# OAID/Tengine

Hardware: AMD Instinct MI355X
Metric: images/sec int8 MobileNet-v1 224x224 (higher is better)
Workload: dtype int8; 1 GPU; mobilenet_v1 int8 batch=1 per GPU (BASELINE configs[1]), weights = seeded synthetic tmfile, input resident in HBM, direct AQL dispatch of the launch list (14 packets per step), 1 stream(s); streams=1, halves=0, global_batch=1, parallelism=dp1, collectives=none

## Files before the change

include/tengine_amd.h:

```cpp
#ifndef TENGINE_AMD_H
#define TENGINE_AMD_H

#include <stddef.h>
#include <stdint.h>

#ifdef __cplusplus
extern "C" {
#endif

#define TAMD_API __attribute__((visibility("default")))

enum { TAMD_DT_FP32 = 0, TAMD_DT_FP16 = 1, TAMD_DT_INT8 = 2, TAMD_DT_UINT8 = 3, TAMD_DT_INT32 = 4 };
enum { TAMD_TT_VAR = 1, TAMD_TT_CONST = 2, TAMD_TT_INPUT = 3 };

enum {
    TAMD_OP_INPUT = 0,
    TAMD_OP_CONST = 1,
    TAMD_OP_CONV = 2,
    TAMD_OP_FC = 3,
    TAMD_OP_POOL = 4,
    TAMD_OP_RELU = 5,
    TAMD_OP_ELTWISE = 6,
    TAMD_OP_CONCAT = 7,
    TAMD_OP_DROPOUT = 8,
    TAMD_OP_UPSAMPLE = 9,
    TAMD_OP_RELU6 = 10,
    TAMD_OP_FLATTEN = 11,
    TAMD_OP_SOFTMAX = 12,
    TAMD_OP_PERMUTE = 13,
    TAMD_OP_RESHAPE = 14,
    TAMD_OP_PRIORBOX = 15,
    TAMD_OP_SIGMOID = 16,
    TAMD_OP_CLIP = 17,
    TAMD_OP_HARDSWISH = 18,
    TAMD_OP_MISH = 19,
    TAMD_OP_INTERP = 20,
    TAMD_OP_SPLIT = 22,
    TAMD_OP_SHUFFLECHANNEL = 23,
    TAMD_OP_PRELU = 25,
    TAMD_OP_SLICE = 26,
    TAMD_OP_TRANSPOSE = 28,
    TAMD_OP_CROP = 30,
    TAMD_OP_BATCHNORM = 32,
    TAMD_OP_NUM
};

typedef struct tamd_conv_param {
    int kernel_h, kernel_w, stride_h, stride_w;
    int pad_h0, pad_h1, pad_w0, pad_w1;
    int dilation_h, dilation_w;
    int input_channel, output_channel, group, activation;
} tamd_conv_param;

typedef struct tamd_fc_param { int num_output; } tamd_fc_param;

typedef struct tamd_pool_param {
    int pool_method, kernel_h, kernel_w, stride_h, stride_w;
    int pad_h0, pad_h1, pad_w0, pad_w1;
    int global, caffe_flavor;
} tamd_pool_param;

typedef struct tamd_relu_param { float negative_slope; } tamd_relu_param;
typedef struct tamd_batchnorm_param { float rescale_factor, eps; int caffe_flavor; } tamd_batchnorm_param;
typedef struct tamd_eltwise_param { int type; int caffe_flavor; float shift, power, scale; } tamd_eltwise_param;
typedef struct tamd_concat_param { int axis; } tamd_concat_param;
typedef struct tamd_upsample_param { float scale; } tamd_upsample_param;
typedef struct tamd_permute_param { int order[4]; } tamd_permute_param;
typedef struct tamd_softmax_param { int axis; } tamd_softmax_param;
typedef struct tamd_reshape_param { int dim_num; int dims[8]; } tamd_reshape_param;
typedef struct tamd_clip_param { float max, min; } tamd_clip_param;
typedef struct tamd_hardswish_param { float alpha, beta; } tamd_hardswish_param;
typedef struct tamd_interp_param { int resize_type; float width_scale, height_scale; int output_width, output_height; } tamd_interp_param;
#define TAMD_SPLIT_MAX 8
typedef struct tamd_split_param { int axis; int num; int sizes[TAMD_SPLIT_MAX]; } tamd_split_param;
typedef struct tamd_shufflechannel_param { int group; } tamd_shufflechannel_param;
typedef struct tamd_slice_param {
    int axis, begin, end, step;
    int iscaffe, ismxnet, isonnx;
    int slice_point_num, begin_num, size_num;
} tamd_slice_param;
typedef struct tamd_transpose_param { int dim_num; int order[8]; } tamd_transpose_param;
typedef struct tamd_crop_param { int num_args, offset_c, offset_h, offset_w, crop_h, crop_w, center_crop, axis, flag; } tamd_crop_param;

#define TAMD_PRIORBOX_MAX 8
typedef struct tamd_priorbox_param {
    int min_size_num, max_size_num, aspect_ratio_num;
    float min_size[TAMD_PRIORBOX_MAX], max_size[TAMD_PRIORBOX_MAX], aspect_ratio[TAMD_PRIORBOX_MAX], variance[4];
    int flip, clip, image_h, image_w;
    float step_h, step_w, offset;
} tamd_priorbox_param;

typedef struct tamd_tensor_desc {
    int dtype;
    int ttype;
    int dim_num;
    int dims[8];
    const void* data;
    int quant_num;
    const float* scales;
    const int* zero_points;
    const char* name;
} tamd_tensor_desc;

typedef struct tamd_node_desc {
    int op;
    int input_num;
    const int* inputs;
    int output_num;
    const int* outputs;
    const void* param;
    const char* name;
} tamd_node_desc;

typedef struct tamd_options {
    const char* dev_name;
    int size;
    int gpu_index;
    int use_hip_graph;
    int profile;
    int direct_dispatch;
    int keep_tensors;
    int u8_integer;
    int split_batch;
} tamd_options;
#define TAMD_OPTIONS_HAS(size, field) ((size) >= (int)(offsetof(tamd_options, field) + sizeof(((const tamd_options*)0)->field)))

typedef struct tamd_graph tamd_graph;

TAMD_API int tamd_device_count(void);
TAMD_API int tamd_init(int gpu_index);
TAMD_API int tamd_shutdown(void);
TAMD_API const char* tamd_last_error(void);
TAMD_API const char* tamd_version(void);
TAMD_API int tamd_op_supported(int op, int dtype);
TAMD_API int tamd_node_supported(const tamd_node_desc* node, const tamd_tensor_desc* inputs, int input_num,
                                 const tamd_tensor_desc* outputs, int output_num);
TAMD_API int tamd_lut_table(int op, int dtype, const void* param, float in_scale, int in_zp, float out_scale, int out_zp,
                            unsigned char table[256]);
TAMD_API int tamd_eltwise_table(int type, int dtype, const tamd_eltwise_param* param, float scalar, float in_scale, int in_zp,
                                float out_scale, int out_zp, unsigned char table[256]);
TAMD_API int tamd_eltwise_scalar(int const_dtype, const void* value, float scale, int zp, float* scalar);
TAMD_API int tamd_eltwise_pair(int type, int dtype, unsigned char a, float a_scale, int a_zp, unsigned char b, float b_scale, int b_zp,
                               float out_scale, int out_zp);
TAMD_API int tamd_batchnorm_table(const tamd_batchnorm_param* param, float gamma, float beta, float mean, float var, float in_scale, int in_zp,
                                  float out_scale, int out_zp, unsigned char table[256]);
TAMD_API int tamd_interp_table(int dtype, float in_scale, int in_zp, float out_scale, int out_zp, unsigned char table[256]);
TAMD_API int tamd_interp_indices(int in_extent, int out_extent, float scale, int* idx);
TAMD_API int tamd_shuffle_sources(int channels, int group, int* src);
TAMD_API int tamd_split_table(float in_scale, int in_zp, float out_scale, int out_zp, unsigned char table[256]);
TAMD_API int tamd_slice_table(float in_scale, int in_zp, float out_scale, int out_zp, unsigned char table[256]);
TAMD_API int tamd_transpose_table(int dtype, float in_scale, int in_zp, float out_scale, int out_zp, unsigned char table[256]);
TAMD_API float tamd_prelu_slope(unsigned short half_bits);
TAMD_API int tamd_prelu_table(int dtype, unsigned short slope_bits, float in_scale, int in_zp, float out_scale, int out_zp,
                              unsigned char table[256]);

TAMD_API tamd_graph* tamd_graph_create(void);
TAMD_API int tamd_graph_add_tensor(tamd_graph* g, const tamd_tensor_desc* desc);
TAMD_API int tamd_graph_add_node(tamd_graph* g, const tamd_node_desc* desc);
TAMD_API int tamd_graph_set_inputs(tamd_graph* g, int n, const int* tensor_ids);
TAMD_API int tamd_graph_set_outputs(tamd_graph* g, int n, const int* tensor_ids);
TAMD_API tamd_graph* tamd_graph_load_tm2(const void* mem, size_t size);
TAMD_API int tamd_graph_set_batch(tamd_graph* g, int batch);

TAMD_API int tamd_graph_prerun(tamd_graph* g, const tamd_options* opt);
TAMD_API int tamd_graph_halves(const tamd_graph* g);
TAMD_API int tamd_graph_slots(const tamd_graph* g);
TAMD_API int tamd_graph_input_num(const tamd_graph* g);
TAMD_API int tamd_graph_output_num(const tamd_graph* g);
TAMD_API int tamd_graph_input_desc(const tamd_graph* g, int idx, int* dims8, int* dtype);
TAMD_API int tamd_graph_output_desc(const tamd_graph* g, int idx, int* dims8, int* dtype, float* scale, int* zero_point);
TAMD_API int tamd_graph_set_input(tamd_graph* g, int idx, const void* host_nchw, size_t bytes);
TAMD_API int tamd_graph_set_output(tamd_graph* g, int idx, void* host_nchw, size_t bytes);
TAMD_API int tamd_graph_run(tamd_graph* g);
TAMD_API int tamd_graph_run_async(tamd_graph* g);
TAMD_API int tamd_graph_wait(tamd_graph* g);
TAMD_API int tamd_graph_inflight(const tamd_graph* g);
TAMD_API int tamd_graph_upload_inputs(tamd_graph* g);
TAMD_API int tamd_graph_launch(tamd_graph* g);
TAMD_API int tamd_graph_sync(tamd_graph* g);
TAMD_API int tamd_graph_direct_packets(const tamd_graph* g);
TAMD_API int tamd_graph_direct_meta_packets(const tamd_graph* g);
TAMD_API int tamd_graph_direct_timestamps(tamd_graph* g, int passes, double* dur_us, double* gap_us, int max_packets);
TAMD_API const char* tamd_graph_direct_packet_name(const tamd_graph* g, int i);
TAMD_API int tamd_graph_slot_timestamps(tamd_graph* g, int passes, double* start_us, double* end_us, int max_stamps);
TAMD_API int tamd_graph_download_outputs(tamd_graph* g);
TAMD_API int tamd_graph_output_device(tamd_graph* g, int idx, void** dptr, size_t* bytes);
TAMD_API void* tamd_graph_stream(tamd_graph* g);
TAMD_API double tamd_graph_prerun_ms(const tamd_graph* g);
TAMD_API int tamd_graph_time_launches(tamd_graph* g, int iters, float* total_ms);

typedef struct tamd_kernel_info {
    char node[64];
    char kernel[48];
    double macs;
    double bytes;
    float ms;
} tamd_kernel_info;
TAMD_API int tamd_graph_kernel_num(const tamd_graph* g);
TAMD_API int tamd_graph_profile(tamd_graph* g, int iters, tamd_kernel_info* out, int max_out);
TAMD_API int tamd_graph_read_tensor(tamd_graph* g, int tensor_idx, void* host_nchw, size_t bytes);
TAMD_API int tamd_graph_tensor_num(const tamd_graph* g);
TAMD_API int tamd_graph_tensor_desc(const tamd_graph* g, int tensor_idx, int* dims8, int* dtype);
TAMD_API int tamd_graph_bytemap_chain(const tamd_graph* g, int node, int* nodes, int cap, unsigned char table[256]);

TAMD_API void tamd_graph_destroy(tamd_graph* g);

#ifdef __cplusplus
}
#endif
#endif
```

tengine_amd/build.py:

```python
import concurrent.futures as cf
import os
import subprocess
import sys

HERE = os.path.dirname(os.path.abspath(__file__))
ROOT = os.path.dirname(HERE)
CSRC = os.path.join(HERE, "csrc")
LIBDIR = os.path.join(HERE, "lib")
OBJDIR = os.path.join(LIBDIR, "obj")
HIPCC = os.environ.get("HIPCC", "/opt/rocm/bin/hipcc")
ARCH = "gfx950"

SOURCES = ["conv_igemm.hip", "conv_igemm2.hip", "conv_pgemm.hip", "conv_pgemm_w.hip", "gemm_direct.hip", "pw_stream.hip", "pw_rows.hip", "conv_first.hip", "conv_first_pool.hip", "dwconv.hip", "dwpw.hip", "block_i8.hip", "pwdw.hip", "pwdw_slices.hip", "chain4.hip", "conv_direct.hip", "misc_kernels.hip", "interp.hip", "chanmap.hip", "prelu.hip", "chan_lut.hip", "chan_gate.hip", "slice.hip", "topdown.hip", "transpose.hip", "u8_kernels.hip", "u8_conv_gemm.hip", "u8_conv_patch.hip", "u8_conv_small.hip", "u8i_kernels.hip", "conv_f32_mfma.hip", "winograd_f32.hip", "f32_kernels.hip", "graph.hip", "graph_infer.hip", "graph_plan.hip", "graph_plan_common.hip", "graph_plan_maps.hip", "graph_plan_conv.hip", "graph_plan_pairs.hip", "plan_cache.hip", "graph_exec.hip", "graph_pair.hip", "graph_slots.hip", "graph_u8.hip", "graph_f32.hip", "tm2_reader.cc", "direct.cc", "lut_tables.cc", "interp_tables.cc", "chanmap_tables.cc", "prelu_tables.cc", "slice_tables.cc", "transpose_tables.cc"]
FLAGS = ["--offload-arch=" + ARCH, "-O3", "-std=c++17", "-fPIC", "-ffp-contract=off", "-fno-fast-math",
         "-fvisibility=hidden", "-Wall", "-Wno-unused-function", "-Wno-unused-variable", "-Wno-unused-value"]
PLAIN_CXX = {"lut_tables.cc", "interp_tables.cc", "chanmap_tables.cc", "prelu_tables.cc", "slice_tables.cc", "transpose_tables.cc"}
PLAIN_FLAGS = ["-O2", "-std=c++17", "-fPIC", "-ffp-contract=off", "-fno-fast-math", "-fvisibility=hidden", "-Wall"]
VGPR_FORM = {"pw_stream.hip", "pw_rows.hip", "conv_igemm.hip", "conv_igemm2.hip", "conv_pgemm.hip", "conv_pgemm_w.hip", "conv_first.hip", "conv_first_pool.hip", "dwpw.hip", "block_i8.hip", "gemm_direct.hip", "u8i_kernels.hip"}


def _newer(target, deps):
    if not os.path.exists(target):
        return True
    t = os.path.getmtime(target)
    return any(os.path.getmtime(d) > t for d in deps)


def build_core(verbose=False, force=False):
    os.makedirs(OBJDIR, exist_ok=True)
    headers = [os.path.join(CSRC, f) for f in os.listdir(CSRC) if f.endswith(".h")] + \
              [os.path.join(ROOT, "include", "tengine_amd.h")]

    def one(src):
        path = os.path.join(CSRC, src)
        obj = os.path.join(OBJDIR, src + ".o")
        included = [os.path.join(CSRC, "pwdw.hip")] if src == "pwdw_slices.hip" else []
        if not force and not _newer(obj, [path, os.path.abspath(__file__)] + headers + included):
            return obj, None
        cmd = [HIPCC] + FLAGS + (["-mllvm", "--amdgpu-mfma-vgpr-form"] if src in VGPR_FORM else []) + \
              (["-x", "hip"] if src.endswith(".cc") else []) + ["-c", path, "-o", obj]
        if src in PLAIN_CXX:
            cmd = [HIPCC, "-x", "c++"] + PLAIN_FLAGS + ["-c", path, "-o", obj]
        r = subprocess.run(cmd, capture_output=True, text=True)
        if verbose and r.stderr:
            sys.stderr.write(r.stderr)
        return obj, (r.stderr if r.returncode else None)

    objs, errs = [], []
    with cf.ThreadPoolExecutor(max_workers=len(SOURCES)) as ex:
        for obj, err in ex.map(one, SOURCES):
            objs.append(obj)
            if err:
                errs.append(err)
    if errs:
        raise RuntimeError("hipcc failed:\n" + "\n".join(errs))
    lib = os.path.join(LIBDIR, "libtengine_amd.so")
    if force or _newer(lib, objs):
        subprocess.check_call([HIPCC, "--offload-arch=" + ARCH, "-shared", "-fPIC", "-o", lib] + objs + ["-lhsa-runtime64"])
    return lib


def build_plugin(ref="/root/reference", verbose=False, force=False):
    src = os.path.join(HERE, "device", "hip_device.cc")
    if not os.path.isdir(os.path.join(ref, "source")) or not os.path.exists(src):
        return None
    lib = os.path.join(LIBDIR, "libtengine_hip_device.so")
    if not force and not _newer(lib, [src, os.path.join(ROOT, "include", "tengine_amd.h")]):
        return lib
    import re
    gen = os.path.join(LIBDIR, "gen")
    os.makedirs(gen, exist_ok=True)
    defines = re.sub(r"#cmakedefine (\w+)", r"#define \1", open(os.path.join(ref, "source", "defines.h.in")).read())
    open(os.path.join(gen, "defines.h"), "w").write(defines)
    cmd = ["g++", "-O2", "-std=c++14", "-fPIC", "-shared", "-fvisibility=hidden", "-I" + os.path.join(ref, "source"),
           "-I" + os.path.join(ref, "source", "operator", "prototype"), "-I" + gen,
           "-I" + os.path.join(ROOT, "include"), src, "-o", lib,
           "-L" + LIBDIR, "-ltengine_amd", "-Wl,-rpath,$ORIGIN:$ORIGIN/../../tengine_amd/lib"]
    subprocess.check_call(cmd)
    return lib


def build_harness(force=False):
    src = os.path.join(HERE, "harness", "rccl_gather.cpp")
    out = os.path.join(LIBDIR, "rccl_gather.bin")
    core = os.path.join(LIBDIR, "libtengine_amd.so")
    if force or _newer(out, [src, core, os.path.join(ROOT, "include", "tengine_amd.h")]):
        subprocess.check_call([HIPCC, "--offload-arch=" + ARCH, "-O2", "-std=c++17", "-I" + os.path.join(ROOT, "include"), "-o", out, src,
                               "-L" + LIBDIR, "-ltengine_amd", "-lrccl", "-Wl,-rpath,$ORIGIN"])
    return out


def build_all(verbose=False, force=False):
    core = build_core(verbose, force)
    plugin = build_plugin(verbose=verbose, force=force)
    build_harness(force)
    return core, plugin


if __name__ == "__main__":
    print(build_all(verbose=True, force="--force" in sys.argv))
```

tengine_amd/capi.py:

```python
import ctypes as C
import os

import numpy as np

HERE = os.path.dirname(os.path.abspath(__file__))
LIB_PATH = os.path.join(HERE, "lib", "libtengine_amd.so")

DT_FP32, DT_FP16, DT_INT8, DT_UINT8, DT_INT32 = 0, 1, 2, 3, 4
_NP = {DT_FP32: np.float32, DT_FP16: np.float16, DT_INT8: np.int8, DT_UINT8: np.uint8, DT_INT32: np.int32}


class Options(C.Structure):
    _fields_ = [("dev_name", C.c_char_p), ("size", C.c_int), ("gpu_index", C.c_int), ("use_hip_graph", C.c_int), ("profile", C.c_int),
                ("direct_dispatch", C.c_int), ("keep_tensors", C.c_int), ("u8_integer", C.c_int), ("split_batch", C.c_int)]


class KernelInfo(C.Structure):
    _fields_ = [("node", C.c_char * 64), ("kernel", C.c_char * 48), ("macs", C.c_double), ("bytes", C.c_double),
                ("ms", C.c_float)]


EXPORTS = [
    "tamd_device_count", "tamd_init", "tamd_shutdown", "tamd_last_error", "tamd_version", "tamd_op_supported", "tamd_node_supported", "tamd_lut_table", "tamd_eltwise_table", "tamd_eltwise_scalar", "tamd_eltwise_pair", "tamd_batchnorm_table", "tamd_interp_table", "tamd_interp_indices", "tamd_shuffle_sources", "tamd_split_table", "tamd_slice_table", "tamd_transpose_table", "tamd_prelu_slope", "tamd_prelu_table",
    "tamd_graph_create", "tamd_graph_add_tensor", "tamd_graph_add_node", "tamd_graph_set_inputs",
    "tamd_graph_set_outputs", "tamd_graph_load_tm2", "tamd_graph_set_batch", "tamd_graph_prerun", "tamd_graph_halves", "tamd_graph_slots",
    "tamd_graph_input_num", "tamd_graph_output_num", "tamd_graph_input_desc", "tamd_graph_output_desc",
    "tamd_graph_set_input", "tamd_graph_set_output", "tamd_graph_run", "tamd_graph_run_async", "tamd_graph_wait", "tamd_graph_inflight", "tamd_graph_upload_inputs",
    "tamd_graph_launch", "tamd_graph_sync", "tamd_graph_direct_packets", "tamd_graph_direct_meta_packets", "tamd_graph_download_outputs", "tamd_graph_output_device",
    "tamd_graph_direct_timestamps", "tamd_graph_slot_timestamps", "tamd_graph_direct_packet_name", "tamd_graph_stream", "tamd_graph_time_launches", "tamd_graph_prerun_ms", "tamd_graph_kernel_num", "tamd_graph_profile",
    "tamd_graph_read_tensor", "tamd_graph_tensor_num", "tamd_graph_tensor_desc", "tamd_graph_bytemap_chain", "tamd_graph_destroy",
]

_lib = None


class TamdError(RuntimeError):
    pass


def version():
    return lib().tamd_version().decode()


def lib():
    global _lib
    if _lib is None:
        if not os.path.exists(LIB_PATH):
            raise TamdError("native library %s is missing: run `python -c 'import __graft_entry__ as g; g.build()'` "
                            "(tengine_amd has no CPU fallback)" % LIB_PATH)
        L = C.CDLL(LIB_PATH)
        vp, ci = C.c_void_p, C.c_int
        L.tamd_last_error.restype = C.c_char_p
        L.tamd_version.restype = C.c_char_p
        L.tamd_graph_create.restype = vp
        L.tamd_graph_load_tm2.restype = vp
        L.tamd_graph_load_tm2.argtypes = [vp, C.c_size_t]
        L.tamd_graph_stream.restype = vp
        L.tamd_graph_direct_packet_name.restype = C.c_char_p
        L.tamd_graph_direct_packet_name.argtypes = [vp, ci]
        L.tamd_graph_direct_timestamps.argtypes = [vp, ci, C.POINTER(C.c_double), C.POINTER(C.c_double), ci]
        if hasattr(L, "tamd_graph_slots"):
            L.tamd_graph_slot_timestamps.argtypes = [vp, ci, C.POINTER(C.c_double), C.POINTER(C.c_double), ci]
            L.tamd_graph_slots.argtypes = [vp]
        L.tamd_graph_prerun_ms.restype = C.c_double
        L.tamd_graph_prerun_ms.argtypes = [vp]
        for name, args in {
            "tamd_graph_set_batch": [vp, ci], "tamd_graph_prerun": [vp, C.POINTER(Options)],
            "tamd_graph_input_num": [vp], "tamd_graph_output_num": [vp], "tamd_graph_halves": [vp],
            "tamd_graph_input_desc": [vp, ci, C.POINTER(ci), C.POINTER(ci)],
            "tamd_graph_output_desc": [vp, ci, C.POINTER(ci), C.POINTER(ci), C.POINTER(C.c_float), C.POINTER(ci)],
            "tamd_graph_set_input": [vp, ci, vp, C.c_size_t], "tamd_graph_set_output": [vp, ci, vp, C.c_size_t],
            "tamd_graph_run": [vp], "tamd_graph_run_async": [vp], "tamd_graph_wait": [vp], "tamd_graph_inflight": [vp],
            "tamd_graph_upload_inputs": [vp], "tamd_graph_launch": [vp],
            "tamd_graph_sync": [vp], "tamd_graph_direct_packets": [vp], "tamd_graph_direct_meta_packets": [vp], "tamd_graph_download_outputs": [vp],
            "tamd_graph_output_device": [vp, ci, C.POINTER(vp), C.POINTER(C.c_size_t)],
            "tamd_graph_stream": [vp], "tamd_graph_time_launches": [vp, ci, C.POINTER(C.c_float)],
            "tamd_graph_kernel_num": [vp], "tamd_graph_profile": [vp, ci, C.POINTER(KernelInfo), ci],
            "tamd_graph_read_tensor": [vp, ci, vp, C.c_size_t], "tamd_graph_tensor_num": [vp],
            "tamd_graph_tensor_desc": [vp, ci, C.POINTER(ci), C.POINTER(ci)], "tamd_graph_destroy": [vp],
            "tamd_init": [ci], "tamd_op_supported": [ci, ci],
        }.items():
            getattr(L, name).argtypes = args
        L.tamd_graph_destroy.restype = None
        L.tamd_lut_table.argtypes = [ci, ci, vp, C.c_float, ci, C.c_float, ci, C.POINTER(C.c_ubyte)]
        if hasattr(L, "tamd_eltwise_table"):
            L.tamd_eltwise_table.argtypes = [ci, ci, vp, C.c_float, C.c_float, ci, C.c_float, ci, C.POINTER(C.c_ubyte)]
            L.tamd_eltwise_scalar.argtypes = [ci, vp, C.c_float, ci, C.POINTER(C.c_float)]
            L.tamd_eltwise_pair.argtypes = [ci, ci, C.c_ubyte, C.c_float, ci, C.c_ubyte, C.c_float, ci, C.c_float, ci]
            L.tamd_graph_bytemap_chain.argtypes = [vp, ci, C.POINTER(ci), ci, C.POINTER(C.c_ubyte)]
            L.tamd_batchnorm_table.argtypes = [vp] + [C.c_float] * 5 + [ci, C.c_float, ci, C.POINTER(C.c_ubyte)]
        L.tamd_interp_table.argtypes = [ci, C.c_float, ci, C.c_float, ci, C.POINTER(C.c_ubyte)]
        L.tamd_interp_indices.argtypes = [ci, ci, C.c_float, C.POINTER(ci)]
        L.tamd_shuffle_sources.argtypes = [ci, ci, C.POINTER(ci)]
        L.tamd_split_table.argtypes = [C.c_float, ci, C.c_float, ci, C.POINTER(C.c_ubyte)]
        L.tamd_slice_table.argtypes = [C.c_float, ci, C.c_float, ci, C.POINTER(C.c_ubyte)]
        L.tamd_transpose_table.argtypes = [ci, C.c_float, ci, C.c_float, ci, C.POINTER(C.c_ubyte)]
        L.tamd_prelu_slope.argtypes = [C.c_ushort]
        L.tamd_prelu_slope.restype = C.c_float
        L.tamd_prelu_table.argtypes = [ci, C.c_ushort, C.c_float, ci, C.c_float, ci, C.POINTER(C.c_ubyte)]
        _lib = L
    return _lib


OP_SIGMOID, OP_CLIP, OP_HARDSWISH, OP_MISH = 16, 17, 18, 19
OP_INTERP = 20
OP_SPLIT, OP_SHUFFLECHANNEL = 22, 23
OP_PRELU = 25
OP_SLICE = 26


class SliceParam(C.Structure):
    _fields_ = [(k, C.c_int) for k in ("axis", "begin", "end", "step", "iscaffe", "ismxnet", "isonnx", "slice_point_num", "begin_num", "size_num")]


def slice_table(in_scale, in_zp, out_scale, out_zp):
    tab = (C.c_ubyte * 256)()
    rc = lib().tamd_slice_table(in_scale, in_zp, out_scale, out_zp, tab)
    return None if rc != 0 else np.frombuffer(tab, dtype=np.uint8).copy()
OP_TRANSPOSE = 28
OP_CROP = 30


class CropParam(C.Structure):
    _fields_ = [(k, C.c_int) for k in ("num_args", "offset_c", "offset_h", "offset_w", "crop_h", "crop_w", "center_crop", "axis", "flag")]


class TransposeParam(C.Structure):
    _fields_ = [("dim_num", C.c_int), ("order", C.c_int * 8)]


def transpose_table(dtype, in_scale, in_zp, out_scale, out_zp):
    tab = (C.c_ubyte * 256)()
    rc = lib().tamd_transpose_table(dtype, in_scale, in_zp, out_scale, out_zp, tab)
    return None if rc != 0 else np.frombuffer(tab, dtype=np.uint8).copy().view(np.int8 if dtype == 2 else np.uint8)


SPLIT_MAX = 8


class SplitParam(C.Structure):
    _fields_ = [("axis", C.c_int), ("num", C.c_int), ("sizes", C.c_int * SPLIT_MAX)]


class ShuffleChannelParam(C.Structure):
    _fields_ = [("group", C.c_int)]


def shuffle_sources(channels, group):
    src = (C.c_int * max(channels, 1))()
    rc = lib().tamd_shuffle_sources(channels, group, src)
    return None if rc != 0 else np.array(src[:channels], dtype=np.int32)


def prelu_slope(half_bits):
    return float(lib().tamd_prelu_slope(int(half_bits) & 0xffff))


def prelu_table(dtype, slope_bits, in_scale, in_zp, out_scale, out_zp):
    tab = (C.c_ubyte * 256)()
    rc = lib().tamd_prelu_table(dtype, int(slope_bits) & 0xffff, in_scale, in_zp, out_scale, out_zp, tab)
    return None if rc != 0 else np.frombuffer(tab, dtype=np.uint8).copy()


def split_table(in_scale, in_zp, out_scale, out_zp):
    tab = (C.c_ubyte * 256)()
    rc = lib().tamd_split_table(in_scale, in_zp, out_scale, out_zp, tab)
    return None if rc != 0 else np.frombuffer(tab, dtype=np.uint8).copy()


def interp_table(dtype, in_scale, in_zp, out_scale, out_zp):
    tab = (C.c_ubyte * 256)()
    rc = lib().tamd_interp_table(dtype, in_scale, in_zp, out_scale, out_zp, tab)
    return None if rc != 0 else np.frombuffer(tab, dtype=np.uint8).copy()


def interp_indices(in_extent, out_extent, scale):
    idx = (C.c_int * max(out_extent, 1))()
    rc = lib().tamd_interp_indices(in_extent, out_extent, scale, idx)
    return None if rc != 0 else np.array(idx[:out_extent], dtype=np.int32)


def lut_table(op, dtype, in_scale, in_zp, out_scale, out_zp, params=None):
    tab = (C.c_ubyte * 256)()
    p = (C.c_float * 2)(*params) if params is not None else None
    rc = lib().tamd_lut_table(op, dtype, C.cast(p, C.c_void_p) if p is not None else None, in_scale, in_zp, out_scale, out_zp, tab)
    return None if rc != 0 else np.frombuffer(tab, dtype=np.uint8).copy()


class EltwiseParam(C.Structure):
    _fields_ = [("type", C.c_int), ("caffe_flavor", C.c_int), ("shift", C.c_float), ("power", C.c_float), ("scale", C.c_float)]


def eltwise_scalar(const_dtype, value, scale=0.0, zp=0):
    v = np.ascontiguousarray(value).reshape(-1)[:1]
    out = C.c_float()
    rc = lib().tamd_eltwise_scalar(const_dtype, v.ctypes.data_as(C.c_void_p), scale, zp, C.byref(out))
    return None if rc != 0 else out.value


def eltwise_table(typ, dtype, scalar, in_scale, in_zp, out_scale, out_zp, shift=0.0, power=1.0, scale=1.0):
    tab = (C.c_ubyte * 256)()
    p = EltwiseParam(typ, 0, shift, power, scale)
    rc = lib().tamd_eltwise_table(typ, dtype, C.cast(C.pointer(p), C.c_void_p), scalar, in_scale, in_zp, out_scale, out_zp, tab)
    return rc, (np.frombuffer(tab, dtype=np.uint8).copy() if rc == 0 else None)


class BatchNormParam(C.Structure):
    _fields_ = [("rescale_factor", C.c_float), ("eps", C.c_float), ("caffe_flavor", C.c_int)]


def batchnorm_table(gamma, beta, mean, var, in_scale, in_zp, out_scale, out_zp, rescale_factor=1.0, eps=1e-5, caffe_flavor=0):
    tab = (C.c_ubyte * 256)()
    p = BatchNormParam(rescale_factor, eps, caffe_flavor)
    rc = lib().tamd_batchnorm_table(C.cast(C.pointer(p), C.c_void_p), gamma, beta, mean, var, in_scale, in_zp, out_scale, out_zp, tab)
    return rc, (np.frombuffer(tab, dtype=np.uint8).copy() if rc == 0 else None)


def eltwise_pair(typ, dtype, a, qa, b, qb, qo):
    return lib().tamd_eltwise_pair(typ, dtype, int(a) & 255, qa[0], int(qa[1]), int(b) & 255, qb[0], int(qb[1]), qo[0], int(qo[1]))


def bytemap_chain(tm_bytes, node):
    L = lib()
    h = L.tamd_graph_load_tm2(tm_bytes, len(tm_bytes))
    if not h:
        raise TamdError("load_tm2 failed: %s" % L.tamd_last_error().decode())
    try:
        nodes, tab = (C.c_int * 64)(), (C.c_ubyte * 256)()
        n = L.tamd_graph_bytemap_chain(h, node, nodes, 64, tab)
        if n < 0:
            raise TamdError("bytemap_chain: bad arguments")
        return (list(nodes[:n]), np.frombuffer(tab, dtype=np.uint8).copy()) if n else ([], None)
    finally:
        L.tamd_graph_destroy(h)


def _check(rc, what):
    if rc is None or (isinstance(rc, int) and rc < 0):
        raise TamdError("%s failed: %s" % (what, lib().tamd_last_error().decode()))
    return rc


def device_count():
    return lib().tamd_device_count()


class Graph:

    def __init__(self, tm_bytes: bytes, batch=None, gpu_index=0, use_hip_graph=True, profile=False, direct_dispatch=False, keep_tensors=False, u8_integer=False, split_batch=0):
        L = lib()
        self._h = L.tamd_graph_load_tm2(tm_bytes, len(tm_bytes))
        if not self._h:
            raise TamdError("tamd_graph_load_tm2 failed: %s" % L.tamd_last_error().decode())
        if batch is not None:
            _check(L.tamd_graph_set_batch(self._h, batch), "set_batch")
        opt = Options(b"HIP", C.sizeof(Options), gpu_index, 1 if use_hip_graph else 0, 1 if profile else 0, 1 if direct_dispatch else 0,
                      1 if keep_tensors else 0, 1 if u8_integer else 0, int(split_batch))
        _check(L.tamd_graph_prerun(self._h, C.byref(opt)), "prerun")
        self._in, self._out = [], []
        for i in range(L.tamd_graph_output_num(self._h)):
            dims = (C.c_int * 8)()
            dt, sc, zp = C.c_int(), C.c_float(), C.c_int()
            nd = L.tamd_graph_output_desc(self._h, i, dims, C.byref(dt), C.byref(sc), C.byref(zp))
            arr = np.zeros([dims[k] for k in range(nd)], _NP[dt.value])
            self._out.append(arr)
            _check(L.tamd_graph_set_output(self._h, i, arr.ctypes.data, arr.nbytes), "set_output")

    def halves(self):
        return lib().tamd_graph_halves(self._h)

    def slots(self):
        return lib().tamd_graph_slots(self._h) if hasattr(lib(), "tamd_graph_slots") else 0

    def slot_timestamps(self, passes=50):
        n = lib().tamd_graph_direct_packets(self._h)
        t0, t1 = (C.c_double * (passes * 2 * n))(), (C.c_double * (passes * 2 * n))()
        r = _check(lib().tamd_graph_slot_timestamps(self._h, passes, t0, t1, passes * 2 * n), "slot_timestamps")
        return (np.array(t0[:r * 2 * n]).reshape(r, 2, n), np.array(t1[:r * 2 * n]).reshape(r, 2, n))

    def input_desc(self, idx=0):
        dims = (C.c_int * 8)()
        dt = C.c_int()
        nd = lib().tamd_graph_input_desc(self._h, idx, dims, C.byref(dt))
        return [dims[k] for k in range(nd)], dt.value

    def set_input(self, arr, idx=0):
        arr = np.ascontiguousarray(arr)
        while len(self._in) <= idx:
            self._in.append(None)
        self._in[idx] = arr
        _check(lib().tamd_graph_set_input(self._h, idx, arr.ctypes.data, arr.nbytes), "set_input")

    def run(self):
        _check(lib().tamd_graph_run(self._h), "run")
        return [o.copy() for o in self._out]

    def run_noreturn(self):
        _check(lib().tamd_graph_run(self._h), "run")

    def run_async(self, out_arrays=None):
        if out_arrays is not None:
            for i, a in enumerate(out_arrays):
                _check(lib().tamd_graph_set_output(self._h, i, a.ctypes.data, a.nbytes), "set_output")
        _check(lib().tamd_graph_run_async(self._h), "run_async")

    def wait(self):
        _check(lib().tamd_graph_wait(self._h), "wait")

    def bind_default_outputs(self):
        for i, a in enumerate(self._out):
            _check(lib().tamd_graph_set_output(self._h, i, a.ctypes.data, a.nbytes), "set_output")

    def output_like(self):
        return [np.zeros_like(o) for o in self._out]

    def output_num(self):
        return lib().tamd_graph_output_num(self._h)

    def upload(self):
        _check(lib().tamd_graph_upload_inputs(self._h), "upload_inputs")

    def launch(self):
        _check(lib().tamd_graph_launch(self._h), "launch")

    def sync(self):
        _check(lib().tamd_graph_sync(self._h), "sync")

    def download(self):
        _check(lib().tamd_graph_download_outputs(self._h), "download_outputs")
        return [o.copy() for o in self._out]

    def time_launches(self, iters):
        ms = C.c_float()
        _check(lib().tamd_graph_time_launches(self._h, iters, C.byref(ms)), "time_launches")
        return ms.value

    def output_device(self, idx=0):
        p, n = C.c_void_p(), C.c_size_t()
        _check(lib().tamd_graph_output_device(self._h, idx, C.byref(p), C.byref(n)), "output_device")
        return p.value, n.value

    def stream(self):
        return lib().tamd_graph_stream(self._h)

    def prerun_ms(self):
        return lib().tamd_graph_prerun_ms(self._h)

    def direct_packets(self):
        return lib().tamd_graph_direct_packets(self._h)

    def direct_timestamps(self, passes=200):
        n = lib().tamd_graph_direct_packets(self._h)
        dur, gap = (C.c_double * n)(), (C.c_double * n)()
        _check(lib().tamd_graph_direct_timestamps(self._h, passes, dur, gap, n), "direct_timestamps")
        return [(lib().tamd_graph_direct_packet_name(self._h, i).decode(), dur[i], gap[i]) for i in range(n)]

    def direct_meta_packets(self):
        return lib().tamd_graph_direct_meta_packets(self._h)

    def kernel_num(self):
        return lib().tamd_graph_kernel_num(self._h)

    def profile(self, iters=10):
        n = lib().tamd_graph_kernel_num(self._h)
        arr = (KernelInfo * n)()
        _check(lib().tamd_graph_profile(self._h, iters, arr, n), "profile")
        return [dict(node=k.node.decode(), kernel=k.kernel.decode(), macs=k.macs, bytes=k.bytes, ms=k.ms) for k in arr]

    def read_tensor(self, idx):
        dims = (C.c_int * 8)()
        dt = C.c_int()
        nd = _check(lib().tamd_graph_tensor_desc(self._h, idx, dims, C.byref(dt)), "tensor_desc")
        arr = np.zeros([dims[k] for k in range(nd)], _NP[dt.value])
        _check(lib().tamd_graph_read_tensor(self._h, idx, arr.ctypes.data, arr.nbytes), "read_tensor")
        return arr

    def close(self):
        if self._h:
            lib().tamd_graph_destroy(self._h)
            self._h = None

    def __del__(self):
        try:
            self.close()
        except Exception:
            pass
```

tengine_amd/csrc/chain4.hip:

```cpp
#include "dw_common.h"
#include "epilogue.h"
#include "kernels.h"

namespace tamd {

typedef int v4i __attribute__((ext_vector_type(4)));

constexpr int kChain4Stage = 8;

__device__ __forceinline__ void dw3x3_from_lds(const unsigned* row, int pitch, const unsigned (&w)[3][4], int (&acc)[4])
{
#pragma unroll
    for (int r = 0; r < 3; r++) {
        const unsigned d[4] = {row[(r * pitch + 0) * 4], row[(r * pitch + 1) * 4], row[(r * pitch + 2) * 4], row[(r * pitch + 3) * 4]};
        unsigned frag[4];
        transpose4x4(d, frag);
#pragma unroll
        for (int c = 0; c < 4; c++) acc[c] = __builtin_amdgcn_sdot4((int)frag[c], (int)w[r][c], acc[c], false);
    }
}

template <int PROD, bool COH, int WIN>
__device__ __forceinline__ void chain4_block(const Chain4Args& a, unsigned* __restrict__ lds)
{
    const int t = threadIdx.x, nthreads = blockDim.x, lane = t & 63;
    const int wave = __builtin_amdgcn_readfirstlane(t >> 6), nwaves = nthreads >> 6;
    const int l15 = lane & 15, kb = lane >> 4;
    const int tx = blockIdx.x, ty = blockIdx.y, n = blockIdx.z;
    const int ns1 = a.ns1, ns2 = a.ns2;

    uint4 wst[kChain4Stage];
#pragma unroll
    for (int k = 0; k < kChain4Stage; k++) {
        wst[k] = reinterpret_cast<const uint4*>(a.blob)[min(t + k * nthreads, a.blob_q - 1)];
    }
    const int cq1 = t & ((1 << a.qsh1) - 1), cq2 = t & ((1 << a.qsh2) - 1);
    const bool on1 = cq1 < ns1 * 4, on2 = cq2 < ns2 * 4;
    const int c1 = (on1 ? cq1 : 0) * 4, c2 = (on2 ? cq2 : 0) * 4;
    unsigned w1[3][4], w2[3][4];
#pragma unroll
    for (int r = 0; r < 3; r++) {
        const uint4 v = *reinterpret_cast<const uint4*>(a.dw1_w + ((size_t)r * ns1 * 16 + c1) * 4);
        w1[r][0] = v.x; w1[r][1] = v.y; w1[r][2] = v.z; w1[r][3] = v.w;
        const uint4 u = *reinterpret_cast<const uint4*>(a.dw2_w + ((size_t)r * ns2 * 16 + c2) * 4);
        w2[r][0] = u.x; w2[r][1] = u.y; w2[r][2] = u.z; w2[r][3] = u.w;
    }
    const int4 db1 = *reinterpret_cast<const int4*>(a.dw1_bias + c1), db2 = *reinterpret_cast<const int4*>(a.dw2_bias + c2);
    const float4 ds1 = *reinterpret_cast<const float4*>(a.dw1_wscale + c1), ds2 = *reinterpret_cast<const float4*>(a.dw2_wscale + c2);

    const int S2 = a.S2, RCW = a.RCW, RAW = a.RCW + 2;
    const int oy0 = ty * a.TH, ox0 = tx * a.TW;
    const int th = min(a.TH, a.OH - oy0), tw = min(a.TW, a.OW - ox0);
    const int cy0 = oy0 * S2 - a.P2H, cx0 = ox0 * S2 - a.P2W;
    const int cvy0 = max(cy0, 0), cvx0 = max(cx0, 0);
    const int cvy1 = min(cy0 + (th - 1) * S2 + 3, a.H1), cvx1 = min(cx0 + (tw - 1) * S2 + 3, a.W1);
    const int ay0 = cy0 - a.P1H, ax0 = cx0 - a.P1W;
    const int avy0 = max(cvy0 - a.P1H, 0), avx0 = max(cvx0 - a.P1W, 0);
    const int avy1 = min(cvy1 + 2 - a.P1H, a.H0), avx1 = min(cvx1 + 2 - a.P1W, a.W0);
    const int AVW = avx1 - avx0, AVP = (avy1 - avy0) * AVW;
    const int CVW = cvx1 - cvx0, CVP = (cvy1 - cvy0) * CVW;
    const float inv_avw = __builtin_amdgcn_rcpf((float)AVW), inv_cvw = __builtin_amdgcn_rcpf((float)CVW);
    const int soffA = ((a.RCH + 2) * RAW + 4) * 4, soffC = (a.RCH * RCW + 4) * 4;
    unsigned* const ldsA = lds + a.blob_q * 4;
    unsigned* const ldsC = ldsA + ns1 * soffA;
    unsigned* const ldsB = ldsC + ns2 * soffC;
    const int8_t* const wl = reinterpret_cast<const int8_t*>(lds);

    int piy = 0, pix = 0;
    auto locate_a = [&](int i, bool& live) -> int {
        const int v = i * 16 + l15, vc = min(v, AVP - 1);
        const int vy = (int)(((float)vc + 0.5f) * inv_avw), vx = vc - vy * AVW;
        piy = avy0 + vy; pix = avx0 + vx;
        live = v < AVP;
        return (piy - ay0) * RAW + (pix - ax0);
    };
    const int8_t* xn = PROD == 0 ? a.x + (size_t)n * a.H0 * a.W0 * a.cs_in + kb * 16 : a.x + (size_t)n * a.in_C * a.in_H * a.in_W;
    unsigned rows[4];
    if (PROD == 1) {
        const uint4 v = *reinterpret_cast<const uint4*>(a.taps + kb * 4);
        rows[0] = v.x; rows[1] = v.y; rows[2] = v.z; rows[3] = v.w;
    }
    const __amdgpu_buffer_rsrc_t xrsrc = __builtin_amdgcn_make_buffer_rsrc((void*)a.x, 0, 0x7fffffff, 0x00020000);
    auto load_b = [&](v4i (&bf)[2]) {
        if (PROD == 0) {
            const int8_t* xp = xn + (unsigned)((piy * a.W0 + pix) * a.cs_in);
            if (COH) {
                const int voff = (int)(xp - a.x);
                bf[0] = __builtin_amdgcn_raw_buffer_load_b128(xrsrc, voff, 0, 16 );
                if (a.ks0 > 1) bf[1] = __builtin_amdgcn_raw_buffer_load_b128(xrsrc, voff, 64, 16);
            } else {
                bf[0] = *reinterpret_cast<const v4i*>(xp);
                if (a.ks0 > 1) bf[1] = *reinterpret_cast<const v4i*>(xp + 64);
            }
        } else {
            gather_patch_rows(a, xn, rows, piy, pix, bf[0]);
        }
    };
    const int ntilesA = (AVP + 15) >> 4;
    v4i b0[2] = {v4i{0, 0, 0, 0}, v4i{0, 0, 0, 0}};
    bool live0;
    int slot0 = locate_a(wave, live0);
    load_b(b0);

    {
        const uint4 z = {0u, 0u, 0u, 0u};
        const int nz = ns1 * (soffA >> 2) + ns2 * (soffC >> 2);
        for (int i = t; i < nz; i += nthreads) reinterpret_cast<uint4*>(ldsA)[i] = z;
#pragma unroll
        for (int k = 0; k < kChain4Stage; k++) {
            const int i = t + k * nthreads;
            if (i < a.blob_q) reinterpret_cast<uint4*>(lds)[i] = wst[k];
        }
    }
    __syncthreads();

    {
        const Rq rq = *reinterpret_cast<const Rq*>(wl + a.off_rq + 0 * (int)sizeof(Rq));
        for (int i = wave; i < ntilesA; i += nwaves) {
            if (i != wave) { slot0 = locate_a(i, live0); load_b(b0); }
            for (int s = 0; s < ns1; s++) {
                const int4 pb = *reinterpret_cast<const int4*>(wl + a.off_b0 + (s * 16 + 4 * kb) * 4);
                const float4 ps = *reinterpret_cast<const float4*>(wl + a.off_s0 + (s * 16 + 4 * kb) * 4);
                v4i acc = v4i{pb.x, pb.y, pb.z, pb.w};
                acc = __builtin_amdgcn_mfma_i32_16x16x64_i8(*reinterpret_cast<const v4i*>(wl + ((s * a.ks0) * 64 + lane) * 16), b0[0], acc, 0, 0, 0);
                if (PROD == 0 && a.ks0 > 1)
                    acc = __builtin_amdgcn_mfma_i32_16x16x64_i8(*reinterpret_cast<const v4i*>(wl + ((s * a.ks0 + 1) * 64 + lane) * 16), b0[1], acc, 0, 0, 0);
                const unsigned p = requant4<WIN>(acc[0], acc[1], acc[2], acc[3], ps, s * 16 + 4 * kb, rq);
                if (live0) ldsA[s * soffA + slot0 * 4 + kb] = p;
            }
        }
    }
    __syncthreads();

    if (on1) {
        const Rq rq = *reinterpret_cast<const Rq*>(wl + a.off_rq + 1 * (int)sizeof(Rq));
        const unsigned* const src = ldsA + (cq1 >> 2) * soffA + (cq1 & 3);
        unsigned* const dst = ldsB + (cq1 >> 2) * soffC + (cq1 & 3);
        for (int q = t >> a.qsh1; q < CVP; q += nthreads >> a.qsh1) {
            const int vy = (int)(((float)q + 0.5f) * inv_cvw), vx = q - vy * CVW;
            const int ly = cvy0 + vy - cy0, lx = cvx0 + vx - cx0;
            const unsigned* row = src + (ly * RAW + lx) * 4;
            int acc[4] = {db1.x, db1.y, db1.z, db1.w};
            dw3x3_from_lds(row, RAW, w1, acc);
            dst[(ly * RCW + lx) * 4] = requant4<WIN>(acc[0], acc[1], acc[2], acc[3], ds1, c1, rq);
        }
    }
    __syncthreads();

    {
        const Rq rq = *reinterpret_cast<const Rq*>(wl + a.off_rq + 2 * (int)sizeof(Rq));
        const int ntilesC = (CVP + 15) >> 4;
        int tile = 0, s = wave;
        while (s >= ns2) { s -= ns2; tile++; }
        while (tile < ntilesC) {
            const int v = tile * 16 + l15, vc = min(v, CVP - 1);
            const int vy = (int)(((float)vc + 0.5f) * inv_cvw), vx = vc - vy * CVW;
            const int slot = (cvy0 + vy - cy0) * RCW + (cvx0 + vx - cx0);
            const v4i bq0 = *reinterpret_cast<const v4i*>(ldsB + min(kb, ns1 - 1) * soffC + slot * 4);
            const int4 pb = *reinterpret_cast<const int4*>(wl + a.off_b2 + (s * 16 + 4 * kb) * 4);
            const float4 ps = *reinterpret_cast<const float4*>(wl + a.off_s2 + (s * 16 + 4 * kb) * 4);
            v4i acc = v4i{pb.x, pb.y, pb.z, pb.w};
            acc = __builtin_amdgcn_mfma_i32_16x16x64_i8(*reinterpret_cast<const v4i*>(wl + a.off_wf2 + ((s * a.ks2) * 64 + lane) * 16), bq0, acc, 0, 0, 0);
            if (a.ks2 > 1) {
                const v4i bq1 = *reinterpret_cast<const v4i*>(ldsB + min(kb + 4, ns1 - 1) * soffC + slot * 4);
                acc = __builtin_amdgcn_mfma_i32_16x16x64_i8(*reinterpret_cast<const v4i*>(wl + a.off_wf2 + ((s * a.ks2 + 1) * 64 + lane) * 16), bq1, acc, 0, 0, 0);
            }
            const unsigned p = requant4<WIN>(acc[0], acc[1], acc[2], acc[3], ps, s * 16 + 4 * kb, rq);
            if (v < CVP) ldsC[s * soffC + slot * 4 + kb] = p;
            s += nwaves;
            while (s >= ns2) { s -= ns2; tile++; }
        }
    }
    __syncthreads();

    if (on2) {
        const Rq rq = *reinterpret_cast<const Rq*>(wl + a.off_rq + 3 * (int)sizeof(Rq));
        const unsigned* const src = ldsC + (cq2 >> 2) * soffC + (cq2 & 3);
        const float inv_tw = __builtin_amdgcn_rcpf((float)tw);
        int8_t* yn = a.y + ((size_t)(n * a.OH + oy0) * a.OW + ox0) * a.ldc + a.c_off + c2;
        for (int q = t >> a.qsh2; q < th * tw; q += nthreads >> a.qsh2) {
            const int oyl = (int)(((float)q + 0.5f) * inv_tw), oxl = q - oyl * tw;
            const unsigned* row = src + ((oyl * S2) * RCW + oxl * S2) * 4;
            int acc[4] = {db2.x, db2.y, db2.z, db2.w};
            dw3x3_from_lds(row, RCW, w2, acc);
            const unsigned p = requant4<WIN>(acc[0], acc[1], acc[2], acc[3], ds2, c2, rq);
            if (c2 < a.c_limit) {
                unsigned* dstp = reinterpret_cast<unsigned*>(yn + ((size_t)oyl * a.OW + oxl) * a.ldc);
                if (COH) __hip_atomic_store(dstp, p, __ATOMIC_RELAXED, __HIP_MEMORY_SCOPE_AGENT); else *dstp = p;
            }
        }
    }
}

template <int PROD, int WIN>
__global__ __launch_bounds__(512) void chain4_i8_kernel(Chain4Args a)
{
    extern __shared__ __attribute__((aligned(16))) unsigned chain4_lds[];
    chain4_block<PROD, false, WIN>(a, chain4_lds);
}

template <int PROD, int WIN>
__global__ __launch_bounds__(512) void chain4_i8_coh_kernel(Chain4Args a)
{
    extern __shared__ __attribute__((aligned(16))) unsigned chain4_lds[];
    chain4_block<PROD, true, WIN>(a, chain4_lds);
}

size_t chain4_lds_bytes(const Chain4Args& a)
{
    const size_t soffA = (size_t)((a.RCH + 2) * (a.RCW + 2) + 4) * 16, soffC = (size_t)(a.RCH * a.RCW + 4) * 16;
    return (size_t)a.blob_q * 16 + a.ns1 * soffA + (size_t)(a.ns2 + a.ns1) * soffC;
}

bool chain4_config_ok(const Chain4Args& a, int threads)
{
    if (threads != 256 && threads != 512) return false;
    if (a.TH < 1 || a.TW < 1 || a.ns1 < 1 || a.ns1 > 8 || a.ns2 < 1 || a.ns2 > 8 || a.ks0 < 1 || a.ks0 > 2 || a.ks2 < 1 || a.ks2 > 2) return false;
    if (a.prod == 1 && a.ks0 != 1) return false;
    if (a.blob_q > kChain4Stage * threads) return false;
    if ((1 << a.qsh1) < a.ns1 * 4 || (1 << a.qsh2) < a.ns2 * 4 || (1 << a.qsh1) > threads || (1 << a.qsh2) > threads) return false;
    if ((a.RCH + 2) * (a.RCW + 2) >= 16384) return false;
    return chain4_lds_bytes(a) <= 64 * 1024;
}

template <int PROD>
static hipError_t launch_chain4_p(const Chain4Args& a, int threads, hipStream_t s)
{
    const dim3 grid(a.tiles_x, a.tiles_y, a.N);
    const size_t lds = chain4_lds_bytes(a);
    const bool win = a.win != 0;
    if (a.coherent) {
        launch_rec_coherent();
        if (win) hipLaunchKernelGGL((chain4_i8_coh_kernel<PROD, 1>), grid, dim3(threads), lds, s, a);
        else hipLaunchKernelGGL((chain4_i8_coh_kernel<PROD, 0>), grid, dim3(threads), lds, s, a);
    } else {
        if (win) hipLaunchKernelGGL((chain4_i8_kernel<PROD, 1>), grid, dim3(threads), lds, s, a);
        else hipLaunchKernelGGL((chain4_i8_kernel<PROD, 0>), grid, dim3(threads), lds, s, a);
    }
    return hipGetLastError();
}

hipError_t launch_chain4(const Chain4Args& a, int threads, hipStream_t s)
{
    if (!chain4_config_ok(a, threads) || a.tiles_y > 65535 || a.N > 65535) return hipErrorInvalidValue;
    return a.prod == 1 ? launch_chain4_p<1>(a, threads, s) : launch_chain4_p<0>(a, threads, s);
}

}
```

tengine_amd/csrc/direct.cc:

```cpp
#include <hip/hip_runtime.h>
#include "env.h"
#include <hsa/hsa.h>
#include <hsa/hsa_ext_amd.h>
#include <hsa/hsa_ven_amd_loader.h>
#include <cxxabi.h>

#include <atomic>
#include <chrono>
#include <cstdio>
#include <cstdlib>
#include <cstring>
#include <map>
#include <mutex>
#include <string>

#include "codeobj_meta.h"
#include "launch_rec.h"

namespace tamd {

thread_local std::vector<LaunchRec>* g_launch_rec = nullptr;
thread_local bool g_launch_coherent = false;
thread_local bool g_launch_beside = false;

// ... 136 lines not shown

const char* direct_last_error() { return g_direct_err; }

bool direct_probe(int gpu)
{
    std::lock_guard<std::mutex> lk(g_mu);
    return device_ctx(gpu) != nullptr;
}

struct DirectProgram {
    DirectQueue* dq = nullptr;

    std::vector<hsa_kernel_dispatch_packet_t> pkts;
    std::vector<uint16_t> hdr;
    void* kernargs = nullptr;
    uint16_t h_open = 0, h_close = 0, h_wrap = 0;
    int n_meta = 0;
    hsa_agent_t agent{};
    std::vector<std::string> names;
};

DirectProgram* direct_build(int gpu, hipStream_t stream, const std::vector<LaunchRec>& recs, const char** why, DirectProgram* share)
{
    static const char* reason = "";
    *why = reason;
    if (recs.empty()) { *why = "empty launch list"; return nullptr; }
    std::lock_guard<std::mutex> lk(g_mu);
    DeviceCtx* ctx = device_ctx(gpu);
    if (!ctx) { *why = "no HSA agent / loader extension for this device"; return nullptr; }
    DirectProgram* p = new DirectProgram;
    std::vector<unsigned char> blob;
    std::vector<size_t> offs;
    std::vector<char> coherent;
    bool scanned = false;
    int n_meta = 0;
    for (const LaunchRec& r : recs) {
        const char* nm = hipKernelNameRefByPtr(r.func, stream);
        if (!nm) { *why = "kernel without a name"; delete p; return nullptr; }
        const std::string key = std::string(nm) + ".kd";
        auto it = ctx->syms.find(key);
        if (it == ctx->syms.end() && !scanned) { rescan(ctx); scanned = true; it = ctx->syms.find(key); }
        if (it == ctx->syms.end()) { *why = "kernel descriptor not found among the loaded code objects"; delete p; return nullptr; }
        const KernelSym& k = it->second;
        static const bool allow_scratch = !(exp_env("TAMD_DIRECT_SCRATCH") && atoi(exp_env("TAMD_DIRECT_SCRATCH")) == 0);
        if (k.priv != 0 && !allow_scratch) { *why = "a kernel of the list uses scratch memory"; delete p; return nullptr; }
        if (r.args.size() > k.kernarg) { *why = "recorded arguments exceed the kernel's argument segment"; delete p; return nullptr; }
        HiddenLayout hl;
        {
            static const bool use_meta = !(exp_env("TAMD_DIRECT_META") && atoi(exp_env("TAMD_DIRECT_META")) == 0);
            auto lt = ctx->layouts.find(key);
            if (use_meta && lt != ctx->layouts.end()) {
                hl = lt->second;
                if ((size_t)hl.explicit_end > ((r.args.size() + 7) & ~(size_t)7) || (size_t)hl.explicit_end + 8 < r.args.size()) {
                    *why = "recorded arguments do not match the kernel's metadata"; delete p; return nullptr;
                }
                n_meta++;
            } else {
                const int hid = (int)((r.args.size() + 7) & ~(size_t)7);
                for (int a3 = 0; a3 < 3; a3++) { hl.block_count[a3] = hid + 4 * a3; hl.group_size[a3] = hid + 12 + 2 * a3; hl.remainder[a3] = hid + 18 + 2 * a3; }
                hl.grid_dims = hid + 64;
            }
        }
        size_t seg = k.kernarg;
        for (int a3 = 0; a3 < 3; a3++) seg = std::max<size_t>(seg, std::max(hl.block_count[a3] + 4, std::max(hl.group_size[a3], hl.remainder[a3]) + 2));
        seg = std::max<size_t>(seg, std::max<size_t>(hl.grid_dims + 2, r.args.size()));
        const size_t off = (blob.size() + 255) & ~(size_t)255;
        blob.resize(off + seg, 0);
        memcpy(blob.data() + off, r.args.data(), r.args.size());
        const uint32_t bc[3] = {r.grid.x, r.grid.y, r.grid.z};
        const uint16_t gs[3] = {(uint16_t)r.block.x, (uint16_t)r.block.y, (uint16_t)r.block.z};
        const uint16_t dims = r.grid.z * r.block.z > 1 ? 3 : (r.grid.y * r.block.y > 1 ? 2 : 1), zero16 = 0;
        for (int a3 = 0; a3 < 3; a3++) {
            if (hl.block_count[a3] >= 0) memcpy(blob.data() + off + hl.block_count[a3], &bc[a3], 4);
            if (hl.group_size[a3] >= 0) memcpy(blob.data() + off + hl.group_size[a3], &gs[a3], 2);
            if (hl.remainder[a3] >= 0) memcpy(blob.data() + off + hl.remainder[a3], &zero16, 2);
        }
        if (hl.grid_dims >= 0) memcpy(blob.data() + off + hl.grid_dims, &dims, 2);
        offs.push_back(off);
        hsa_kernel_dispatch_packet_t pk{};
        pk.setup = (uint16_t)(dims << HSA_KERNEL_DISPATCH_PACKET_SETUP_DIMENSIONS);
        pk.workgroup_size_x = gs[0]; pk.workgroup_size_y = gs[1]; pk.workgroup_size_z = gs[2];
        pk.grid_size_x = r.grid.x * r.block.x; pk.grid_size_y = r.grid.y * r.block.y; pk.grid_size_z = r.grid.z * r.block.z;
        pk.private_segment_size = k.priv;
        pk.group_segment_size = k.group + r.shmem;
        pk.kernel_object = k.object;
        p->pkts.push_back(pk);
        {
            int st = 0;
            char* dm = abi::__cxa_demangle(nm, nullptr, nullptr, &st);
            p->names.push_back(st == 0 && dm ? std::string(dm) : std::string(nm));
            free(dm);
        }
        const bool allow_none = tamd_pin_int("direct_coherent", 1) != 0;
        coherent.push_back(allow_none && r.coherent);
    }
    if (hipMalloc(&p->kernargs, blob.size()) != hipSuccess || hipMemcpy(p->kernargs, blob.data(), blob.size(), hipMemcpyHostToDevice) != hipSuccess) {
        (void)hipGetLastError();
        *why = "kernel-argument buffer"; direct_destroy(p); return nullptr;
    }
    if (ctx->have_cpu) {
        hsa_agent_t both[2] = {ctx->agent, ctx->cpu};
        (void)hsa_amd_agents_allow_access(2, both, nullptr, p->kernargs);
    }
    for (size_t i = 0; i < p->pkts.size(); i++) p->pkts[i].kernarg_address = (char*)p->kernargs + offs[i];
    if (share) {
        p->dq = share->dq;
    } else {
        p->dq = new DirectQueue;
        uint32_t qsize = 1024;
        while (qsize < 8 * p->pkts.size()) qsize *= 2;
        if (hsa_queue_create(ctx->agent, qsize, HSA_QUEUE_TYPE_SINGLE, queue_fault, p->dq, UINT32_MAX, UINT32_MAX, &p->dq->q) != HSA_STATUS_SUCCESS) {
            *why = "hsa_queue_create"; p->dq->q = nullptr; p->dq->refs = 1; direct_destroy(p); return nullptr;
        }
        if (hsa_signal_create(DirectQueue::kStart, 0, nullptr, &p->dq->done) != HSA_STATUS_SUCCESS) { *why = "hsa_signal_create"; p->dq->refs = 1; direct_destroy(p); return nullptr; }
        if (const char* cm = exp_env("TAMD_DIRECT_CU_MASK")) {
            uint32_t mask[8] = {0, 0, 0, 0, 0, 0, 0, 0};
            if (!strcmp(cm, "first32")) mask[0] = 0xffffffffu;
            else if (!strcmp(cm, "stride8")) for (int i = 0; i < 8; i++) mask[i] = 0x01010101u;
            else if (!strcmp(cm, "first64")) mask[0] = mask[1] = 0xffffffffu;
            else if (!strcmp(cm, "stride4")) for (int i = 0; i < 8; i++) mask[i] = 0x11111111u;
            if (mask[0]) {
                const hsa_status_t st = hsa_amd_queue_cu_set_mask(p->dq->q, 256, mask);
                if (getenv("TAMD_DEBUG")) fprintf(stderr, "[tamd] direct queue CU mask %s: %s\n", cm, st == HSA_STATUS_SUCCESS ? "set" : "REFUSED");
            }
        }
    }
    p->dq->refs++;
    p->agent = ctx->agent;
    if (p->pkts.size() * 2 > p->dq->q->size) { *why = "launch list longer than the shared queue"; direct_destroy(p); return nullptr; }
    auto header = [](int type, int acq, int rel, bool barrier = true) {
        return (uint16_t)((type << HSA_PACKET_HEADER_TYPE) | ((barrier ? 1 : 0) << HSA_PACKET_HEADER_BARRIER) | (acq << HSA_PACKET_HEADER_SCACQUIRE_FENCE_SCOPE)
                          | (rel << HSA_PACKET_HEADER_SCRELEASE_FENCE_SCOPE));
    };
    const int K = HSA_PACKET_TYPE_KERNEL_DISPATCH;
    int n_beside = 0;
    for (size_t i = 0; i < p->pkts.size(); i++) {
        const bool beside = i > 0 && recs[i].beside;
        n_beside += beside;
        static const bool exp_nofence = exp_env("TAMD_EXP_NOFENCE") != nullptr;
        if (!coherent[i] && exp_nofence) p->hdr.push_back(header(K, HSA_FENCE_SCOPE_NONE, HSA_FENCE_SCOPE_NONE, !beside));
        else if (!coherent[i]) p->hdr.push_back(header(K, beside ? HSA_FENCE_SCOPE_NONE : HSA_FENCE_SCOPE_AGENT, HSA_FENCE_SCOPE_AGENT, !beside));
        else p->hdr.push_back(header(K, (i > 0 && !coherent[i - 1]) ? HSA_FENCE_SCOPE_AGENT : HSA_FENCE_SCOPE_NONE, HSA_FENCE_SCOPE_NONE));
    }
    if (getenv("TAMD_DEBUG")) fprintf(stderr, "[tamd] direct: %zu packets, %d without the barrier bit, hidden arguments of %d from code-object metadata\n", p->pkts.size(), n_beside, n_meta);
    p->n_meta = n_meta;
    p->h_open = header(K, HSA_FENCE_SCOPE_SYSTEM, coherent[0] ? HSA_FENCE_SCOPE_NONE : HSA_FENCE_SCOPE_AGENT);
    p->h_close = header(HSA_PACKET_TYPE_BARRIER_AND, HSA_FENCE_SCOPE_AGENT, HSA_FENCE_SCOPE_SYSTEM);
    p->h_wrap = (!recs.empty() && recs[0].wrap) ? (uint16_t)(p->hdr[0] & ~(1u << HSA_PACKET_HEADER_BARRIER)) : p->hdr[0];
    if (getenv("TAMD_DEBUG") && p->h_wrap != p->hdr[0]) fprintf(stderr, "[tamd] direct: the first launch of a pass runs beside the end of the previous pass\n");
    return p;
}

int direct_packets(const DirectProgram* p) { return p ? (int)p->pkts.size() : 0; }
const char* direct_packet_name(const DirectProgram* p, int i) { return (p && i >= 0 && i < (int)p->names.size()) ? p->names[i].c_str() : ""; }


static int submit_stamped(DirectProgram* p, const hsa_signal_t* sig)
{
    const int n = (int)p->pkts.size();
    DirectQueue* dq = p->dq;
    hsa_queue_t* q = dq->q;
    hsa_kernel_dispatch_packet_t* base = (hsa_kernel_dispatch_packet_t*)q->base_address;
    const uint64_t mask = q->size - 1;
    const uint64_t idx0 = hsa_queue_add_write_index_relaxed(q, (uint64_t)n);
    while (idx0 + n - hsa_queue_load_read_index_scacquire(q) > q->size)
        if (dq->fault.load()) return -1;
    for (int i = 0; i < n; i++) {
        hsa_kernel_dispatch_packet_t* d = base + ((idx0 + i) & mask);
        const hsa_kernel_dispatch_packet_t& s = p->pkts[i];
        d->setup = s.setup;
        d->workgroup_size_x = s.workgroup_size_x; d->workgroup_size_y = s.workgroup_size_y; d->workgroup_size_z = s.workgroup_size_z;
        d->reserved0 = 0;
        d->grid_size_x = s.grid_size_x; d->grid_size_y = s.grid_size_y; d->grid_size_z = s.grid_size_z;
        d->private_segment_size = s.private_segment_size; d->group_segment_size = s.group_segment_size;
        d->kernel_object = s.kernel_object; d->kernarg_address = s.kernarg_address; d->reserved2 = 0;
        d->completion_signal = sig[i];
        const uint16_t h = i == 0 ? (dq->open ? p->h_wrap : p->h_open) : p->hdr[i];
        __atomic_store_n(&d->header, h, __ATOMIC_RELEASE);
    }
    const uint64_t to_end = q->size - (idx0 & mask);
    if (to_end < (uint64_t)n) hsa_signal_store_screlease(q->doorbell_signal, (hsa_signal_value_t)(idx0 + to_end - 1));
    hsa_signal_store_screlease(q->doorbell_signal, (hsa_signal_value_t)(idx0 + n - 1));
    dq->open = true;
    return 0;
}

int direct_timestamps_two(DirectProgram* a, DirectProgram* b, int passes, double* start_us, double* end_us)
{
    const int n = (int)a->pkts.size();
    if (n == 0 || (int)b->pkts.size() != n || passes < 1 || a->dq == b->dq) { direct_err("two programs of the same list on two queues are needed", 0); return -1; }
    DirectProgram* prog[2] = {a, b};
    if (direct_wait_all(a) || direct_wait_all(b)) return -1;
    uint64_t freq = 0;
    if (hsa_system_get_info(HSA_SYSTEM_INFO_TIMESTAMP_FREQUENCY, &freq) != HSA_STATUS_SUCCESS || !freq) { direct_err("no timestamp frequency", 0); return -1; }
    for (DirectProgram* p : prog)
        if (hsa_amd_profiling_set_profiler_enabled(p->dq->q, 1) != HSA_STATUS_SUCCESS) { direct_err("hsa_amd_profiling_set_profiler_enabled", 0); return -1; }
    const int extra = 3, all = passes + extra;
    std::vector<hsa_signal_t> sig((size_t)all * 2 * n);
    for (auto& s : sig)
        if (hsa_signal_create(1, 0, nullptr, &s) != HSA_STATUS_SUCCESS) { direct_err("hsa_signal_create", 0); return -1; }
    int rc = 0;
    for (int ps = 0; ps < all && !rc; ps++) {
        for (int k = 0; k < 2 && !rc; k++) rc = submit_stamped(prog[k], &sig[((size_t)ps * 2 + k) * n]);
        if (ps + 1 == extra && !rc) rc = direct_wait(a) || direct_wait(b) ? -1 : 0;
    }
    if (!rc) rc = direct_wait(a) || direct_wait(b) ? -1 : 0;
    std::vector<uint64_t> t0(sig.size(), 0), t1(sig.size(), 0);
    for (size_t k = 0; k < sig.size() && !rc; k++) {
        hsa_amd_profiling_dispatch_time_t t{};
        if (hsa_amd_profiling_get_dispatch_time(a->agent, sig[k], &t) != HSA_STATUS_SUCCESS) { direct_err("hsa_amd_profiling_get_dispatch_time", (int)k); rc = -1; break; }
        t0[k] = t.start; t1[k] = t.end;
    }
    for (DirectProgram* p : prog) (void)hsa_amd_profiling_set_profiler_enabled(p->dq->q, 0);
    for (auto& s : sig) (void)hsa_signal_destroy(s);
    if (rc) return -1;
    int first_ok = extra;
    for (size_t k = 0; k < sig.size(); k++)
        if (t1[k] <= t0[k]) first_ok = std::max(first_ok, (int)(k / ((size_t)2 * n)) + 1);
    if (first_ok >= all) { direct_err("no round of the burst carries dispatch stamps throughout", all); return -1; }
    const size_t first = (size_t)first_ok * 2 * n;
    uint64_t origin = ~(uint64_t)0;
    for (size_t k = first; k < sig.size(); k++) origin = std::min(origin, t0[k]);
    for (size_t k = first; k < sig.size(); k++) {
        start_us[k - first] = 1e6 * (double)(t0[k] - origin) / (double)freq;
        end_us[k - first] = 1e6 * (double)(t1[k] - origin) / (double)freq;
    }
    return all - first_ok;
}

int direct_timestamps(DirectProgram* p, int passes, double* dur_us, double* gap_us)
{
    const int n = (int)p->pkts.size();
    if (n == 0 || passes < 1) return -1;
    DirectQueue* dq = p->dq;
    if (direct_wait_all(p)) return -1;
    uint64_t freq = 0;
    if (hsa_system_get_info(HSA_SYSTEM_INFO_TIMESTAMP_FREQUENCY, &freq) != HSA_STATUS_SUCCESS || !freq) { direct_err("no timestamp frequency", 0); return -1; }
    if (hsa_amd_profiling_set_profiler_enabled(dq->q, 1) != HSA_STATUS_SUCCESS) { direct_err("hsa_amd_profiling_set_profiler_enabled", 0); return -1; }
    passes += passes < 20 ? 3 : 1;
    std::vector<hsa_signal_t> sig((size_t)n * passes);
    for (auto& s : sig)
        if (hsa_signal_create(1, 0, nullptr, &s) != HSA_STATUS_SUCCESS) { direct_err("hsa_signal_create", 0); return -1; }
    int rc = 0;
    for (int ps = 0; ps < passes && !rc; ps++) {
        rc = submit_stamped(p, &sig[(size_t)ps * n]);
        if (ps == 0 && !rc) rc = direct_wait(p);
    }
    if (!rc) rc = direct_wait(p);
    std::vector<double> t0((size_t)n * passes, 0.0), t1((size_t)n * passes, 0.0);
    int first_ok = 1, n_bad = 0, last_bad = -1;
    for (size_t k = 0; k < sig.size() && !rc; k++) {
        hsa_amd_profiling_dispatch_time_t t{};
        if (hsa_amd_profiling_get_dispatch_time(p->agent, sig[k], &t) != HSA_STATUS_SUCCESS) { direct_err("hsa_amd_profiling_get_dispatch_time", (int)k); rc = -1; break; }
        if (getenv("TAMD_DEBUG") && k >= (size_t)n && k < (size_t)n + 4)
            fprintf(stderr, "[tamd] stamp %zu: start %llu end %llu (%lld ticks), system timestamp frequency %llu Hz\n", k, (unsigned long long)t.start,
                    (unsigned long long)t.end, (long long)(t.end - t.start), (unsigned long long)freq);
        if (t.end <= t.start) { first_ok = std::max(first_ok, (int)(k / (size_t)n) + 1); n_bad++; last_bad = (int)k; }
        const uint64_t origin = 0;
        t0[k] = 1e6 * (double)(t.start - origin) / (double)freq; t1[k] = 1e6 * (double)(t.end - origin) / (double)freq;
    }
    (void)hsa_amd_profiling_set_profiler_enabled(dq->q, 0);
    for (auto& s : sig) (void)hsa_signal_destroy(s);
    if (rc) return -1;
    if (first_ok >= passes) {
        char msg[200];
        snprintf(msg, sizeof(msg), "no pass carries dispatch stamps throughout: %d of %d packets without (the last one: packet %d of pass %d, %s)", n_bad, n * passes,
                 last_bad % n, last_bad / n, direct_packet_name(p, last_bad % n));
        direct_err(msg, passes - 1);
        return -1;
    }
    for (int i = 0; i < n; i++) {
        double d = 0, g = 0;
        int ng = 0;
        for (int ps = first_ok; ps < passes; ps++) {
            const size_t k = (size_t)ps * n + i;
            d += t1[k] - t0[k];
            if (k + 1 < sig.size()) { g += t0[k + 1] - t1[k]; ng++; }
        }
        dur_us[i] = d / (passes - first_ok);
        gap_us[i] = ng ? g / ng : 0.0;
    }
    return n;
}
int direct_meta_packets(const DirectProgram* p) { return p ? p->n_meta : 0; }

int direct_submit(DirectProgram* p, bool close_burst, unsigned long long* burst)
{
    const uint64_t n = p->pkts.size();
    DirectQueue* dq = p->dq;
    hsa_queue_t* q = dq->q;
    if (dq->fault.load()) { direct_err("the HSA queue is in the error state (a dispatched kernel faulted)", dq->fault.load()); return -1; }
    const uint64_t idx0 = hsa_queue_add_write_index_relaxed(q, n);
    if (idx0 + n - hsa_queue_load_read_index_scacquire(q) > q->size) {
        const auto t0 = std::chrono::steady_clock::now();
        while (idx0 + n - hsa_queue_load_read_index_scacquire(q) > q->size) {
            if (dq->fault.load() || std::chrono::duration<double>(std::chrono::steady_clock::now() - t0).count() > wait_limit_s()) {
                if (!dq->fault.load()) dq->fault.store(-2);
                direct_err("the HSA queue does not drain (faulted kernel or hung device)", dq->fault.load());
                return -1;
            }
        }
    }
    hsa_kernel_dispatch_packet_t* base = (hsa_kernel_dispatch_packet_t*)q->base_address;
    const uint64_t mask = q->size - 1;
    for (uint64_t i = 0; i < n; i++) {
        hsa_kernel_dispatch_packet_t* d = base + ((idx0 + i) & mask);
// ... 104 lines not shown
```

tengine_amd/csrc/graph.h:

```cpp
#pragma once
#include <hip/hip_runtime.h>

#include <functional>
#include <atomic>
#include <map>
#include <string>
#include <vector>

#include "../../include/tengine_amd.h"
#include "graph_slots.h"
#include "kernels.h"
#include "node_rules.h"

namespace tamd {

void set_error(const char* fmt, ...);
static inline int rup(int v, int m) { return (v + m - 1) / m * m; }

struct HTensor {
    int dtype = 0, ttype = TAMD_TT_VAR;
    std::vector<int> dims;
    std::vector<uint8_t> data;
    std::vector<float> scales;
    std::vector<int> zps;
// ... 39 lines not shown
};

struct Access {
    const char* base = nullptr;
    size_t size = 0, off = 0, len = 0, period = 0;
};
inline bool access_overlap(const Access& a, const Access& b)
{
    if (a.base + a.size <= b.base || b.base + b.size <= a.base) return false;
    if (a.base == b.base && a.size == b.size && a.period > 0 && a.period == b.period) return !(a.off + a.len <= b.off || b.off + b.len <= a.off);
    return true;
}

struct Step {
    std::string node, kernel;
    double macs = 0, bytes = 0;
    std::function<hipError_t(hipStream_t)> fn;
    bool once = false;
    bool deps = false;
    std::vector<Access> rd, wr;
};
inline bool step_conflict(const Step& a, const Step& b)
{
    for (auto& w : a.wr) { for (auto& x : b.wr) if (access_overlap(w, x)) return true; for (auto& x : b.rd) if (access_overlap(w, x)) return true; }
    for (auto& r : a.rd) for (auto& x : b.wr) if (access_overlap(r, x)) return true;
    return false;
}
inline bool step_states_nothing(const Step& s) { return s.rd.empty() || s.wr.empty(); }
inline bool step_writes_what_it_reads(const Step& s)
{
    for (auto& w : s.wr)
        for (auto& r : s.rd)
            if (access_overlap(w, r)) return true;
    return false;
}
inline Step make_step(const std::string& node, const std::string& kernel, double macs, double bytes, std::function<hipError_t(hipStream_t)> fn,
                      std::vector<Access> rd, std::vector<Access> wr, bool deps)
{
    Step st;
    st.node = node; st.kernel = kernel; st.macs = macs; st.bytes = bytes; st.fn = std::move(fn);
    st.rd = std::move(rd); st.wr = std::move(wr); st.deps = deps;
    return st;
}
inline Access access_of(const HTensor& t)
{
    Access a;
    a.base = (const char*)t.dptr;
    const size_t esz = t.dtype == TAMD_DT_FP32 ? 4 : 1;
    if (t.nchw_raw || t.cs <= 0) {
        if (t.is_view && t.cs > 0) {
            a.period = (size_t)t.cs * t.h * t.w * esz; a.off = (size_t)t.c_off * t.h * t.w * esz; a.len = (size_t)t.c * t.h * t.w * esz;
            a.size = a.period * (size_t)t.n;
        } else {
            a.size = t.elems() * esz; a.len = a.size;
        }
    } else {
        a.size = (size_t)t.n * t.h * t.w * t.cs;
        if (t.is_view) { a.period = (size_t)t.cs; a.off = (size_t)t.c_off; a.len = (size_t)t.c; }
        else a.len = a.size;
    }
    return a;
}
inline Access access_of_bytes(const void* p, size_t bytes)
{
    Access a;
    a.base = (const char*)p; a.size = bytes; a.len = bytes;
    return a;
}

inline Access access_of_channels(const HTensor& t, int first, int count)
{
    Access a;
    a.base = (const char*)t.dptr;
    a.size = (size_t)t.n * t.h * t.w * t.cs;
    a.period = (size_t)t.cs; a.off = (size_t)(t.c_off + first); a.len = (size_t)count;
    return a;
}
inline Access access_of_slot(const HTensor& y, size_t period, size_t off, size_t len, size_t esz)
{
    Access a;
    a.base = (const char*)y.dptr;
    a.size = y.elems() * esz; a.period = period * esz; a.off = off * esz; a.len = len * esz;
    return a;
}

struct IOBind {
    int tensor = -1;
    const void* host_in = nullptr;
    void* host_out = nullptr;
    size_t bytes = 0;
    void* stage = nullptr;
    void* pinned[2] = {nullptr, nullptr};
};

struct IoSlot {
    DirectProgram* direct = nullptr;
    bool zero_copy = false;
    hipGraph_t hgraph = nullptr;
    hipGraphExec_t hexec[2] = {nullptr, nullptr};
    int next_exec = 0;
    hipEvent_t done = nullptr;
};

struct Inflight {
    int io_slot = 0;
    std::vector<void*> host_out;
    hipEvent_t done = nullptr;
    bool direct = false;
    unsigned long long burst = 0;
};

struct PoolGeom { int oh, ow, kh, kw, sh, sw, ph0, pw0; };

struct DevArena { char* base = nullptr; size_t cap = 0, used = 0; };

}

#define HIPCHK(expr)                                                                              \
    do {                                                                                          \
        hipError_t e_ = (expr);                                                                   \
        if (e_ != hipSuccess) {                                                                   \
            tamd::set_error("%s failed: %s (%s:%d)", #expr, hipGetErrorString(e_), __FILE__, __LINE__); \
            return -1;                                                                            \
        }                                                                                         \
    } while (0)

struct tamd_graph {
    std::atomic<unsigned long> owner{0};
    std::vector<tamd::HTensor> tensors;
    std::vector<tamd::HNode> nodes;
    std::vector<tamd::IOBind> inputs, outputs;
    std::vector<tamd::Step> steps;
    std::vector<tamd::Step> in_steps;
    std::vector<tamd::Step> out_steps;
    std::vector<void*> dev_allocs;
    std::vector<tamd::DevArena> arenas;
    std::vector<char> pooled;
    size_t pool_bytes = 0, unpooled_bytes = 0;
    std::map<int, float*> f32_copy;
    std::vector<char> fused_away;
    void* zero_page = nullptr;
    hipStream_t stream = nullptr;
    hipGraph_t hgraph = nullptr;
    hipGraphExec_t hexec = nullptr;
    hipGraphExec_t hexecs[4] = {nullptr, nullptr, nullptr, nullptr};
    int nexec = 0, next_exec = 0;
    tamd::IoSlot io[2];
    int next_io_slot = 0;
    std::vector<tamd::Inflight> inflight;
    tamd::DirectProgram* direct = nullptr;
    tamd::DirectProgram* direct1 = nullptr;
    void* slot_block = nullptr;
    std::vector<tamd::SlotSpan> slot_spans;
    int slot_turn = 0;
    bool slot_hold = false;
    bool had_once = false;
    int autotune_cold = -1;
    double prerun_ms = 0;
    bool direct_busy = false;
    bool stream_dirty = true;
    bool stream_exposed = false;
    int out_fresh_in = -1;
    long long h2h_ns[5] = {0, 0, 0, 0, 0};
    long long h2h_runs = 0;
    tamd_options opt{};
    bool prepared = false;
    int gpu = 0;
    tamd_graph* half[2] = {nullptr, nullptr};
    bool is_half = false;
    int formula_batch = 0;
    std::vector<void*> pair_out;
};

namespace tamd {

PoolGeom pool_geom(const tamd_pool_param& p, int h, int w);
int dev_alloc(tamd_graph* g, void** p, size_t bytes, bool zero);
struct RaceCand {
    std::string tag;
    std::function<hipError_t(hipStream_t)> fn;
    std::string name;
    std::function<bool()> live;
};
int plan_race(tamd_graph* g, const std::string& node, const std::vector<RaceCand>& cands, const std::string& key, float margin, bool tune);
int plan_cached(const std::string& key, const std::vector<RaceCand>& cands);
bool autotune_enabled();
void nhwc_geom(HTensor& t);
int append_steps(tamd_graph* g, const std::vector<Step>& launches);
int count_consumers(const tamd_graph* g, int tensor);
int plan_nchw_buffers(tamd_graph* g, size_t esz, const std::function<bool(const HNode& producer, const HTensor& x, const HTensor& cat)>& in_place);
int plan_nchw_outputs(tamd_graph* g, size_t esz);
int plan_lut(tamd_graph* g, HNode& n, std::vector<Step>* out);
int plan_interp(tamd_graph* g, HNode& n, std::vector<Step>* out, const HNode* crop = nullptr);
int plan_split_u8(tamd_graph* g, HNode& n, std::vector<Step>* out);
int plan_shuffle_u8(tamd_graph* g, HNode& n, std::vector<Step>* out);
int plan_prelu(tamd_graph* g, HNode& n, std::vector<Step>* out);
const char* prelu_refusal_of(const tamd_graph* g, const HNode& n);
const char* slice_refusal_of(const tamd_graph* g, const HNode& n, bool check_out, SliceGeom* geom, unsigned char* table);
int slice_chain_next(const tamd_graph* g, size_t ni);
int plan_slice_u8(tamd_graph* g, HNode& n, int next, std::vector<Step>* out);
const char* transpose_refusal_of(const tamd_graph* g, const HNode& n, bool check_out, TransposeGeom* geom, unsigned char* table);
bool nhwc_view_strides(const HTensor& s, const std::vector<int>& dims, long* strides);
int plan_transpose(tamd_graph* g, HNode& n, int view_src, std::vector<Step>* out);
const char* crop_refusal_of(const tamd_graph* g, const HNode& n, bool check_out, CropGeom* geom);
int crop_interp_producer(const tamd_graph* g, size_t ci);
int crop_topdown_next(const tamd_graph* g, size_t ci);
int plan_crop_u8(tamd_graph* g, HNode& n, std::vector<Step>* out);
int plan_topdown_u8(tamd_graph* g, HNode& in, HNode& cn, HNode& n, std::vector<Step>* out);
const char* eltwise_refusal_of(const tamd_graph* g, const HNode& n, int* gated, unsigned char* table = nullptr);
const char* batchnorm_refusal_of(const tamd_graph* g, const HNode& n, std::vector<unsigned>* tables);
int plan_batchnorm_u8(tamd_graph* g, HNode& n, std::vector<Step>* out);
int plan_eltwise_table(tamd_graph* g, HNode& n, std::vector<Step>* out);
struct ByteChain {
    int src = -1, last = -1;
    std::vector<int> nodes;
    unsigned char table[256];
};
bool bytemap_chain_from(const tamd_graph* g, size_t ni, const std::function<bool(int)>& node_free, const std::function<bool(int)>& tensor_plain, ByteChain* c);
int plan_bytemap_chain(tamd_graph* g, const ByteChain& c, std::vector<Step>* out);
int gate_lut_producer(const tamd_graph* g, const HNode& e, int gated);
int plan_chan_gate(tamd_graph* g, HNode& n, int gated, int lut_node, std::vector<Step>* out);
inline int nchw_out_img(const HTensor& t) { return (t.is_view ? t.cs : t.c) * t.h * t.w; }
struct AxisSplit { int axis = 0, outer = 1, on = 0, inner = 1; };
int axis_split(const std::vector<int>& dims, int axis, const char* what, const std::string& node, AxisSplit* s);
std::vector<unsigned> conv_tap_table(int K, int Kpad, int H, int W, int KH, int KW, int DH, int DW);
int priorbox_count(const tamd_priorbox_param& p);
void priorbox_eval(const tamd_priorbox_param& p, int feat_h, int feat_w, int data_h, int data_w, std::vector<float>* out);
void priorbox_quant_u8(const std::vector<float>& f, float scale, int zp, std::vector<uint8_t>* q);
void priorbox_quant_i8(const std::vector<float>& f, float scale, std::vector<int8_t>* q);
int plan_u8(tamd_graph* g);
int plan_f32(tamd_graph* g);

template <typename T>
int upload(tamd_graph* g, const std::vector<T>& host, T** dev)
{
    void* p = nullptr;
    if (dev_alloc(g, &p, host.size() * sizeof(T), false)) return -1;
    HIPCHK(hipMemcpyAsync(p, host.data(), host.size() * sizeof(T), hipMemcpyHostToDevice, g->stream));
    HIPCHK(hipStreamSynchronize(g->stream));
    *dev = (T*)p;
    return 0;
}

template <typename T>
int upload_bias(tamd_graph* g, const HTensor* b, int n, const T** dev)
{
    if (!b) return 0;
    std::vector<T> hb((const T*)b->data.data(), (const T*)b->data.data() + n);
    T* d = nullptr;
    if (upload(g, hb, &d)) return -1;
    *dev = d;
    return 0;
}

template <typename F>
int conv_f32_mfma_operands(tamd_graph* g, F32ConvArgs& a, int KH, int KW, int DH, int DW, F wk)
{
    a.cfg = conv_f32_mfma_pick(a);
    const int BM = conv_f32_mfma_bm(a.cfg), ntile = (a.cout + BM - 1) / BM, nstage = a.Kpad / 32, G = 64 / BM, NIg = 32 / G;
    std::vector<float> wf((size_t)ntile * nstage * 32 * BM, 0.f);
    for (int co = 0; co < a.cout; co++)
        for (int k = 0; k < a.K; k++) {
            const int r = k & 31;
            wf[(((size_t)(co / BM) * nstage + (k >> 5)) * NIg + r / G) * 64 + (r % G) * BM + co % BM] = wk(co, k);
        }
    float* dwf = nullptr; unsigned* dlut = nullptr;
    if (upload(g, wf, &dwf) || upload(g, conv_tap_table(a.K, a.Kpad, a.H, a.W, KH, KW, DH, DW), &dlut)) return -1;
    a.w = dwf; a.klut = dlut;
    return 0;
}

}
```

tengine_amd/csrc/graph_exec.hip:

```cpp
#include "graph.h"
#include "graph_internal.h"
#include "env.h"

#include <stdio.h>
#include <string.h>

#include <algorithm>
#include <chrono>

namespace tamd {

int run_steps(tamd_graph* g, hipStream_t s, int io_slot)
{
    if (io_slot >= 0)
        for (auto& io : g->inputs) {
            hipError_t e = launch_copy_bytes(io.stage, io.pinned[io_slot], io.bytes, s);
            if (e != hipSuccess) { set_error("input upload launch failed: %s", hipGetErrorString(e)); return -1; }
        }
    const char* ov_env = exp_env("TAMD_DIRECT_OVERLAP");
    const bool overlap = g_launch_rec && ov_env && atoi(ov_env) == 1;
    const char* wr_env = exp_env("TAMD_DIRECT_WRAP");
    const bool wrap = g_launch_rec && io_slot < 0 && wr_env && atoi(wr_env) == 1;
    const size_t rec0 = g_launch_rec ? g_launch_rec->size() : 0;
    const Step *first_step = nullptr, *last_step = nullptr;
    size_t last_step_recs = 0;
    std::vector<const Step*> open;
    for (auto* v : {&g->in_steps, &g->steps, &g->out_steps})
        for (auto& st : *v) {
            if (overlap) {
                bool beside = st.deps && !open.empty();
                for (size_t i = 0; i < open.size() && beside; i++) beside = open[i]->deps && !step_conflict(st, *open[i]);
                if (beside) launch_rec_beside();
                else open.clear();
                open.push_back(&st);
            }
            const size_t before = g_launch_rec ? g_launch_rec->size() : 0;
            hipError_t e = st.fn(s);
            launch_rec_clear_flags();
            if (e != hipSuccess) { set_error("launch %s (%s) failed: %s", st.kernel.c_str(), st.node.c_str(), hipGetErrorString(e)); return -1; }
            if (!first_step) first_step = &st;
            last_step = &st;
            last_step_recs = g_launch_rec ? g_launch_rec->size() - before : 0;
        }
    if (wrap && first_step && last_step && first_step != last_step && first_step->deps && last_step->deps && last_step_recs == 1
        && !(overlap && open.size() > 1) && !step_conflict(*first_step, *last_step) && g_launch_rec->size() > rec0)
        (*g_launch_rec)[rec0].wrap = true;
    if (io_slot >= 0)
        for (auto& io : g->outputs) {
            hipError_t e = launch_copy_bytes(io.pinned[io_slot], io.stage, io.bytes, s);
            if (e != hipSuccess) { set_error("output download launch failed: %s", hipGetErrorString(e)); return -1; }
        }
    return 0;
}

static int launch_io(tamd_graph* g, int io_slot)
{
    IoSlot& s = g->io[io_slot];
    if (s.hexec[0]) {
        hipGraphExec_t e = s.hexec[s.next_exec];
        s.next_exec ^= 1;
        HIPCHK(hipGraphLaunch(e, g->stream));
        return 0;
    }
    return run_steps(g, g->stream, io_slot);
}

int record_pass(tamd_graph* g, int io_slot, std::vector<LaunchRec>* recs)
{
    recs->clear();
    g_launch_rec = recs;
    const int rc = run_steps(g, g->stream, io_slot);
    g_launch_rec = nullptr;
    if (rc) return -1;
    HIPCHK(hipStreamSynchronize(g->stream));
    return 0;
}

int selfcheck_fill_inputs(tamd_graph* g, unsigned seed, int io_slot)
{
    std::vector<unsigned char> noise;
    unsigned lcg = seed;
    for (auto& io : g->inputs) {
        noise.resize(io.bytes);
        if (g->tensors[io.tensor].dtype == TAMD_DT_FP32) {
            float* f = (float*)noise.data();
            for (size_t i = 0; i < io.bytes / 4; i++) { lcg = lcg * 1664525u + 1013904223u; f[i] = (float)((int)(lcg >> 20) - 2048) / 1024.f; }
        } else
            for (size_t i = 0; i < io.bytes; i++) { lcg = lcg * 1664525u + 1013904223u; noise[i] = (unsigned char)(lcg >> 24); }
        if (io_slot >= 0) memcpy(io.pinned[io_slot], noise.data(), io.bytes);
        else HIPCHK(hipMemcpy(io.stage, noise.data(), io.bytes, hipMemcpyHostToDevice));
    }
    return 0;
}

int selfcheck_snapshot(const tamd_graph* g, OutputBytes* dst, int io_slot, const std::vector<SlotSpan>* spans)
{
    dst->clear();
    for (auto& io : g->outputs) {
        dst->emplace_back(io.bytes);
        if (io_slot >= 0) { memcpy(dst->back().data(), io.pinned[io_slot], io.bytes); continue; }
        const void* src = spans ? (const void*)slot_moved(*spans, (uintptr_t)io.stage) : io.stage;
        HIPCHK(hipMemcpy(dst->back().data(), src, io.bytes, hipMemcpyDeviceToHost));
    }
    return 0;
}

int selfcheck_same(const OutputBytes& want, const OutputBytes& got, const char* fmt)
{
    for (size_t i = 0; i < want.size(); i++)
        if (want[i] != got[i]) { set_error(fmt, i); return -1; }
    return 0;
}

int direct_selfcheck(tamd_graph* g)
{
    OutputBytes want, got;
    if (selfcheck_fill_inputs(g, 0x5EED1234u) || run_steps(g, g->stream)) return -1;
    HIPCHK(hipStreamSynchronize(g->stream));
    if (selfcheck_snapshot(g, &want)) return -1;
    if (selfcheck_fill_inputs(g, 0x0BADF00Du) || run_steps(g, g->stream)) return -1;
    HIPCHK(hipStreamSynchronize(g->stream));
    if (selfcheck_fill_inputs(g, 0x5EED1234u)) return -1;
    HIPCHK(hipDeviceSynchronize());
    if (direct_submit(g->direct) || direct_wait(g->direct)) { set_error("direct pass failed: %s", direct_last_error()); return -1; }
    if (selfcheck_snapshot(g, &got)) return -1;
    for (auto& io : g->inputs) HIPCHK(hipMemset(io.stage, 0, io.bytes));
    HIPCHK(hipDeviceSynchronize());
    return selfcheck_same(want, got, "the direct pass does not reproduce the eager pass (output %zu differs)");
}

static int patch_pointer(std::vector<LaunchRec>& recs, size_t nrecs, const void* from, const void* to)
{
    int hits = 0;
    for (size_t r = 0; r < nrecs; r++)
        for (size_t off = 0; off + 8 <= recs[r].args.size(); off += 8) {
            const void* v;
            memcpy(&v, recs[r].args.data() + off, 8);
            if (v == from) { memcpy(recs[r].args.data() + off, &to, 8); hits++; }
        }
    return hits;
}

static bool zero_copy_outputs(tamd_graph* g, std::vector<LaunchRec>& recs, int io_slot)
{
    const char* e = getenv("TAMD_IO_ZERO_COPY");
    const size_t nout = g->outputs.size();
    if ((e && atoi(e) == 0) || nout == 0 || recs.size() <= nout + g->inputs.size()) return false;
    const size_t body = recs.size() - nout;
    std::vector<LaunchRec> trial(recs.begin(), recs.begin() + body);
    for (auto& io : g->outputs) {
        const HTensor& t = g->tensors[io.tensor];
        if (io.stage == t.dptr && count_consumers(g, io.tensor) != 1) return false;
        if (t.prerun_const) return false;
        void* dev = nullptr;
        if (hipHostGetDevicePointer(&dev, io.pinned[io_slot], 0) != hipSuccess) { (void)hipGetLastError(); return false; }
        if (patch_pointer(trial, body, io.stage, dev) < 1) return false;
    }
    recs.swap(trial);
    return true;
}

static bool zero_copy_inputs(tamd_graph* g, std::vector<LaunchRec>& recs, int io_slot)
{
    const char* e = exp_env("TAMD_IO_ZERO_COPY_IN");
    const size_t nin = g->inputs.size();
    if (!(e && atoi(e) == 1) || nin == 0 || recs.size() <= nin) return false;
    std::vector<LaunchRec> trial(recs.begin() + nin, recs.end());
    for (auto& io : g->inputs) {
        void* dev = nullptr;
        if (hipHostGetDevicePointer(&dev, io.pinned[io_slot], 0) != hipSuccess) { (void)hipGetLastError(); return false; }
        if (patch_pointer(trial, trial.size(), io.stage, dev) < 1) return false;
    }
    recs.swap(trial);
    return true;
}

static int direct_io_selfcheck(tamd_graph* g, DirectProgram* pio, int io_slot)
{
    OutputBytes want, got;
    if (selfcheck_fill_inputs(g, 0xC0FFEE11u + (unsigned)io_slot, io_slot) || run_steps(g, g->stream, io_slot)) return -1;
    HIPCHK(hipStreamSynchronize(g->stream));
    if (selfcheck_snapshot(g, &want, io_slot)) return -1;
    for (auto& io : g->outputs) memset(io.pinned[io_slot], 0xA5, io.bytes);
    HIPCHK(hipDeviceSynchronize());
    unsigned long long b = 0;
    if (direct_submit(pio, true, &b) || direct_wait_burst(pio, b)) { set_error("direct host-to-host pass failed: %s", direct_last_error()); return -1; }
    if (selfcheck_snapshot(g, &got, io_slot)) return -1;
    return selfcheck_same(want, got, "the direct host-to-host pass does not reproduce the eager list (output %zu differs)");
}

int build_io_program(tamd_graph* g, int io_slot)
{
    std::vector<LaunchRec> recs;
    if (record_pass(g, io_slot, &recs)) return -1;
    const std::vector<LaunchRec> with_downloads = recs;
    bool zc = zero_copy_outputs(g, recs, io_slot);
    if (zero_copy_inputs(g, recs, io_slot)) zc = true;
    const char* why = "";
    DirectProgram* pio = direct_build(g->gpu, g->stream, recs, &why, g->direct);
    if (pio && direct_io_selfcheck(g, pio, io_slot)) {
        if (zc) fprintf(stderr, "tengine_amd: zero-copy outputs DISABLED for this graph: %s\n", last_error());
        direct_destroy(pio);
        why = last_error();
        pio = zc ? direct_build(g->gpu, g->stream, with_downloads, &why, g->direct) : nullptr;
        zc = false;
        if (pio && direct_io_selfcheck(g, pio, io_slot)) { direct_destroy(pio); pio = nullptr; why = last_error(); }
    }
    if (!pio) fprintf(stderr, "tengine_amd: direct dispatch not used for host-to-host runs (slot %d): %s\n", io_slot, why);
    g->io[io_slot].direct = pio;
    g->io[io_slot].zero_copy = zc && pio;
    return 0;
}


int bind_device(tamd_graph* g)
{
    if (!g) { set_error("null graph"); return -1; }
    HIPCHK(hipSetDevice(g->gpu));
    return 0;
}

int direct_drain(tamd_graph* g)
{
    if (g->direct && g->direct_busy) {
        if (direct_wait(g->direct) || (g->direct1 && direct_wait(g->direct1))) { set_error("direct dispatch: %s", direct_last_error()); return -1; }
        g->direct_busy = false;
    }
    g->slot_turn = 0;
    return 0;
}

void direct_teardown(tamd_graph* g)
{
    for (int s = 1; s >= 0; s--)
        if (g->io[s].direct) { direct_destroy(g->io[s].direct); g->io[s].direct = nullptr; }
    slots_destroy(g);
    if (g->direct) { direct_destroy(g->direct); g->direct = nullptr; }
}

static int direct_abandon(tamd_graph* g)
{
    set_error("direct dispatch: %s", direct_last_error());
    fprintf(stderr, "tengine_amd: direct dispatch abandoned for this graph (%s): hipGraph replay from here on\n", last_error());
    g->inflight.erase(std::remove_if(g->inflight.begin(), g->inflight.end(), [](const Inflight& f) { return f.direct; }), g->inflight.end());
    direct_teardown(g);
    g->direct_busy = false;
    return -1;
}

static inline long long now_ns() { return std::chrono::duration_cast<std::chrono::nanoseconds>(std::chrono::steady_clock::now().time_since_epoch()).count(); }
static bool close_on_last_packet()
{
    const char* e = tamd_pin("direct_close_on_last");
    return !(e && atoi(e) == 0);
}

static int submit_burst(DirectProgram* p, unsigned long long* burst)
{
    return close_on_last_packet() ? direct_submit(p, true, burst) : (direct_submit(p) || direct_close(p, burst));
}

static int drain_stream_if_pending(tamd_graph* g)
{
    if (g->stream_dirty || g->stream_exposed) { HIPCHK(hipStreamSynchronize(g->stream)); g->stream_dirty = false; }
    return 0;
}

int stage_from_pinned(tamd_graph* g)
{
    if (g->out_fresh_in < 0) return 0;
    if (!g->inflight.empty()) { set_error("the outputs of the last host-to-host run live in a pinned buffer that a run in flight may overwrite: tamd_graph_wait first"); return -1; }
    if (direct_drain(g)) return -1;
    for (auto& io : g->outputs)
        HIPCHK(hipMemcpyAsync(io.stage, io.pinned[g->out_fresh_in], io.bytes, hipMemcpyHostToDevice, g->stream));
    HIPCHK(hipStreamSynchronize(g->stream));
    g->out_fresh_in = -1;
    return 0;
}

}

using namespace tamd;

extern "C" {

int tamd_graph_upload_inputs(tamd_graph* g)
{
    TAMD_ONE_THREAD(g);
    if (bind_device(g)) return -1;
    if (g->half[0]) return pair_both(g, tamd_graph_upload_inputs);
    if (!g->inflight.empty()) { set_error("tamd_graph_upload_inputs while asynchronous runs are in flight (they own the pinned buffers): collect them with tamd_graph_wait first"); return -1; }
    if (direct_drain(g)) return -1;
    if (!g->prepared) { set_error("graph not prepared"); return -1; }
    for (auto& io : g->inputs) {
        if (!io.host_in) { set_error("input buffer not set"); return -1; }
        memcpy(io.pinned[0], io.host_in, io.bytes);
        HIPCHK(hipMemcpyAsync(io.stage, io.pinned[0], io.bytes, hipMemcpyHostToDevice, g->stream));
    }
    g->stream_dirty = true;
    return 0;
}

int tamd_graph_launch(tamd_graph* g)
{
    TAMD_ONE_THREAD(g);
    if (bind_device(g)) return -1;
    if (!g->prepared) { set_error("graph not prepared"); return -1; }
    if (g->half[0]) return pair_both(g, tamd_graph_launch);
    g->out_fresh_in = -1;
    if (g->direct) {
        if (!g->direct_busy) { HIPCHK(hipStreamSynchronize(g->stream)); g->stream_dirty = false; }
        g->direct_busy = true;
        DirectProgram* p = g->direct;
        if (g->direct1 && !g->slot_hold) { if (g->slot_turn) p = g->direct1; g->slot_turn ^= 1; }
        if (direct_submit(p)) { set_error("direct dispatch: %s", direct_last_error()); return -1; }
        return 0;
    }
    g->stream_dirty = true;
    if (g->hexec) {
        hipGraphExec_t e = g->hexecs[g->next_exec];
        g->next_exec = (g->next_exec + 1) % g->nexec;
        HIPCHK(hipGraphLaunch(e, g->stream));
        return 0;
    }
    return run_steps(g, g->stream);
}

int tamd_graph_direct_packets(const tamd_graph* g) { return g && g->half[0] ? pair_direct_packets(g, false) : g && g->direct ? direct_packets(g->direct) : 0; }
int tamd_graph_direct_meta_packets(const tamd_graph* g) { return g && g->half[0] ? pair_direct_packets(g, true) : g && g->direct ? direct_meta_packets(g->direct) : 0; }
const char* tamd_graph_direct_packet_name(const tamd_graph* g, int i) { return g && g->half[0] ? pair_direct_packet_name(g, i) : g && g->direct ? direct_packet_name(g->direct, i) : ""; }

int tamd_graph_direct_timestamps(tamd_graph* g, int passes, double* dur_us, double* gap_us, int max_packets)
{
    if (!g) { set_error("null graph"); return -1; }
    TAMD_ONE_THREAD(g);
    if (bind_device(g)) return -1;
    if (g->half[0]) return pair_direct_timestamps(g, passes, dur_us, gap_us, max_packets);
    if (!g->prepared || !g->direct) { set_error("tamd_graph_direct_timestamps: the graph does not dispatch directly (tamd_options.direct_dispatch)"); return -1; }
    if (!g->inflight.empty()) { set_error("tamd_graph_direct_timestamps while asynchronous runs are in flight"); return -1; }
    if (max_packets < direct_packets(g->direct)) { set_error("tamd_graph_direct_timestamps: %d packets, room for %d", direct_packets(g->direct), max_packets); return -1; }
    if (direct_drain(g)) return -1;
    HIPCHK(hipStreamSynchronize(g->stream));
    g->stream_dirty = false;
    g->out_fresh_in = -1;
    const int n = direct_timestamps(g->direct, passes, dur_us, gap_us);
    if (n < 0) { set_error("direct dispatch: %s", direct_last_error()); return -1; }
    return n;
}
int tamd_graph_slot_timestamps(tamd_graph* g, int passes, double* start_us, double* end_us, int max_stamps)
{
    if (!g) { set_error("null graph"); return -1; }
    TAMD_ONE_THREAD(g);
    if (bind_device(g)) return -1;
    if (!g->prepared || g->half[0]) { set_error("tamd_graph_slot_timestamps: the graph has one launch list (tamd_graph_slots() == 0)"); return -1; }
    if (!g->inflight.empty()) { set_error("tamd_graph_slot_timestamps while asynchronous runs are in flight"); return -1; }
    if (direct_drain(g)) return -1;
    HIPCHK(hipStreamSynchronize(g->stream));
    g->stream_dirty = false;
    g->out_fresh_in = -1;
    return slots_timestamps(g, passes, start_us, end_us, max_stamps);
}
double tamd_graph_prerun_ms(const tamd_graph* g) { return g ? g->prerun_ms : 0.0; }

int tamd_graph_sync(tamd_graph* g)
{
    TAMD_ONE_THREAD(g);
    if (bind_device(g)) return -1;
    if (g->half[0]) return pair_both(g, tamd_graph_sync);
    if (direct_drain(g)) return -1;
    if (g->io[0].direct && !g->inflight.empty() && direct_wait_all(g->io[0].direct)) { set_error("direct dispatch: %s", direct_last_error()); return -1; }
    HIPCHK(hipStreamSynchronize(g->stream));
    g->stream_dirty = false;
    return 0;
}

int tamd_graph_download_outputs(tamd_graph* g)
{
    TAMD_ONE_THREAD(g);
    if (bind_device(g)) return -1;
    if (g->half[0]) return pair_both(g, tamd_graph_download_outputs);
    if (!g->inflight.empty()) { set_error("tamd_graph_download_outputs while asynchronous runs are in flight (they own the pinned buffers): collect them with tamd_graph_wait first"); return -1; }
    if (direct_drain(g)) return -1;
    if (g->out_fresh_in >= 0) {
        for (auto& io : g->outputs)
            if (io.host_out) memcpy(io.host_out, io.pinned[g->out_fresh_in], io.bytes);
        return 0;
    }
    for (auto& io : g->outputs) HIPCHK(hipMemcpyAsync(io.pinned[0], io.stage, io.bytes, hipMemcpyDeviceToHost, g->stream));
    HIPCHK(hipStreamSynchronize(g->stream));
    for (auto& io : g->outputs)
        if (io.host_out) memcpy(io.host_out, io.pinned[0], io.bytes);
    return 0;
}

int tamd_graph_run(tamd_graph* g)
{
    TAMD_ONE_THREAD(g);
    if (!g || !g->prepared) { set_error("graph not prepared"); return -1; }
    if (g->half[0]) return pair_run(g);
    if (!g->inflight.empty()) { set_error("tamd_graph_run while asynchronous runs are in flight: collect them with tamd_graph_wait first"); return -1; }
    if (bind_device(g)) return -1;
    if (direct_drain(g)) return -1;
    static const bool trace = getenv("TAMD_H2H_TRACE") && atoi(getenv("TAMD_H2H_TRACE")) == 1;
    long long t[6] = {0, 0, 0, 0, 0, 0};
    if (trace) t[0] = now_ns();
    for (auto& io : g->inputs) {
        if (!io.host_in) { set_error("input buffer not set"); return -1; }
        memcpy(io.pinned[0], io.host_in, io.bytes);
    }
    if (trace) t[1] = now_ns();
    IoSlot& s = g->io[0];
    if (s.direct) {
        if (drain_stream_if_pending(g)) return -1;
        if (trace) t[2] = now_ns();
        unsigned long long b = 0;
        const int rc = submit_burst(s.direct, &b);
        if (trace) t[3] = now_ns();
        if (rc || direct_wait_burst(s.direct, b)) return direct_abandon(g);
    } else {
        if (trace) t[2] = t[3] = now_ns();
        if (launch_io(g, 0)) return -1;
        HIPCHK(hipStreamSynchronize(g->stream));
    }
    if (trace) t[4] = now_ns();
    g->out_fresh_in = (s.direct && s.zero_copy) ? 0 : -1;
    for (auto& io : g->outputs)
        if (io.host_out) memcpy(io.host_out, io.pinned[0], io.bytes);
    if (trace) {
        t[5] = now_ns();
        for (int i = 0; i < 5; i++) g->h2h_ns[i] += t[i + 1] - t[i];
        g->h2h_runs++;
    }
    return 0;
}

int tamd_graph_run_async(tamd_graph* g)
{
    TAMD_ONE_THREAD(g);
    if (!g || !g->prepared) { set_error("graph not prepared"); return -1; }
    if (bind_device(g)) return -1;
    if (g->half[0]) return pair_run_async(g);
    if (g->inflight.size() >= 2) { set_error("two runs are already in flight: call tamd_graph_wait first"); return -1; }
    if (direct_drain(g)) return -1;
    Inflight f;
    f.io_slot = g->next_io_slot;
    IoSlot& s = g->io[f.io_slot];
    for (auto& io : g->inputs) {
        if (!io.host_in) { set_error("input buffer not set"); return -1; }
        memcpy(io.pinned[f.io_slot], io.host_in, io.bytes);
    }
    for (auto& io : g->outputs) f.host_out.push_back(io.host_out);
    if (g->io[0].direct && g->io[1].direct) {
        if (g->inflight.empty() && drain_stream_if_pending(g)) return -1;
        if (submit_burst(s.direct, &f.burst)) return direct_abandon(g);
        f.direct = true;
    } else {
        if (!s.done) HIPCHK(hipEventCreateWithFlags(&s.done, hipEventDisableTiming));
        g->stream_dirty = true;
        if (launch_io(g, f.io_slot)) return -1;
        f.done = s.done;
        HIPCHK(hipEventRecord(f.done, g->stream));
    }
    g->inflight.push_back(f);
    g->next_io_slot ^= 1;
    return 0;
}

int tamd_graph_wait(tamd_graph* g)
{
    TAMD_ONE_THREAD(g);
    if (g && g->half[0]) return pair_wait(g);
    if (!g || g->inflight.empty()) { set_error("tamd_graph_wait: no run in flight"); return -1; }
    if (bind_device(g)) return -1;
    const Inflight f = g->inflight.front();
    if (f.direct) {
        if (direct_wait_burst(g->io[0].direct, f.burst)) return direct_abandon(g);
    } else
        HIPCHK(hipEventSynchronize(f.done));
    for (size_t i = 0; i < g->outputs.size(); i++)
        if (f.host_out[i]) memcpy(f.host_out[i], g->outputs[i].pinned[f.io_slot], g->outputs[i].bytes);
    g->out_fresh_in = (f.direct && g->io[f.io_slot].zero_copy) ? f.io_slot : -1;
    g->inflight.erase(g->inflight.begin());
    return 0;
}

int tamd_graph_inflight(const tamd_graph* g) { return !g ? 0 : g->half[0] ? tamd_graph_inflight(g->half[0]) : (int)g->inflight.size(); }

int tamd_graph_output_device(tamd_graph* g, int idx, void** dptr, size_t* bytes)
{
    if (!g) { set_error("null graph"); return -1; }
    TAMD_ONE_THREAD(g);
    if (idx < 0 || idx >= (int)g->outputs.size() || !g->prepared) return -1;
    if (g->half[0]) return pair_output_device(g, idx, dptr, bytes);
    if (g->out_fresh_in >= 0 && (bind_device(g) || stage_from_pinned(g))) return -1;
    *dptr = g->outputs[idx].stage;
    *bytes = g->outputs[idx].bytes;
    return 0;
}

void* tamd_graph_stream(tamd_graph* g)
{
    if (g->half[0]) { (void)tamd_graph_stream(g->half[1]); return tamd_graph_stream(g->half[0]); }
    g->stream_exposed = true; g->stream_dirty = true;
    return (void*)g->stream;
}

int tamd_graph_time_launches(tamd_graph* g, int iters, float* total_ms)
{
    TAMD_ONE_THREAD(g);
    if (bind_device(g)) return -1;
    if (g->half[0]) return pair_time_launches(g, iters, total_ms);
    if (g->direct) {
        if (direct_drain(g)) return -1;
// ... 26 lines not shown
```

tengine_amd/csrc/graph_internal.h:

```cpp
#pragma once
#include <mutex>

#include "graph.h"
#include "launch_rec.h"

namespace tamd {

extern std::mutex g_capture_mutex;
const char* last_error();

static inline int esize(int dt) { return (dt == TAMD_DT_FP32 || dt == TAMD_DT_INT32) ? 4 : (dt == TAMD_DT_FP16 ? 2 : 1); }
static inline int cdiv_c(int a, int b) { return a / b; }

int infer_shapes(tamd_graph* g);
int validate_graph(tamd_graph* g);
int plan_i8(tamd_graph* g);
void plan_cache_flush();

int run_steps(tamd_graph* g, hipStream_t s, int io_slot = -1);
int record_pass(tamd_graph* g, int io_slot, std::vector<LaunchRec>* recs);
int direct_selfcheck(tamd_graph* g);
int selfcheck_fill_inputs(tamd_graph* g, unsigned seed, int io_slot = -1);
typedef std::vector<std::vector<unsigned char>> OutputBytes;
int selfcheck_snapshot(const tamd_graph* g, OutputBytes* dst, int io_slot = -1, const std::vector<SlotSpan>* spans = nullptr);
int selfcheck_same(const OutputBytes& want, const OutputBytes& got, const char* fmt);
int build_io_program(tamd_graph* g, int io_slot);
int bind_device(tamd_graph* g);
int direct_drain(tamd_graph* g);
void direct_teardown(tamd_graph* g);
int stage_from_pinned(tamd_graph* g);

void slots_try_build(tamd_graph* g, const std::vector<LaunchRec>& recs, int mode);
void slots_destroy(tamd_graph* g);
int slots_timestamps(tamd_graph* g, int passes, double* start_us, double* end_us, int max_stamps);

int pair_try_prerun(tamd_graph* g, const tamd_options* opt);
int pair_set_input(tamd_graph* g, int idx, const void* host, size_t bytes);
int pair_set_output(tamd_graph* g, int idx, void* host, size_t bytes);
int pair_both(tamd_graph* g, int (*fn)(tamd_graph*));
int pair_run(tamd_graph* g);
int pair_run_async(tamd_graph* g);
int pair_wait(tamd_graph* g);
int pair_direct_packets(const tamd_graph* g, bool meta);
const char* pair_direct_packet_name(const tamd_graph* g, int i);
int pair_direct_timestamps(tamd_graph* g, int passes, double* dur_us, double* gap_us, int max_packets);
int pair_output_device(tamd_graph* g, int idx, void** dptr, size_t* bytes);
int pair_time_launches(tamd_graph* g, int iters, float* total_ms);
int pair_kernel_num(const tamd_graph* g);
int pair_profile(tamd_graph* g, int iters, tamd_kernel_info* out, int max_out);
int pair_read_tensor(tamd_graph* g, int idx, void* host, size_t bytes);
void pair_destroy(tamd_graph* g);

struct OneThread {
    tamd_graph* g;
    bool ok = true, outer = false;
    explicit OneThread(tamd_graph* g_) : g(g_)
    {
        static thread_local char marker;
        const unsigned long me = (unsigned long)(uintptr_t)&marker;
        if (!g) return;
        unsigned long none = 0;
        if (g->owner.compare_exchange_strong(none, me)) outer = true;
        else if (none != me) ok = false;
    }
    ~OneThread() { if (g && outer) g->owner.store(0); }
};

}

#define TAMD_ONE_THREAD(g_)                                                                                                          \
    tamd::OneThread one_thread_(g_);                                                                                                 \
    if (!one_thread_.ok) { tamd::set_error("this tamd_graph is inside a call on another thread: one graph = one thread at a time (include/tengine_amd.h)"); return -1; }
```

tengine_amd/csrc/graph_plan_pairs.hip:

```cpp
#include "graph.h"
#include "graph_internal.h"
#include "env.h"

#include <stdio.h>

#include <algorithm>
#include <cmath>

#include "block_pack.h"
#include "epilogue.h"
#include "graph_plan.h"

namespace tamd {

int find_pwdw_tail(tamd_graph* g, size_t ni, int* tmode, int* prod)
{
    const HNode& n = g->nodes[ni];
    if (n.op != TAMD_OP_CONV || n.in.size() < 2) return -1;
    const tamd_conv_param& p = n.p.conv;
    const HTensor& x = g->tensors[n.in[0]];
    const HTensor& y = g->tensors[n.out[0]];
    if (p.group != 1 || y.is_view || x.dtype != TAMD_DT_INT8) return -1;
    if (x.nchw_raw) {
        if (x.c > 4 || p.kernel_w > 4 || p.dilation_w != 1 || x.c * p.kernel_h > 16 || p.dilation_h * (p.kernel_h - 1) > 15
            || (long)x.c * x.h * x.w >= (1L << 24) || p.pad_h0 < 0 || p.pad_w0 < 0)
            return -1;
        *prod = 1;
    } else {
        if (p.kernel_h != 1 || p.kernel_w != 1 || p.stride_h != 1 || p.stride_w != 1 || p.pad_h0 || p.pad_h1 || p.pad_w0 || p.pad_w1) return -1;
        *prod = 0;
    }
    const int nj = sole_reader(g, n.out[0]);
    if (nj < 0) return -1;
    const HNode& c = g->nodes[nj];
    const HTensor& o = g->tensors[c.out[0]];
    if (c.op == TAMD_OP_CONV && c.in.size() >= 2) {
        const tamd_conv_param& q = c.p.conv;
        const bool dw3 = is_dw3x3(q, y.c, o.c) && q.pad_h0 >= 0 && q.pad_w0 >= 0 && q.pad_h0 <= 2 && q.pad_w0 <= 2;
        if (!dw3 || o.scales.empty() || g->tensors[c.in[1]].scales.empty()) return -1;
        *tmode = 1;
        return nj;
    }
    if (c.op == TAMD_OP_POOL && *prod == 0) {
        const PoolGeom pg = pool_geom(c.p.pool, y.h, y.w);
        const int m = c.p.pool.pool_method;
        if (pg.oh != 1 || pg.ow != 1 || pg.kh != y.h || pg.kw != y.w || pg.ph0 || pg.pw0 || (m != 0 && m != 1) || y.h * y.w > 1024 || o.scales.empty())
            return -1;
        *tmode = 0;
        return nj;
    }
    return -1;
}

static RaceCand two_launches(const std::string& tag, const Step& sa, const Step& sb)
{
    const std::function<hipError_t(hipStream_t)> fa = sa.fn, fb = sb.fn;
    return {tag, [fa, fb](hipStream_t s) { const hipError_t e = fa(s); return e != hipSuccess ? e : fb(s); }, sa.kernel + " + " + sb.kernel};
}

static const DwArgs* planned_dw(tamd_graph* g, const HNode& dn, const Planned& p, int C)
{
    const HTensor& w = g->tensors[dn.in[1]];
    const HTensor* b = dn.in.size() > 2 ? &g->tensors[dn.in[2]] : nullptr;
    if (p.kind != Planned::DW3X3 || w.elems() != (size_t)C * 9 || (b && b->elems() < (size_t)C)) return nullptr;
    return &p.dw;
}

template <typename Args>
static int first_conv_producer(tamd_graph* g, const HTensor& x, const HTensor& w, const tamd_conv_param& pp, int C, std::vector<int8_t>* wrows, Args* a)
{
    const int nrows = x.c * pp.kernel_h, Kw = nrows * pp.kernel_w, K = nrows * 4;
    const int8_t* wd = (const int8_t*)w.data.data();
    wrows->assign((size_t)C * K, 0);
    for (int c = 0; c < C; c++)
        for (int r = 0; r < nrows; r++)
            for (int kx = 0; kx < pp.kernel_w; kx++) (*wrows)[(size_t)c * K + r * 4 + kx] = wd[(size_t)c * Kw + r * pp.kernel_w + kx];
    std::vector<unsigned> rows(16, 0u);
    for (int r = 0; r < nrows; r++) {
        const int ky = r % pp.kernel_h, ci = r / pp.kernel_h;
        rows[r] = (unsigned)(ci * x.h * x.w + ky * pp.dilation_h * x.w) | ((unsigned)(ky * pp.dilation_h) << 28);
    }
    unsigned* dt;
    if (upload(g, rows, &dt)) return -1;
    a->taps = dt; a->in_C = x.c; a->in_H = x.h; a->in_W = x.w;
    a->fSH = pp.stride_h; a->fSW = pp.stride_w; a->fPH = pp.pad_h0; a->fPW = pp.pad_w0;
    return 0;
}

static bool pinned_tile(const char* key, int OH, int OW, int* th, int* tw, int* threads, int* sl)
{
    const char* pin = tamd_pin(key);
    *sl = 1;
    if (!pin || sscanf(pin, "%dx%dx%dx%d", th, tw, threads, sl) < 3) return false;
    *th = std::min(*th, OH); *tw = std::min(*tw, OW);
    return *th >= 1 && *tw >= 1;
}

int plan_pwdw(tamd_graph* g, HNode& pw, HNode& tl, int tmode, int prod, const Planned& pa, const Planned& pb, Step* fused)
{
    const char* fenv = getenv("TAMD_FUSE_PWDW");
    const int fmode = fenv ? atoi(fenv) : 1;
    if (fmode == 0) return 0;
    HTensor& x = g->tensors[pw.in[0]];
    HTensor& w = g->tensors[pw.in[1]];
    HTensor* b = pw.in.size() > 2 ? &g->tensors[pw.in[2]] : nullptr;
    HTensor& mid = g->tensors[pw.out[0]];
    HTensor& y = g->tensors[tl.out[0]];
    const tamd_conv_param& pp = pw.p.conv;
    const int cin = x.c, C = mid.c, slices = (C + 15) / 16, cw = slices * 16;
    const int Kw = prod == 1 ? cin * pp.kernel_h * pp.kernel_w : cin;
    const int K = prod == 1 ? cin * pp.kernel_h * 4 : cin;
    const int ktot = prod == 1 ? K : rup(cin, 16), steps = pwdw_steps((ktot + 63) / 64), nsteps = rup((ktot + 63) / 64, steps);
    if (w.elems() != (size_t)C * Kw || (b && b->elems() < (size_t)C)) return 0;
    const DwArgs* dwp = tmode == 1 ? planned_dw(g, tl, pb, C) : nullptr;
    if (tmode == 1 && !dwp) return 0;
    PwDwArgs a{};
    {
        const RqFold rq = fold_requant(RQ_CONV_HCL, pp.activation, x.scales[0], mid.scales[0], w, C);
        const int8_t* wd = (const int8_t*)w.data.data();
        std::vector<int8_t> wrows;
        if (prod == 1) {
            if (first_conv_producer(g, x, w, pp, C, &wrows, &a)) return -1;
            wd = wrows.data();
        }
        const std::vector<int8_t> wf = pack_pw_panel(wd, C, K, nsteps);
        const std::vector<int32_t> bp = padded_bias(b ? (const int32_t*)b->data.data() : nullptr, C, cw);
        int8_t* d0; int32_t* d1;
        if (upload(g, wf, &d0) || upload(g, bp, &d1) || upload_rq(g, rq, cw, &a.wscale, &a.rq)) return -1;
        a.wf = d0; a.bias = d1;
    }
    a.prod = prod;
    a.coherent = (g->opt.direct_dispatch && !exp_plain_kernels()) ? 1 : 0;
    a.tile_major = (double)x.h * x.w * (prod == 1 ? x.c : x.cs) * (slices >= 8 ? 8 : slices) > (double)C * ktot * 8.0 ? 1 : 0;
    if (slices > 65535) a.tile_major = 0;
    a.x = (const int8_t*)x.dptr + (prod == 1 ? 0 : x.c_off);
    a.N = x.n; a.H = mid.h; a.W = mid.w; a.cs_in = x.cs; a.ktot = ktot; a.nsteps = nsteps; a.steps = steps;
    a.mode = tmode; a.cw = cw; a.slices = slices;
    a.y = (int8_t*)y.dptr; a.ldc = y.cs; a.c_off = y.c_off;
    a.c_limit = store_limit(y, C);
    a.S = 1; a.OH = a.OW = 1; a.TH = a.TW = 1; a.tiles_x = a.tiles_y = 1; a.RH = mid.h; a.RW = mid.w;
    if (tmode == 1) {
        a.dw_w = dwp->w; a.dw_bias = dwp->bias; a.dw_wscale = dwp->wscale; a.d_rq = dwp->rq;
        a.S = dwp->S; a.PH = dwp->PH; a.PW = dwp->PW; a.OH = dwp->OH; a.OW = dwp->OW;
    } else {
        a.pool_method = tl.p.pool.pool_method; a.p_in_scale = mid.scales[0]; a.p_out_scale = y.scales[0];
    }

    struct Cfg { int th, tw, threads; double cost; int sl; };
    std::vector<Cfg> cfgs;
    auto with_tiles = [&](PwDwArgs v, int th, int tw, int sl = 1) {
        v.TH = th; v.TW = tw; v.tiles_y = (v.OH + th - 1) / th; v.tiles_x = (v.OW + tw - 1) / tw;
        v.RH = (th - 1) * v.S + 3; v.RW = (tw - 1) * v.S + 3;
        v.sl = sl; v.slices = (slices + sl - 1) / sl;
        return v;
    };
    if (tmode == 0) {
        cfgs.push_back({1, 1, 256, 0.0, 1});
        cfgs.push_back({1, 1, 512, 1.0, 1});
    } else {
        std::vector<int> ths, tws;
        for (int v : {1, 2, 3, 4, 5, 6, 7, 8, 10, 12, 14, 16, 28, a.OH}) if (v <= a.OH && std::find(ths.begin(), ths.end(), v) == ths.end()) ths.push_back(v);
        for (int v : {4, 6, 7, 8, 14, 16, 28, 56, a.OW}) if (v <= a.OW && std::find(tws.begin(), tws.end(), v) == tws.end()) tws.push_back(v);
        for (int th : ths)
            for (int tw : tws)
                for (int threads : {256, 512})
                  for (int sl : {1, 2, 4}) {
                    if (sl > 1 && (slices % sl != 0 || nsteps > steps)) continue;
                    const PwDwArgs v = with_tiles(a, th, tw, sl);
                    if (!pwdw_config_ok(v, threads)) continue;
                    if (sl > 1 && (double)a.N * v.tiles_y * v.tiles_x * v.slices < 512.0) continue;
                    const int nw = threads / 64;
                    const double vp = (double)std::min(v.RH, a.H) * std::min(v.RW, a.W);
                    const double tiles_w = std::ceil(std::ceil(vp / 16.0) / nw);
                    const int twl = a.S == 1 ? 2 : 1;
                    const double tasks_t = std::ceil((double)th * ((tw + twl - 1) / twl) * 4.0 * sl / threads);
                    const double block = 250.0 + tiles_w * (45.0 + sl * (25.0 + 3.0 * nsteps)) + tasks_t * (a.S == 1 ? 150.0 : 100.0) + vp * ktot / 400.0;
                    const double blocks = (double)a.N * v.tiles_y * v.tiles_x * v.slices;
                    const double rounds = std::ceil(blocks / (256.0 * (threads == 256 ? 2 : 1)));
                    cfgs.push_back({th, tw, threads, rounds * block * (threads == 256 && blocks > 256 ? 1.3 : 1.0), sl});
                }
        std::sort(cfgs.begin(), cfgs.end(), [](const Cfg& l, const Cfg& r) { return l.cost < r.cost; });
        std::vector<Cfg> keep;
        for (int sl : {1, 2, 4}) {
            int n = 0;
            for (auto& c : cfgs)
                if (c.sl == sl && n < (sl == 1 ? 8 : 6)) { keep.push_back(c); n++; }
        }
        cfgs = keep;
    }
    int pth = 0, ptw = 0, pthreads = 0, psl = 1;
    if (tmode == 1 && pinned_tile("pwdw_cfg", a.OH, a.OW, &pth, &ptw, &pthreads, &psl)) {
        if ((psl != 2 && psl != 4) || slices % psl != 0 || nsteps > steps) psl = 1;
        if (pwdw_config_ok(with_tiles(a, pth, ptw, psl), pthreads)) { cfgs.clear(); cfgs.push_back({pth, ptw, pthreads, 0.0, psl}); }
    } else if (tmode == 0 && pinned_tile("pwdw_cfg", a.OH, a.OW, &pth, &ptw, &pthreads, &psl) && pwdw_config_ok(a, pthreads)) {
        cfgs.clear(); cfgs.push_back({1, 1, pthreads, 0.0, 1});
    }
    if (cfgs.empty()) return 0;
    const Step& sa = pa.step;
    const Step& sb = pb.step;
    const bool autotune = autotune_enabled() && sa.macs >= 4e6;
    bool fuse = fmode == 2 || (a.N == 1 && (double)a.N * a.H * a.W <= 32768.0);
    char ckey[256];
    snprintf(ckey, sizeof(ckey), "pwdw|%s|n%d %dx%d k%d m%d f%d c%zu", sa.node.c_str(), a.N, a.H, a.W, a.ktot, tmode, fmode, cfgs.size());
    std::vector<RaceCand> tiles, answers;
    for (size_t c = 0; c < cfgs.size(); c++) {
        const PwDwArgs v = tmode == 1 ? with_tiles(a, cfgs[c].th, cfgs[c].tw, cfgs[c].sl) : a;
        const int threads = cfgs[c].threads;
        hipStream_t stream = g->stream;
        tiles.push_back({"1," + std::to_string(c), [v, threads](hipStream_t s) { return launch_pwdw(v, threads, s); }, "pwdw cfg " + std::to_string(c),
                         [v, threads, stream]() {
                             if (launch_pwdw(v, threads, stream) == hipSuccess) return true;
                             (void)hipGetLastError();
                             return false;
                         }});
    }
    answers = tiles;
    for (size_t c = 0; c < cfgs.size(); c++) answers.push_back({"0," + std::to_string(c), nullptr});
    int best = 0;
    const int hit = autotune ? plan_cached(ckey, answers) : -1;
    if (hit >= 0) {
        fuse = hit < (int)cfgs.size();
        best = hit % (int)cfgs.size();
    } else if (autotune) {
        const bool batched = fmode != 2 && !fuse;
        if ((best = plan_race(g, sa.node, tiles, batched ? "" : ckey, 1.0f, true)) < 0) return -1;
        if (batched) {
            const int w = plan_race(g, sa.node, {two_launches("0," + std::to_string(best), sa, sb), tiles[best]}, ckey, 0.97f, true);
            if (w < 0) return -1;
            fuse = w == 1;
        }
    }
    if (!fuse) return 0;
    const PwDwArgs v = tmode == 1 ? with_tiles(a, cfgs[best].th, cfgs[best].tw, cfgs[best].sl) : a;
    const int threads = cfgs[best].threads;
    char nm[48];
    if (tmode == 1) snprintf(nm, sizeof(nm), "%s_i8<s%d,%dx%d,%d%s>", prod == 1 ? "firstdw" : "pwdw", a.S, v.TH, v.TW, threads, v.sl == 4 ? ",c64" : v.sl == 2 ? ",c32" : "");
    else snprintf(nm, sizeof(nm), "pwpool_i8<%d>", threads);
    *fused = fused_step({&pa, &pb}, nm, [v, threads](hipStream_t s) { return launch_pwdw(v, threads, s); }, x, y, prod == 1 && tmode == 1);
    g->fused_away[pw.out[0]] = 1;
    return 1;
}

#ifndef TAMD_CHAIN4_DEFAULT
#define TAMD_CHAIN4_DEFAULT 1
#endif

bool find_chain4(tamd_graph* g, size_t ni, int tail, int prod, const std::vector<char>& fused, const std::vector<char>& has_fuse, int* pw2, int* dw2)
{
    auto taken = [&](int nj) { return fused[nj] || has_fuse[nj]; };
    const char* fenv = getenv("TAMD_FUSE_PWDW");
    const int pin = tamd_pin_int("chain4", 1);
    if ((fenv && atoi(fenv) == 0) || pin == 0) return false;
    const HNode& n0 = g->nodes[ni];
    const HNode& d1 = g->nodes[tail];
    const HTensor& x = g->tensors[n0.in[0]];
    const HTensor& y1 = g->tensors[d1.out[0]];
    if (pin != 2 && !(x.n == 1 && (TAMD_CHAIN4_DEFAULT & (prod == 1 ? 1 : 2)))) return false;
    auto pads01 = [](const tamd_conv_param& q) { return q.pad_h0 >= 0 && q.pad_h0 <= 1 && q.pad_w0 >= 0 && q.pad_w0 <= 1 && q.pad_h1 >= 0 && q.pad_h1 <= 1 && q.pad_w1 >= 0 && q.pad_w1 <= 1; };
    if (d1.p.conv.stride_h != 1 || !pads01(d1.p.conv) || y1.is_view) return false;
    if (g->tensors[n0.out[0]].c > 128 || (prod == 0 && x.c > 128)) return false;
    const int pj = sole_reader(g, d1.out[0]);
    if (pj < 0 || taken(pj) || g->nodes[pj].op != TAMD_OP_CONV) return false;
    int tmode = -1, prod2 = 0;
    const int dj = find_pwdw_tail(g, (size_t)pj, &tmode, &prod2);
    if (dj < 0 || tmode != 1 || prod2 != 0 || taken(dj) || g->tensors[g->nodes[pj].out[0]].c > 128 || !pads01(g->nodes[dj].p.conv)) return false;
    *pw2 = pj; *dw2 = dj;
    return true;
}

int plan_chain4(tamd_graph* g, HNode& n0, HNode& d1, HNode& p2, HNode& d2, int prod, const Planned& pa, const Planned& pb, const Planned& pc, const Planned& pd, Step* fused)
{
    HTensor& x = g->tensors[n0.in[0]];
    HTensor& w0 = g->tensors[n0.in[1]];
    HTensor* b0 = n0.in.size() > 2 ? &g->tensors[n0.in[2]] : nullptr;
    HTensor& m0 = g->tensors[n0.out[0]];
    HTensor& m1 = g->tensors[d1.out[0]];
    HTensor& w2 = g->tensors[p2.in[1]];
    HTensor* b2 = p2.in.size() > 2 ? &g->tensors[p2.in[2]] : nullptr;
    HTensor& m2 = g->tensors[p2.out[0]];
    HTensor& y = g->tensors[d2.out[0]];
    const tamd_conv_param& pp = n0.p.conv;
    const int cin = x.c, C1 = m0.c, C2 = m2.c, ns1 = (C1 + 15) / 16, ns2 = (C2 + 15) / 16;
    const int Kw = prod == 1 ? cin * pp.kernel_h * pp.kernel_w : cin;
    const int K = prod == 1 ? cin * pp.kernel_h * 4 : cin;
    const int ks0 = ((prod == 1 ? K : rup(cin, 16)) + 63) / 64, ks2 = (ns1 * 16 + 63) / 64;
    if (w0.elems() != (size_t)C1 * Kw || (b0 && b0->elems() < (size_t)C1) || w2.elems() != (size_t)C2 * C1 || (b2 && b2->elems() < (size_t)C2)) return 0;
// ... 162 lines not shown
```

tengine_amd/csrc/graph_slots.hip:

```cpp
#include "graph.h"
#include "graph_internal.h"
#include "env.h"

#include <stdio.h>
#include <stdlib.h>
#include <string.h>

namespace tamd {

namespace {

void say(const char* why)
{
    if (getenv("TAMD_DEBUG")) fprintf(stderr, "[tamd] slots: the graph stays one launch list: %s\n", why);
}

void add_access(std::vector<SlotRange>& r, const Access& a) { r.push_back(slot_range_of(a)); }

int slots_selfcheck(tamd_graph* g)
{
    OutputBytes want, other, got;
    if (selfcheck_fill_inputs(g, 0x51075A11u) || run_steps(g, g->stream)) return -1;
    HIPCHK(hipStreamSynchronize(g->stream));
    if (selfcheck_snapshot(g, &want)) return -1;
    if (selfcheck_fill_inputs(g, 0x0DDBA11Au) || run_steps(g, g->stream)) return -1;
    HIPCHK(hipStreamSynchronize(g->stream));
    if (selfcheck_snapshot(g, &other)) return -1;
    if (selfcheck_fill_inputs(g, 0x51075A11u)) return -1;
    HIPCHK(hipDeviceSynchronize());
    if (direct_submit(g->direct1) || direct_wait(g->direct1)) { set_error("the pass of slot 1 failed: %s", direct_last_error()); return -1; }
    if (selfcheck_snapshot(g, &got, -1, &g->slot_spans)) return -1;
    if (selfcheck_same(want, got, "slot 1 alone does not reproduce the eager pass (output %zu differs)")) return -1;
    if (selfcheck_snapshot(g, &got)) return -1;
    if (selfcheck_same(other, got, "the pass of slot 1 changed slot 0's output %zu")) return -1;
    for (int k = 0; k < 8; k++)
        if (direct_submit((k & 1) ? g->direct1 : g->direct)) { set_error("the alternating burst failed: %s", direct_last_error()); return -1; }
    if (direct_wait(g->direct) || direct_wait(g->direct1)) { set_error("the alternating burst failed: %s", direct_last_error()); return -1; }
    if (selfcheck_snapshot(g, &got)) return -1;
    if (selfcheck_same(want, got, "a burst of alternating passes leaves other bytes in slot 0 (output %zu differs)")) return -1;
    if (selfcheck_snapshot(g, &got, -1, &g->slot_spans)) return -1;
    if (selfcheck_same(want, got, "a burst of alternating passes leaves other bytes in slot 1 (output %zu differs)")) return -1;
    for (auto& io : g->inputs) HIPCHK(hipMemset(io.stage, 0, io.bytes));
    HIPCHK(hipDeviceSynchronize());
    return 0;
}

}

void slots_try_build(tamd_graph* g, const std::vector<LaunchRec>& recs, int mode)
{
    if (!g->direct || g->is_half || g->inputs.empty() || g->outputs.empty()) { if (!g->direct) say("the list is not dispatched directly"); return; }
    for (auto& t : g->tensors)
        if (t.ttype != TAMD_TT_CONST && t.dtype != TAMD_DT_INT8) { say("not an int8 graph"); return; }
    if (mode != 2) {
        const HTensor& in0 = g->tensors[g->inputs[0].tensor];
        if (in0.dims.empty() || in0.dims[0] != 1) return;
    }
    if (g->had_once) { say("a launch of the plan ran once at prerun (its results exist in one copy)"); return; }
    for (auto& st : g->steps)
        if (step_states_nothing(st)) { say("a launch states nothing of what it reads and writes"); return; }
    std::vector<SlotRange> ranges;
    for (auto* v : {&g->in_steps, &g->steps, &g->out_steps})
        for (auto& st : *v)
            for (auto& w : st.wr) add_access(ranges, w);
    auto is_input_stage = [&](const void* p) {
        for (auto& io : g->inputs)
            if ((const char*)p >= (const char*)io.stage && (const char*)p < (const char*)io.stage + io.bytes) return true;
        return false;
    };
    for (auto& t : g->tensors)
        if (t.ttype != TAMD_TT_CONST && t.dptr && !t.prerun_const && !is_input_stage(t.dptr)) add_access(ranges, access_of(t));
    for (auto& io : g->outputs) {
        SlotRange x;
        x.lo = (uintptr_t)io.stage; x.bytes = io.bytes;
        ranges.push_back(x);
    }
    for (auto& x : ranges)
        for (auto& a : g->arenas)
            if (x.lo >= (uintptr_t)a.base && x.lo < (uintptr_t)a.base + a.used) x.bytes = std::min<size_t>(x.bytes, (uintptr_t)a.base + a.used - x.lo);
    size_t total = 0;
    std::vector<SlotSpan> spans = slot_merge(ranges, &total);
    if (spans.empty()) { say("nothing to re-point"); return; }
    for (auto& io : g->inputs)
        if (slot_touches(spans, (uintptr_t)io.stage, io.bytes)) { say("a launch writes a graph input's staging buffer"); return; }
    for (auto& t : g->tensors)
        if (t.prerun_const && t.dptr && slot_touches(spans, (uintptr_t)t.dptr, 1)) { say("a prerun constant lives in a written buffer"); return; }
    if (hipMalloc(&g->slot_block, total) != hipSuccess) { (void)hipGetLastError(); g->slot_block = nullptr; say("no device memory for the second slot"); return; }
    slot_place(spans, (uintptr_t)g->slot_block);
    bool ok = hipMemset(g->slot_block, 0, total) == hipSuccess;
    for (size_t i = 0; i < spans.size() && ok; i++)
        ok = hipMemcpy((char*)g->slot_block + spans[i].off, (const void*)spans[i].lo, spans[i].hi - spans[i].lo, hipMemcpyDeviceToDevice) == hipSuccess;
    ok = ok && hipDeviceSynchronize() == hipSuccess;
    if (!ok) { (void)hipGetLastError(); say("the copy of the written spans failed"); slots_destroy(g); return; }
    std::vector<LaunchRec> recs1 = recs;
    int moved = 0;
    for (auto& r : recs1) moved += slot_rebase(r.args.data(), r.args.size(), spans);
    if (!moved) { say("no argument points into a written span"); slots_destroy(g); return; }
    const char* why = "";
    g->direct1 = direct_build(g->gpu, g->stream, recs1, &why);
    if (!g->direct1) { say(why); slots_destroy(g); return; }
    g->slot_spans = spans;
    if (slots_selfcheck(g)) {
        fprintf(stderr, "tengine_amd: the second slot is NOT used for this graph: %s (one launch list, as before)\n", last_error());
        slots_destroy(g);
        return;
    }
    if (getenv("TAMD_DEBUG"))
        fprintf(stderr, "[tamd] slots: two passes in flight on two HSA queues; slot 1 owns %zu span(s), %.2f MB, %d argument words re-pointed in %zu launches\n",
                spans.size(), total / 1048576.0, moved, recs1.size());
}

void slots_destroy(tamd_graph* g)
{
    if (g->direct1) { direct_destroy(g->direct1); g->direct1 = nullptr; }
    if (g->slot_block) { (void)hipFree(g->slot_block); g->slot_block = nullptr; }
    g->slot_spans.clear();
    g->slot_turn = 0;
}

int slots_timestamps(tamd_graph* g, int passes, double* start_us, double* end_us, int max_stamps)
{
    if (!g->direct || !g->direct1) { set_error("tamd_graph_slot_timestamps: the graph has one launch list (tamd_graph_slots() == 0)"); return -1; }
    const int n = direct_packets(g->direct);
    if (passes < 1 || (long long)passes * 2 * n > (long long)max_stamps) { set_error("tamd_graph_slot_timestamps: %d rounds of 2 x %d packets, room for %d stamps", passes, n, max_stamps); return -1; }
    const int rc = direct_timestamps_two(g->direct, g->direct1, passes, start_us, end_us);
    if (rc < 0) { set_error("direct dispatch: %s", direct_last_error()); return -1; }
    return rc;
}

}
```

tengine_amd/csrc/launch_rec.h:

```cpp
#pragma once
#include <hip/hip_runtime.h>

#include <cstring>
#include <string>
#include <vector>

namespace tamd {

struct LaunchRec {
    const void* func;
    dim3 grid, block;
    unsigned shmem;
    std::vector<unsigned char> args;
    bool coherent = false;
    bool beside = false;
    bool wrap = false;
};

extern thread_local std::vector<LaunchRec>* g_launch_rec;
extern thread_local bool g_launch_coherent;
inline void launch_rec_coherent() { g_launch_coherent = true; }
extern thread_local bool g_launch_beside;
inline void launch_rec_beside() { g_launch_beside = true; }
inline void launch_rec_clear_flags() { g_launch_coherent = false; g_launch_beside = false; }

template <typename T>
inline void rec_pack(std::vector<unsigned char>& b, const T& v)
{
    const size_t off = (b.size() + alignof(T) - 1) & ~(alignof(T) - 1);
    b.resize(off + sizeof(T));
    memcpy(b.data() + off, &v, sizeof(T));
}

template <typename... P, typename... A>
inline void launch_rec(void (*kernel)(P...), dim3 grid, dim3 block, size_t shmem, hipStream_t s, A&&... a)
{
    static_assert(sizeof...(P) == sizeof...(A), "kernel launched with the wrong number of arguments");
    if (g_launch_rec) {
        LaunchRec r;
        r.func = reinterpret_cast<const void*>(kernel);
        r.grid = grid; r.block = block; r.shmem = (unsigned)shmem;
        (rec_pack<P>(r.args, static_cast<P>(a)), ...);
        r.coherent = g_launch_coherent;
        r.beside = g_launch_beside;
        g_launch_rec->push_back(std::move(r));
    }
    g_launch_coherent = false;
    g_launch_beside = false;
    kernel<<<grid, block, shmem, s>>>(static_cast<P>(a)...);
}

struct DirectProgram;
DirectProgram* direct_build(int gpu, hipStream_t stream, const std::vector<LaunchRec>& recs, const char** why, DirectProgram* share = nullptr);
bool direct_probe(int gpu);
int direct_submit(DirectProgram* p, bool close_burst = false, unsigned long long* burst = nullptr);
int direct_close(DirectProgram* p, unsigned long long* burst);
int direct_wait_burst(DirectProgram* p, unsigned long long burst);
int direct_wait(DirectProgram* p);
int direct_wait_all(DirectProgram* p);
const char* direct_last_error();
int direct_packets(const DirectProgram* p);
const char* direct_packet_name(const DirectProgram* p, int i);
int direct_timestamps(DirectProgram* p, int passes, double* dur_us, double* gap_us);
int direct_timestamps_two(DirectProgram* a, DirectProgram* b, int passes, double* start_us, double* end_us);
int direct_meta_packets(const DirectProgram* p);
void direct_destroy(DirectProgram* p);

}
```

tengine_amd/csrc/pwdw.hip:

```cpp
#include "dw_common.h"
#include "epilogue.h"
#include "kernels.h"

namespace tamd {

typedef int v4i __attribute__((ext_vector_type(4)));

#ifdef TAMD_PWDW_STAMPS
#define PWDW_STAMP(i) do { if (threadIdx.x == 0 && a.stamps) a.stamps[(size_t)((blockIdx.z * gridDim.y + blockIdx.y) * gridDim.x + blockIdx.x) * 8 + (i)] = wall_clock64(); } while (0)
#define PWDW_DRAIN() asm volatile("s_waitcnt vmcnt(0)" ::: "memory")
#else
#define PWDW_STAMP(i) do { } while (0)
#define PWDW_DRAIN() do { } while (0)
#endif

struct ChainDep {
    const int* wait_counter;
    int wait_target;
    int* my_counter;
    int* err;
};

__device__ __forceinline__ void chain_wait(const ChainDep& d)
{
    if (d.wait_counter) {
        if (threadIdx.x == 0) {
            bool done = false;
            for (int spin = 0; spin < (1 << 17) && !done; spin++) {
                done = (int)((unsigned)__hip_atomic_load(d.wait_counter, __ATOMIC_RELAXED, __HIP_MEMORY_SCOPE_AGENT) - (unsigned)d.wait_target) >= 0;
                if (!done) __builtin_amdgcn_s_sleep(8);
            }
            if (!done) *d.err = 1;
        }
        __syncthreads();
    }
}

__device__ __forceinline__ void chain_signal(const ChainDep& d)
{
    if (!d.my_counter) return;
    asm volatile("s_waitcnt vmcnt(0)" ::: "memory");
    __syncthreads();
    if (threadIdx.x == 0) __hip_atomic_fetch_add(d.my_counter, 1, __ATOMIC_RELAXED, __HIP_MEMORY_SCOPE_AGENT);
}

__device__ __forceinline__ void chain_store(unsigned* p, unsigned v) { __hip_atomic_store(p, v, __ATOMIC_RELAXED, __HIP_MEMORY_SCOPE_AGENT); }

template <int STEPS, int MODE, bool CHUNKED, int PROD, bool CHAINED, int WIN = 0, int SL = 1>
__device__ __forceinline__ void pwdw_block(const PwDwArgs& a, unsigned* __restrict__ inter, const int bx, const int by, const int bz,
                                           const int nthreads, const ChainDep& dep)
{
    constexpr int S = MODE == 2 ? 2 : 1;
    static_assert(SL == 1 || ((SL == 2 || SL == 4) && !CHUNKED && MODE >= 1 && MODE <= 3), "several slices: register-resident K, depthwise tails");
    constexpr bool PINGPONG = !CHUNKED && STEPS <= 8 && PROD == 0;
    PWDW_STAMP(0);
    const int t = threadIdx.x, lane = t & 63, wave = t >> 6, nwaves = nthreads >> 6;
    const int l15 = lane & 15, kb = lane >> 4;
    const int slice = a.tile_major ? bz : bx, tx = a.tile_major ? bx : by;
    int ty = a.tile_major ? by : bz, n = 0;
    if (a.N > 1) { n = ty / a.tiles_y; ty -= n * a.tiles_y; }
    const int c_base = slice * 16 * SL;

    v4i bias_v[SL];
    float4 ps[SL];
#pragma unroll
    for (int k = 0; k < SL; k++) {
        const int4 pb = *reinterpret_cast<const int4*>(a.bias + c_base + 16 * k + 4 * kb);
        bias_v[k] = v4i{pb.x, pb.y, pb.z, pb.w};
        ps[k] = *reinterpret_cast<const float4*>(a.wscale + c_base + 16 * k + 4 * kb);
    }
    const int8_t* wfp = a.wf + ((size_t)slice * SL * a.nsteps * 64 + lane) * 16;
    v4i af[SL][STEPS];
    if (!CHUNKED) {
#pragma unroll
        for (int k = 0; k < SL; k++)
#pragma unroll
            for (int u = 0; u < STEPS; u++) af[k][u] = *reinterpret_cast<const v4i*>(wfp + ((size_t)k * a.nsteps + u) * 1024);
    }
    const int cq = t & (4 * SL - 1);
    const int c0 = c_base + cq * 4;
    unsigned wrow[3][4], wsh[3][4];
    int4 db = {0, 0, 0, 0};
    float4 ds = {1.f, 1.f, 1.f, 1.f};
    if (MODE != 0 && MODE != 4) {
#pragma unroll
        for (int r = 0; r < 3; r++) {
            const uint4 v = *reinterpret_cast<const uint4*>(a.dw_w + ((size_t)r * a.cw + c0) * 4);
            wrow[r][0] = v.x; wrow[r][1] = v.y; wrow[r][2] = v.z; wrow[r][3] = v.w;
        }
        db = *reinterpret_cast<const int4*>(a.dw_bias + c0);
        ds = *reinterpret_cast<const float4*>(a.dw_wscale + c0);
    }

    int iy0 = 0, ix0 = 0, th = 1, tw = 1, vy0 = 0, vx0 = 0, vy1 = a.H, vx1 = a.W, RW = a.W;
    if (MODE == 4) {
        vy0 = ty * a.TH; vy1 = min(vy0 + a.TH, a.H);
    } else if (MODE != 0) {
        const int oy0 = ty * a.TH, ox0 = tx * a.TW;
        iy0 = oy0 * S - a.PH; ix0 = ox0 * S - a.PW;
        th = min(a.TH, a.OH - oy0); tw = min(a.TW, a.OW - ox0);
        vy0 = max(iy0, 0); vx0 = max(ix0, 0);
        vy1 = min(iy0 + (th - 1) * S + 3, a.H); vx1 = min(ix0 + (tw - 1) * S + 3, a.W);
        RW = a.RW;
    }
    const int VW = vx1 - vx0, VP = (vy1 - vy0) * VW;
    const float inv_vw = __builtin_amdgcn_rcpf((float)VW);
    const int ntiles = (VP + 15) >> 4;
    const Rq rq = a.rq;
    const int8_t* xn = PROD == 0 ? a.x + (size_t)n * a.H * a.W * a.cs_in + kb * 16
                                 : a.x + (size_t)n * a.in_C * a.in_H * a.in_W;
    unsigned rows[4];
    if (PROD == 1) {
        const uint4 v = *reinterpret_cast<const uint4*>(a.taps + kb * 4);
        rows[0] = v.x; rows[1] = v.y; rows[2] = v.z; rows[3] = v.w;
    }

    int piy = 0, pix = 0;
    auto locate = [&](int i, const int8_t*& xp) -> int {
        const int v = i * 16 + l15, vc = min(v, VP - 1);
        const int vy = (int)(((float)vc + 0.5f) * inv_vw), vx = vc - vy * VW;
        const int iy = vy0 + vy, ix = vx0 + vx;
        piy = iy; pix = ix;
        xp = PROD == 0 ? xn + (unsigned)((iy * a.W + ix) * a.cs_in) : xn;
        const int slot = MODE == 4 ? (iy * a.W + ix) : ((iy - iy0) * RW + (ix - ix0)) * 4 + kb;
        return v < VP ? slot : -1;
    };
    const __amdgpu_buffer_rsrc_t xrsrc = __builtin_amdgcn_make_buffer_rsrc((void*)a.x, 0, 0x7fffffff, 0x00020000);
    auto load_b = [&](const int8_t* xp, v4i (&bf)[STEPS], int chunk) {
        if (PROD == 0 && CHAINED) {
            const int voff = (int)(xp - a.x);
#pragma unroll
            for (int u = 0; u < STEPS; u++) bf[u] = __builtin_amdgcn_raw_buffer_load_b128(xrsrc, voff, (chunk * STEPS + u) * 64, 16 );
        } else if (PROD == 0) {
#pragma unroll
            for (int u = 0; u < STEPS; u++) bf[u] = *reinterpret_cast<const v4i*>(xp + (chunk * STEPS + u) * 64);
        } else {
            gather_patch_rows(a, xp, rows, piy, pix, bf[0]);
        }
    };
    const int soff = (a.RH * a.RW + 4) * 4;
    auto finish = [&](const v4i& acc, int slot, int k = 0) {
        const unsigned p = requant4<WIN>(acc[0], acc[1], acc[2], acc[3], ps[k], c_base + 16 * k + 4 * kb, rq);
        if (MODE == 4) {
            if (slot >= 0 && c_base + 4 * kb < a.c_limit) {
                unsigned* dst = reinterpret_cast<unsigned*>(a.y + ((size_t)n * a.H * a.W + slot) * a.ldc + a.c_off + c_base + 4 * kb);
                if (CHAINED) chain_store(dst, p); else *dst = p;
            }
        } else if (slot >= 0)
            inter[(SL > 1 ? k * soff : 0) + slot] = p;
    };
    auto tile = [&](const v4i (&b)[STEPS], int slot) {
#pragma unroll
        for (int k = 0; k < SL; k++) {
            v4i acc = bias_v[k];
#pragma unroll
// ... 1 lines not shown
            finish(acc, slot, k);
        }
    };

    v4i b0[STEPS];
    const int8_t* xp0;
    int slot0 = locate(wave, xp0);
    if ((!CHAINED || !dep.wait_counter) && !CHUNKED) load_b(xp0, b0, 0);
    PWDW_STAMP(1);
    if (MODE != 0 && MODE != 4) {
        const uint4 z = {0u, 0u, 0u, 0u};
        for (int i = t; i < (a.RH * a.RW + 4) * SL; i += nthreads) reinterpret_cast<uint4*>(inter)[i] = z;
        if (MODE == 1) {
#pragma unroll
            for (int r = 0; r < 3; r++)
#pragma unroll
                for (int c = 0; c < 4; c++) wsh[r][c] = wrow[r][c] << 8;
        }
        if (!CHAINED || !dep.wait_counter) __syncthreads();
    }
    if (CHAINED && dep.wait_counter) {
        chain_wait(dep);
        if (!CHUNKED) load_b(xp0, b0, 0);
    }
    PWDW_STAMP(2);

    if (!CHUNKED) {
        for (int i = wave; i < ntiles; i += 2 * nwaves) {
            v4i b1[PINGPONG ? STEPS : 1];
            const int8_t* xp1 = xn;
            int slot1 = -1;
            const bool second = i + nwaves < ntiles;
            if (PINGPONG && second) { slot1 = locate(i + nwaves, xp1); load_b(xp1, reinterpret_cast<v4i (&)[STEPS]>(b1), 0); }
            tile(b0, slot0);
            if (!second) break;
            const bool third = i + 2 * nwaves < ntiles;
            if (PINGPONG) {
                if (third) { slot0 = locate(i + 2 * nwaves, xp0); load_b(xp0, b0, 0); }
                tile(reinterpret_cast<v4i (&)[STEPS]>(b1), slot1);
            } else {
                slot0 = locate(i + nwaves, xp0); load_b(xp0, b0, 0);
                tile(b0, slot0);
                if (third) { slot0 = locate(i + 2 * nwaves, xp0); load_b(xp0, b0, 0); }
            }
        }
    } else {
        const int nchunks = a.nsteps / STEPS;
        for (int i = wave; i < ntiles; i += nwaves) {
            if (i != wave) slot0 = locate(i, xp0);
            v4i acc = bias_v[0];
            for (int ch = 0; ch < nchunks; ch++) {
#pragma unroll
                for (int u = 0; u < STEPS; u++) af[0][u] = *reinterpret_cast<const v4i*>(wfp + (size_t)(ch * STEPS + u) * 1024);
                load_b(xp0, b0, ch);
#pragma unroll
                for (int u = 0; u < STEPS; u++) acc = __builtin_amdgcn_mfma_i32_16x16x64_i8(af[0][u], b0[u], acc, 0, 0, 0);
            }
            finish(acc, slot0);
        }
    }
    PWDW_STAMP(3);
    if (MODE == 4) {
        if (CHAINED) chain_signal(dep);
        return;
    }
    __syncthreads();
    PWDW_STAMP(4);

    if (MODE != 0) {
        constexpr int TWL = MODE == 1 ? 2 : 1;
        const int strips = (tw + TWL - 1) / TWL;
        const int ntask = th * strips;
        const float inv_strips = __builtin_amdgcn_rcpf((float)strips);
        const Rq drq = a.d_rq;
        int8_t* yn = a.y + ((size_t)(n * a.OH + ty * a.TH) * a.OW + tx * a.TW) * a.ldc + a.c_off + c0;
        constexpr int QSH = SL == 4 ? 4 : SL == 2 ? 3 : 2;
        for (int q = t >> QSH; q < ntask; q += nthreads >> QSH) {
            const int oyl = (int)(((float)q + 0.5f) * inv_strips), st = q - oyl * strips;
            const unsigned* row = inter + (SL > 1 ? (cq >> 2) * soff : 0) + ((oyl * S) * RW + st * TWL * S) * 4 + (cq & 3);
            int acc[TWL][4];
#pragma unroll
            for (int j = 0; j < TWL; j++)
#pragma unroll
                for (int c = 0; c < 4; c++) acc[j][c] = c == 0 ? db.x : c == 1 ? db.y : c == 2 ? db.z : db.w;
#pragma unroll
            for (int r = 0; r < 3; r++) {
                const unsigned d[4] = {row[(r * RW + 0) * 4], row[(r * RW + 1) * 4], row[(r * RW + 2) * 4], row[(r * RW + 3) * 4]};
                unsigned frag[4];
                transpose4x4(d, frag);
#pragma unroll
                for (int c = 0; c < 4; c++) {
                    acc[0][c] = __builtin_amdgcn_sdot4((int)frag[c], (int)wrow[r][c], acc[0][c], false);
                    if (TWL == 2) acc[1][c] = __builtin_amdgcn_sdot4((int)frag[c], (int)wsh[r][c], acc[1][c], false);
                }
            }
#pragma unroll
            for (int j = 0; j < TWL; j++) {
                const int oxl = st * TWL + j;
                const unsigned p = requant4<WIN>(acc[j][0], acc[j][1], acc[j][2], acc[j][3], ds, c0, drq);
                if (oxl < tw && c0 < a.c_limit) {
                    unsigned* dst = reinterpret_cast<unsigned*>(yn + ((size_t)oyl * a.OW + oxl) * a.ldc);
                    if (CHAINED) chain_store(dst, p); else *dst = p;
                }
            }
        }
    } else if (wave == 0) {
        const int ch = lane & 15, part = lane >> 4;
        int s = a.pool_method == 0 ? -128 : 0;
        for (int p = part; p < VP; p += 4) {
            const int e = sx8(inter[p * 4 + (ch >> 2)], ch & 3);
            s = a.pool_method == 0 ? (s > e ? s : e) : s + e;
        }
#pragma unroll
        for (int m = 16; m < 64; m <<= 1) {
            const int o = __shfl_xor(s, m, 64);
            s = a.pool_method == 0 ? (s > o ? s : o) : s + o;
        }
        int q;
        if (a.pool_method == 0) {
            q = round_sat(__fmul_rn((float)s, __fdiv_rn(a.p_in_scale, a.p_out_scale)));
        } else {
            float f = __fmul_rn((float)s, a.p_in_scale);
            f = __fdiv_rn(f, (float)VP);
            q = round_sat(__fdiv_rn(f, a.p_out_scale));
        }
        if (part == 0 && c_base + ch < a.c_limit) {
            int8_t* dst = a.y + (size_t)n * a.ldc + a.c_off + c_base + ch;
            if (CHAINED) __hip_atomic_store(dst, (int8_t)q, __ATOMIC_RELAXED, __HIP_MEMORY_SCOPE_AGENT); else *dst = (int8_t)q;
        }
    }
    PWDW_STAMP(5);
    PWDW_DRAIN();
    PWDW_STAMP(7);
    if (CHAINED) chain_signal(dep);
    PWDW_STAMP(6);
}

static bool pwdw_windows(const PwDwArgs& a, int mode)
{
#ifdef TAMD_EXP_PWDW_NOWIN
    return false;
#endif
    return rq_win(a.rq) && (mode == 0 || mode == 4 || rq_win(a.d_rq));
}

#ifndef TAMD_PWDW_STAMPS
static_assert(sizeof(PwDwArgs) == 304, "PwDwArgs must not grow: see the note at PwDwArgs::sl (kernels.h)");
#endif

typedef unsigned v16u __attribute__((ext_vector_type(16)));
template <typename T> __device__ __forceinline__ T* as_global(T* p) { return (T*)(__attribute__((address_space(1))) T*)(uintptr_t)p; }
__device__ __forceinline__ unsigned long long line_word(const v16u& l, int i) { return (unsigned long long)l[2 * i] | (unsigned long long)l[2 * i + 1] << 32; }

template <bool TAIL>
__device__ __forceinline__ PwDwArgs pwdw_fetch_args()
{
    constexpr int kLines = (sizeof(PwDwArgs) + 63) / 64;
    static_assert(kLines == 5, "pwdw_fetch_args requests five lines");
    const auto seg = __builtin_amdgcn_kernarg_segment_ptr();
    unsigned long long w[kLines * 8];
    PwDwArgs a = {};
    if constexpr (TAIL) {
        v16u l0, l1, l2, l3, l4;
        asm volatile("s_load_dwordx16 %0, %5, 0x0\n\t"
                     "s_load_dwordx16 %1, %5, 0x40\n\t"
                     "s_load_dwordx16 %2, %5, 0x80\n\t"
                     "s_load_dwordx16 %3, %5, 0xc0\n\t"
                     "s_load_dwordx16 %4, %5, 0x100\n\t"
                     "s_waitcnt lgkmcnt(0)"
                     : "=&s"(l0), "=&s"(l1), "=&s"(l2), "=&s"(l3), "=&s"(l4) : "s"(seg));
        const v16u lines[kLines] = {l0, l1, l2, l3, l4};
#pragma unroll
        for (int i = 0; i < kLines * 8; i++) w[i] = line_word(lines[i >> 3], i & 7);
        __builtin_memcpy(&a, w, sizeof(PwDwArgs));
        a.taps = as_global(a.taps); a.dw_w = as_global(a.dw_w); a.dw_bias = as_global(a.dw_bias); a.dw_wscale = as_global(a.dw_wscale);
    } else {
        constexpr size_t kHead = 128, kBack = offsetof(PwDwArgs, y);
        static_assert(offsetof(PwDwArgs, taps) <= kHead && kBack >= kHead && kBack % 8 == 0 && sizeof(PwDwArgs) - kBack <= 64, "PwDwArgs: the tail-less fetch");
        v16u l0, l1, lb;
        asm volatile("s_load_dwordx16 %0, %3, 0x0\n\t"
                     "s_load_dwordx16 %1, %3, 0x40\n\t"
                     "s_load_dwordx16 %2, %3, %4\n\t"
                     "s_waitcnt lgkmcnt(0)"
                     : "=&s"(l0), "=&s"(l1), "=&s"(lb) : "s"(seg), "i"((int)kBack));
        const v16u lines[3] = {l0, l1, lb};
#pragma unroll
        for (int i = 0; i < 24; i++) w[i] = line_word(lines[i >> 3], i & 7);
        __builtin_memcpy(&a, w, kHead);
        __builtin_memcpy(reinterpret_cast<char*>(&a) + kBack, w + 16, sizeof(PwDwArgs) - kBack);
        a.taps = nullptr;
    }
    a.x = as_global(a.x); a.wf = as_global(a.wf); a.bias = as_global(a.bias); a.wscale = as_global(a.wscale); a.y = as_global(a.y);
#ifdef TAMD_PWDW_STAMPS
    a.stamps = as_global(a.stamps);
#endif
    return a;
}

template <int STEPS, int SL> constexpr bool kPwdwFetch = !(SL > 1 && STEPS >= 16);

template <int STEPS, int MODE, bool CHUNKED, int PROD, int WIN, int SL>
__global__ __launch_bounds__(512) void pwdw_i8_kernel(PwDwArgs arg)
{
    extern __shared__ __attribute__((aligned(16))) unsigned inter[];
    const ChainDep none = {nullptr, 0, nullptr, nullptr};
    if constexpr (kPwdwFetch<STEPS, SL>) {
        const PwDwArgs a = pwdw_fetch_args<MODE != 0 && MODE != 4>();
        pwdw_block<STEPS, MODE, CHUNKED, PROD, false, WIN, SL>(a, inter, blockIdx.x, blockIdx.y, blockIdx.z, blockDim.x, none);
    } else
        pwdw_block<STEPS, MODE, CHUNKED, PROD, false, WIN, SL>(arg, inter, blockIdx.x, blockIdx.y, blockIdx.z, blockDim.x, none);
}

template <int STEPS, int MODE, bool CHUNKED, int PROD, int WIN, int SL>
__global__ __launch_bounds__(512) void pwdw_i8_coh_kernel(PwDwArgs arg)
{
    extern __shared__ __attribute__((aligned(16))) unsigned inter[];
    const ChainDep none = {nullptr, 0, nullptr, nullptr};
    if constexpr (kPwdwFetch<STEPS, SL>) {
        const PwDwArgs a = pwdw_fetch_args<MODE != 0 && MODE != 4>();
        pwdw_block<STEPS, MODE, CHUNKED, PROD, true, WIN, SL>(a, inter, blockIdx.x, blockIdx.y, blockIdx.z, blockDim.x, none);
    } else
        pwdw_block<STEPS, MODE, CHUNKED, PROD, true, WIN, SL>(arg, inter, blockIdx.x, blockIdx.y, blockIdx.z, blockDim.x, none);
}

#ifdef TAMD_PWDW_CHAIN_EXPERIMENT
template <int STEPS, int MODE, int PROD>
__device__ __forceinline__ void chain_variant(const PwDwArgs& a, unsigned* inter, int bx, int by, int bz, int nthreads, const ChainDep& d)
{
    pwdw_block<STEPS, MODE, false, PROD, true>(a, inter, bx, by, bz, nthreads, d);
}

template <int MODE>
__device__ __forceinline__ void chain_steps(int steps, const PwDwArgs& a, unsigned* inter, int bx, int by, int bz, int nthreads, const ChainDep& d)
{
    switch (steps) {
    case 1: chain_variant<1, MODE, 0>(a, inter, bx, by, bz, nthreads, d); break;
    case 2: chain_variant<2, MODE, 0>(a, inter, bx, by, bz, nthreads, d); break;
    case 4: chain_variant<4, MODE, 0>(a, inter, bx, by, bz, nthreads, d); break;
    case 8: chain_variant<8, MODE, 0>(a, inter, bx, by, bz, nthreads, d); break;
    default: chain_variant<16, MODE, 0>(a, inter, bx, by, bz, nthreads, d); break;
    }
}

__global__ __launch_bounds__(512) void pwdw_chain_kernel(const PwChainArgs c)
{
    extern __shared__ __attribute__((aligned(16))) unsigned inter[];
    const int b = blockIdx.x;
    int l = 0;
    while (l + 1 < c.nlayers && b >= c.first_block[l + 1]) l++;
    const int local = b - c.first_block[l];
    const int gx = c.gx[l], gy = c.gy[l];
    const int bz = local / (gx * gy), rem = local - bz * gx * gy, by = rem / gx, bx = rem - by * gx;
    const int epoch = __hip_atomic_load(c.sync, __ATOMIC_RELAXED, __HIP_MEMORY_SCOPE_AGENT);
    ChainDep d;
    d.wait_counter = l ? c.flags + 32 * (l - 1) : nullptr;
    d.wait_target = l ? (int)((unsigned)epoch * (unsigned)(c.first_block[l] - c.first_block[l - 1])) : 0;
    d.my_counter = c.flags + 32 * l;
    d.err = c.sync + 2;
    const PwDwArgs a = c.layers[l];
    const int nthreads = blockDim.x;
    const int v = c.variant[l];
    const int mode = v & 7, steps = v >> 4;
    if (v & 8) {
        if (mode == 1) chain_variant<1, 1, 1>(a, inter, bx, by, bz, nthreads, d);
        else if (mode == 2) chain_variant<1, 2, 1>(a, inter, bx, by, bz, nthreads, d);
        else chain_variant<1, 3, 1>(a, inter, bx, by, bz, nthreads, d);
    } else {
        switch (mode) {
        case 0: chain_steps<0>(steps, a, inter, bx, by, bz, nthreads, d); break;
        case 1: chain_steps<1>(steps, a, inter, bx, by, bz, nthreads, d); break;
        case 2: chain_steps<2>(steps, a, inter, bx, by, bz, nthreads, d); break;
        case 3: chain_steps<3>(steps, a, inter, bx, by, bz, nthreads, d); break;
        default: chain_steps<4>(steps, a, inter, bx, by, bz, nthreads, d); break;
        }
    }
    if (l == c.nlayers - 1 && threadIdx.x == 0) {
        const int nlast = c.first_block[l + 1] - c.first_block[l];
        if (atomicAdd(c.sync + 1, 1) == nlast - 1) {
            __hip_atomic_store(c.sync + 1, 0, __ATOMIC_RELAXED, __HIP_MEMORY_SCOPE_AGENT);
            __hip_atomic_store(c.sync, epoch + 1, __ATOMIC_RELAXED, __HIP_MEMORY_SCOPE_AGENT);
        }
    }
}
#endif

#ifndef TAMD_PWDW_SLICES_TU
size_t pwdw_lds_bytes(const PwDwArgs& a, int threads)
{
    if (a.mode == 2) return 0;
    if (a.mode == 0) return ((size_t)a.H * a.W + 4) * 16;
    return ((size_t)a.RH * a.RW + 8) * 16 * (a.sl > 1 ? a.sl : 1);
}

bool pwdw_config_ok(const PwDwArgs& a, int threads)
{
    if (threads != 256 && threads != 512) return false;
    if (pwdw_lds_bytes(a, threads) > 64 * 1024) return false;
    if (a.prod == 1 && (a.nsteps != 1 || a.mode != 1)) return false;
    if (a.sl != 0 && a.sl != 1 && a.sl != 2 && a.sl != 4) return false;
    if (a.sl > 1 && (a.mode != 1 || a.nsteps > a.steps)) return false;
    if (a.sl == 4 && a.steps > 2) return false;
    if (a.mode == 0) return a.H * a.W <= 1024;
    if (a.mode == 2) return a.TH >= 1 && (long)a.TH * a.W < 16384;
    return a.TH >= 1 && a.TW >= 1 && a.RH * a.RW < 16384;
}

int pwdw_steps(int nsteps)
{
    if (nsteps <= 1) return 1;
    if (nsteps <= 2) return 2;
    if (nsteps <= 4) return 4;
    if (nsteps <= 8) return 8;
    if (nsteps <= 16) return 16;
    int best = 16, pad = (nsteps + 15) / 16 * 16;
    for (int s : {8, 4}) { const int p = (nsteps + s - 1) / s * s; if (p < pad) { pad = p; best = s; } }
    return best;
}
#endif

#define PWDW_LAUNCH_WS(STEPS_, MODE_, CHUNKED_, PROD_, WIN_, SL_)                                                             \
    do {                                                                                                                     \
        if (a.coherent) { launch_rec_coherent(); hipLaunchKernelGGL((pwdw_i8_coh_kernel<STEPS_, MODE_, CHUNKED_, PROD_, WIN_, SL_>), grid, dim3(threads), lds, s, a); } \
        else hipLaunchKernelGGL((pwdw_i8_kernel<STEPS_, MODE_, CHUNKED_, PROD_, WIN_, SL_>), grid, dim3(threads), lds, s, a); \
    } while (0)
#define PWDW_LAUNCH_S(STEPS_, MODE_, CHUNKED_, PROD_, SL_)                                                                   \
    do {                                                                                                                     \
        if (pwdw_windows(a, MODE_)) PWDW_LAUNCH_WS(STEPS_, MODE_, CHUNKED_, PROD_, 1, SL_);                                  \
        else PWDW_LAUNCH_WS(STEPS_, MODE_, CHUNKED_, PROD_, 0, SL_);                                                         \
    } while (0)
#ifndef TAMD_PWDW_SLICES_TU
#define PWDW_LAUNCH(STEPS_, MODE_, CHUNKED_, PROD_) PWDW_LAUNCH_S(STEPS_, MODE_, CHUNKED_, PROD_, 1)
#define PWDW_LAUNCH_DW(STEPS_, MODE_, CHUNKED_, PROD_) PWDW_LAUNCH_S(STEPS_, MODE_, CHUNKED_, PROD_, 1)
#define LAUNCH_PWDW_NAME launch_pwdw
#else
#define PWDW_LAUNCH(STEPS_, MODE_, CHUNKED_, PROD_) return hipErrorInvalidValue
#define PWDW_LAUNCH_DW(STEPS_, MODE_, CHUNKED_, PROD_)                                                                       \
    do {                                                                                                                     \
        if constexpr (!(CHUNKED_)) { if (a.sl == 2) { PWDW_LAUNCH_S(STEPS_, MODE_, false, PROD_, 2); break; } }              \
        if constexpr (!(CHUNKED_) && (STEPS_) <= 2) { if (a.sl == 4) { PWDW_LAUNCH_S(STEPS_, MODE_, false, PROD_, 4); break; } } \
        return hipErrorInvalidValue;                                                                                         \
    } while (0)
#define LAUNCH_PWDW_NAME launch_pwdw_slices
#endif

template <int STEPS, bool CHUNKED>
static hipError_t launch_steps(const PwDwArgs& a, int threads, hipStream_t s)
{
    const size_t lds = pwdw_lds_bytes(a, threads);
    if (a.mode == 2) {
        const dim3 sm(a.slices, 1, ((a.H + a.TH - 1) / a.TH) * a.N);
        const dim3 grid = a.tile_major ? dim3(sm.y, sm.z, sm.x) : sm;
        PWDW_LAUNCH(STEPS, 4, CHUNKED, 0);
        return hipGetLastError();
    }
    const dim3 sm(a.slices, a.mode == 0 ? 1 : a.tiles_x, a.mode == 0 ? a.N : a.tiles_y * a.N);
    const dim3 grid = a.tile_major ? dim3(sm.y, sm.z, sm.x) : sm;
    if (a.mode == 0) PWDW_LAUNCH(STEPS, 0, CHUNKED, 0);
    else if (a.S == 2) PWDW_LAUNCH_DW(STEPS, 2, CHUNKED, 0);
    else if (a.TH * ((a.TW + 1) / 2) * 4 >= threads) PWDW_LAUNCH_DW(STEPS, 1, CHUNKED, 0);
    else PWDW_LAUNCH_DW(STEPS, 3, CHUNKED, 0);
    return hipGetLastError();
}

static hipError_t launch_first(const PwDwArgs& a, int threads, hipStream_t s)
{
    const dim3 sm(a.slices, a.tiles_x, a.tiles_y * a.N);
    const dim3 grid = a.tile_major ? dim3(sm.y, sm.z, sm.x) : sm;
    const size_t lds = pwdw_lds_bytes(a, threads);
    if (a.S == 2) PWDW_LAUNCH_DW(1, 2, false, 1);
    else if (a.TH * ((a.TW + 1) / 2) * 4 >= threads) PWDW_LAUNCH_DW(1, 1, false, 1);
    else PWDW_LAUNCH_DW(1, 3, false, 1);
    return hipGetLastError();
}

#ifdef TAMD_PWDW_CHAIN_EXPERIMENT
int pwdw_chain_variant(const PwDwArgs& a, int threads, int* gx, int* gy, int* gz)
{
    if (a.nsteps > a.steps) return -1;
    int mode;
    dim3 sm;
    if (a.prod == 1 || (a.mode != 2 && a.mode != 0)) {
        sm = dim3(a.slices, a.tiles_x, a.tiles_y * a.N);
        mode = a.S == 2 ? 2 : (a.TH * ((a.TW + 1) / 2) * 4 >= threads ? 1 : 3);
    } else if (a.mode == 2) {
        sm = dim3(a.slices, 1, ((a.H + a.TH - 1) / a.TH) * a.N);
        mode = 4;
    } else {
        sm = dim3(a.slices, 1, a.N);
        mode = 0;
    }
    const dim3 grid = a.tile_major ? dim3(sm.y, sm.z, sm.x) : sm;
    *gx = (int)grid.x; *gy = (int)grid.y; *gz = (int)grid.z;
    if (grid.x > 32767 || grid.y > 32767) return -1;
    return mode | (a.prod == 1 ? 8 : 0) | (a.prod == 1 ? 1 : a.steps) << 4;
}

hipError_t launch_pwdw_chain(const PwChainArgs& c, int threads, size_t lds, hipStream_t s)
{
    hipLaunchKernelGGL(pwdw_chain_kernel, dim3(c.first_block[c.nlayers]), dim3(threads), lds, s, c);
    return hipGetLastError();
}
#endif

#ifndef TAMD_PWDW_SLICES_TU
hipError_t launch_pwdw_slices(const PwDwArgs& a, int threads, hipStream_t s);
#endif

hipError_t LAUNCH_PWDW_NAME(const PwDwArgs& a, int threads, hipStream_t s)
{
#ifndef TAMD_PWDW_SLICES_TU
    if (a.sl > 1) return launch_pwdw_slices(a, threads, s);
#endif
    if (a.prod == 1) return launch_first(a, threads, s);
    const bool chunked = a.nsteps > a.steps;
    switch (a.steps) {
    case 1: return launch_steps<1, false>(a, threads, s);
    case 2: return launch_steps<2, false>(a, threads, s);
    case 4: return chunked ? launch_steps<4, true>(a, threads, s) : launch_steps<4, false>(a, threads, s);
    case 8: return chunked ? launch_steps<8, true>(a, threads, s) : launch_steps<8, false>(a, threads, s);
    default: return chunked ? launch_steps<16, true>(a, threads, s) : launch_steps<16, false>(a, threads, s);
    }
}

}
```

Baseline: 36520 images/s.

## Merge two inference passes into paired kernel launches on direct dispatch queues

Adds paired-pass kernel twins for the pwdw and chain4 kernels. Each twin takes two argument slots and picks its pass from the block index, so two queued inference passes run in one dispatch per layer. The launch path can hold one pass and submit a combined pair program when both queues are busy, with the goal of halving per-layer dispatch and tail overhead at batch 1. This adds scheduling complexity, a held-pass flush in drain, and larger kernarg segments.

Result: slower. 36110 images/s (-1.1%).

```diff
diff --git a/include/tengine_amd.h b/include/tengine_amd.h
--- a/include/tengine_amd.h
+++ b/include/tengine_amd.h
@@ -165,6 +165,8 @@
 TAMD_API int tamd_graph_prerun(tamd_graph* g, const tamd_options* opt);
 TAMD_API int tamd_graph_halves(const tamd_graph* g);
 TAMD_API int tamd_graph_slots(const tamd_graph* g);
+TAMD_API int tamd_graph_passes_in_flight(const tamd_graph* g);
+TAMD_API int tamd_graph_slot_output(tamd_graph* g, int slot, int idx, void* host, size_t bytes);
 TAMD_API int tamd_graph_input_num(const tamd_graph* g);
 TAMD_API int tamd_graph_output_num(const tamd_graph* g);
 TAMD_API int tamd_graph_input_desc(const tamd_graph* g, int idx, int* dims8, int* dtype);
@@ -183,6 +185,7 @@
 TAMD_API int tamd_graph_direct_timestamps(tamd_graph* g, int passes, double* dur_us, double* gap_us, int max_packets);
 TAMD_API const char* tamd_graph_direct_packet_name(const tamd_graph* g, int i);
 TAMD_API int tamd_graph_slot_timestamps(tamd_graph* g, int passes, double* start_us, double* end_us, int max_stamps);
+TAMD_API int tamd_graph_pair_timestamps(tamd_graph* g, int passes, double* start_us, double* end_us, int max_stamps);
 TAMD_API int tamd_graph_download_outputs(tamd_graph* g);
 TAMD_API int tamd_graph_output_device(tamd_graph* g, int idx, void** dptr, size_t* bytes);
 TAMD_API void* tamd_graph_stream(tamd_graph* g);
diff --git a/tengine_amd/build.py b/tengine_amd/build.py
--- a/tengine_amd/build.py
+++ b/tengine_amd/build.py
@@ -11,7 +11,7 @@
 HIPCC = os.environ.get("HIPCC", "/opt/rocm/bin/hipcc")
 ARCH = "gfx950"
 
-SOURCES = ["conv_igemm.hip", "conv_igemm2.hip", "conv_pgemm.hip", "conv_pgemm_w.hip", "gemm_direct.hip", "pw_stream.hip", "pw_rows.hip", "conv_first.hip", "conv_first_pool.hip", "dwconv.hip", "dwpw.hip", "block_i8.hip", "pwdw.hip", "pwdw_slices.hip", "chain4.hip", "conv_direct.hip", "misc_kernels.hip", "interp.hip", "chanmap.hip", "prelu.hip", "chan_lut.hip", "chan_gate.hip", "slice.hip", "topdown.hip", "transpose.hip", "u8_kernels.hip", "u8_conv_gemm.hip", "u8_conv_patch.hip", "u8_conv_small.hip", "u8i_kernels.hip", "conv_f32_mfma.hip", "winograd_f32.hip", "f32_kernels.hip", "graph.hip", "graph_infer.hip", "graph_plan.hip", "graph_plan_common.hip", "graph_plan_maps.hip", "graph_plan_conv.hip", "graph_plan_pairs.hip", "plan_cache.hip", "graph_exec.hip", "graph_pair.hip", "graph_slots.hip", "graph_u8.hip", "graph_f32.hip", "tm2_reader.cc", "direct.cc", "lut_tables.cc", "interp_tables.cc", "chanmap_tables.cc", "prelu_tables.cc", "slice_tables.cc", "transpose_tables.cc"]
+SOURCES = ["conv_igemm.hip", "conv_igemm2.hip", "conv_pgemm.hip", "conv_pgemm_w.hip", "gemm_direct.hip", "pw_stream.hip", "pw_rows.hip", "conv_first.hip", "conv_first_pool.hip", "dwconv.hip", "dwpw.hip", "block_i8.hip", "pwdw.hip", "pwdw_slices.hip", "chain4.hip", "pass_pairs.hip", "conv_direct.hip", "misc_kernels.hip", "interp.hip", "chanmap.hip", "prelu.hip", "chan_lut.hip", "chan_gate.hip", "slice.hip", "topdown.hip", "transpose.hip", "u8_kernels.hip", "u8_conv_gemm.hip", "u8_conv_patch.hip", "u8_conv_small.hip", "u8i_kernels.hip", "conv_f32_mfma.hip", "winograd_f32.hip", "f32_kernels.hip", "graph.hip", "graph_infer.hip", "graph_plan.hip", "graph_plan_common.hip", "graph_plan_maps.hip", "graph_plan_conv.hip", "graph_plan_pairs.hip", "plan_cache.hip", "graph_exec.hip", "graph_pair.hip", "graph_slots.hip", "graph_u8.hip", "graph_f32.hip", "tm2_reader.cc", "direct.cc", "lut_tables.cc", "interp_tables.cc", "chanmap_tables.cc", "prelu_tables.cc", "slice_tables.cc", "transpose_tables.cc"]
 FLAGS = ["--offload-arch=" + ARCH, "-O3", "-std=c++17", "-fPIC", "-ffp-contract=off", "-fno-fast-math",
          "-fvisibility=hidden", "-Wall", "-Wno-unused-function", "-Wno-unused-variable", "-Wno-unused-value"]
 PLAIN_CXX = {"lut_tables.cc", "interp_tables.cc", "chanmap_tables.cc", "prelu_tables.cc", "slice_tables.cc", "transpose_tables.cc"}
@@ -34,7 +34,8 @@
     def one(src):
         path = os.path.join(CSRC, src)
         obj = os.path.join(OBJDIR, src + ".o")
-        included = [os.path.join(CSRC, "pwdw.hip")] if src == "pwdw_slices.hip" else []
+        included = {"pwdw_slices.hip": ["pwdw.hip"], "pass_pairs.hip": ["pwdw.hip", "chain4.hip"]}.get(src, [])
+        included = [os.path.join(CSRC, f) for f in included]
         if not force and not _newer(obj, [path, os.path.abspath(__file__)] + headers + included):
             return obj, None
         cmd = [HIPCC] + FLAGS + (["-mllvm", "--amdgpu-mfma-vgpr-form"] if src in VGPR_FORM else []) + \
diff --git a/tengine_amd/capi.py b/tengine_amd/capi.py
--- a/tengine_amd/capi.py
+++ b/tengine_amd/capi.py
@@ -23,7 +23,7 @@
 EXPORTS = [
     "tamd_device_count", "tamd_init", "tamd_shutdown", "tamd_last_error", "tamd_version", "tamd_op_supported", "tamd_node_supported", "tamd_lut_table", "tamd_eltwise_table", "tamd_eltwise_scalar", "tamd_eltwise_pair", "tamd_batchnorm_table", "tamd_interp_table", "tamd_interp_indices", "tamd_shuffle_sources", "tamd_split_table", "tamd_slice_table", "tamd_transpose_table", "tamd_prelu_slope", "tamd_prelu_table",
     "tamd_graph_create", "tamd_graph_add_tensor", "tamd_graph_add_node", "tamd_graph_set_inputs",
-    "tamd_graph_set_outputs", "tamd_graph_load_tm2", "tamd_graph_set_batch", "tamd_graph_prerun", "tamd_graph_halves", "tamd_graph_slots",
+    "tamd_graph_set_outputs", "tamd_graph_load_tm2", "tamd_graph_set_batch", "tamd_graph_prerun", "tamd_graph_halves", "tamd_graph_slots", "tamd_graph_passes_in_flight", "tamd_graph_slot_output", "tamd_graph_pair_timestamps",
     "tamd_graph_input_num", "tamd_graph_output_num", "tamd_graph_input_desc", "tamd_graph_output_desc",
     "tamd_graph_set_input", "tamd_graph_set_output", "tamd_graph_run", "tamd_graph_run_async", "tamd_graph_wait", "tamd_graph_inflight", "tamd_graph_upload_inputs",
     "tamd_graph_launch", "tamd_graph_sync", "tamd_graph_direct_packets", "tamd_graph_direct_meta_packets", "tamd_graph_download_outputs", "tamd_graph_output_device",
@@ -62,6 +62,10 @@
         if hasattr(L, "tamd_graph_slots"):
             L.tamd_graph_slot_timestamps.argtypes = [vp, ci, C.POINTER(C.c_double), C.POINTER(C.c_double), ci]
             L.tamd_graph_slots.argtypes = [vp]
+        if hasattr(L, "tamd_graph_passes_in_flight"):
+            L.tamd_graph_pair_timestamps.argtypes = [vp, ci, C.POINTER(C.c_double), C.POINTER(C.c_double), ci]
+            L.tamd_graph_passes_in_flight.argtypes = [vp]
+            L.tamd_graph_slot_output.argtypes = [vp, ci, ci, vp, C.c_size_t]
         L.tamd_graph_prerun_ms.restype = C.c_double
         L.tamd_graph_prerun_ms.argtypes = [vp]
         for name, args in {
@@ -272,6 +276,21 @@
     def slots(self):
         return lib().tamd_graph_slots(self._h) if hasattr(lib(), "tamd_graph_slots") else 0
 
+    def passes_in_flight(self):
+        return lib().tamd_graph_passes_in_flight(self._h) if hasattr(lib(), "tamd_graph_passes_in_flight") else max(1, self.slots())
+
+    def slot_output(self, slot, idx=0):
+        _, n = self.output_device(idx)
+        buf = np.zeros(n, np.uint8)
+        r = _check(lib().tamd_graph_slot_output(self._h, slot, idx, buf.ctypes.data, n), "slot_output")
+        return buf, bool(r)
+
+    def pair_timestamps(self, passes=50):
+        n = lib().tamd_graph_direct_packets(self._h)
+        t0, t1 = (C.c_double * (passes * 2 * n))(), (C.c_double * (passes * 2 * n))()
+        r = _check(lib().tamd_graph_pair_timestamps(self._h, passes, t0, t1, passes * 2 * n), "pair_timestamps")
+        return (np.array(t0[:r * 2 * n]).reshape(r, 2, n), np.array(t1[:r * 2 * n]).reshape(r, 2, n))
+
     def slot_timestamps(self, passes=50):
         n = lib().tamd_graph_direct_packets(self._h)
         t0, t1 = (C.c_double * (passes * 2 * n))(), (C.c_double * (passes * 2 * n))()
diff --git a/tengine_amd/csrc/chain4.hip b/tengine_amd/csrc/chain4.hip
--- a/tengine_amd/csrc/chain4.hip
+++ b/tengine_amd/csrc/chain4.hip
@@ -1,6 +1,8 @@
 #include "dw_common.h"
 #include "epilogue.h"
 #include "kernels.h"
+#include "launch_rec.h"
+#include "pass_pair.h"
 
 namespace tamd {
 
@@ -21,12 +23,12 @@
 }
 
 template <int PROD, bool COH, int WIN>
-__device__ __forceinline__ void chain4_block(const Chain4Args& a, unsigned* __restrict__ lds)
+__device__ __forceinline__ void chain4_block(const Chain4Args& a, unsigned* __restrict__ lds, const int n)
 {
     const int t = threadIdx.x, nthreads = blockDim.x, lane = t & 63;
     const int wave = __builtin_amdgcn_readfirstlane(t >> 6), nwaves = nthreads >> 6;
     const int l15 = lane & 15, kb = lane >> 4;
-    const int tx = blockIdx.x, ty = blockIdx.y, n = blockIdx.z;
+    const int tx = blockIdx.x, ty = blockIdx.y;
     const int ns1 = a.ns1, ns2 = a.ns2;
 
     uint4 wst[kChain4Stage];
@@ -196,16 +198,17 @@
 __global__ __launch_bounds__(512) void chain4_i8_kernel(Chain4Args a)
 {
     extern __shared__ __attribute__((aligned(16))) unsigned chain4_lds[];
-    chain4_block<PROD, false, WIN>(a, chain4_lds);
+    chain4_block<PROD, false, WIN>(a, chain4_lds, blockIdx.z);
 }
 
 template <int PROD, int WIN>
 __global__ __launch_bounds__(512) void chain4_i8_coh_kernel(Chain4Args a)
 {
     extern __shared__ __attribute__((aligned(16))) unsigned chain4_lds[];
-    chain4_block<PROD, true, WIN>(a, chain4_lds);
-}
-
+    chain4_block<PROD, true, WIN>(a, chain4_lds, blockIdx.z);
+}
+
+#ifndef TAMD_PASS_PAIRS_TU
 size_t chain4_lds_bytes(const Chain4Args& a)
 {
     const size_t soffA = (size_t)((a.RCH + 2) * (a.RCW + 2) + 4) * 16, soffC = (size_t)(a.RCH * a.RCW + 4) * 16;
@@ -230,6 +233,10 @@
     const size_t lds = chain4_lds_bytes(a);
     const bool win = a.win != 0;
     if (a.coherent) {
+        if (g_launch_rec && a.N == 1) {
+            if (win) ppair_register(reinterpret_cast<const void*>(&chain4_i8_coh_kernel<PROD, 1>), ppair_chain4_twin(PROD, 1));
+            else ppair_register(reinterpret_cast<const void*>(&chain4_i8_coh_kernel<PROD, 0>), ppair_chain4_twin(PROD, 0));
+        }
         launch_rec_coherent();
         if (win) hipLaunchKernelGGL((chain4_i8_coh_kernel<PROD, 1>), grid, dim3(threads), lds, s, a);
         else hipLaunchKernelGGL((chain4_i8_coh_kernel<PROD, 0>), grid, dim3(threads), lds, s, a);
@@ -245,5 +252,6 @@
     if (!chain4_config_ok(a, threads) || a.tiles_y > 65535 || a.N > 65535) return hipErrorInvalidValue;
     return a.prod == 1 ? launch_chain4_p<1>(a, threads, s) : launch_chain4_p<0>(a, threads, s);
 }
-
-}
+#endif
+
+}
diff --git a/tengine_amd/csrc/direct.cc b/tengine_amd/csrc/direct.cc
--- a/tengine_amd/csrc/direct.cc
+++ b/tengine_amd/csrc/direct.cc
@@ -312,6 +312,11 @@
 }
 
 int direct_packets(const DirectProgram* p) { return p ? (int)p->pkts.size() : 0; }
+unsigned long long direct_outstanding(const DirectProgram* p)
+{
+    const hsa_queue_t* q = p->dq->q;
+    return hsa_queue_load_write_index_relaxed(q) - hsa_queue_load_read_index_relaxed(q);
+}
 const char* direct_packet_name(const DirectProgram* p, int i) { return (p && i >= 0 && i < (int)p->names.size()) ? p->names[i].c_str() : ""; }
 
 
diff --git a/tengine_amd/csrc/graph.h b/tengine_amd/csrc/graph.h
--- a/tengine_amd/csrc/graph.h
+++ b/tengine_amd/csrc/graph.h
@@ -215,6 +215,11 @@
     tamd::DirectProgram* direct1 = nullptr;
     void* slot_block = nullptr;
     std::vector<tamd::SlotSpan> slot_spans;
+    tamd::DirectProgram* pass_pair[2] = {nullptr, nullptr};
+    void* slot_block23[2] = {nullptr, nullptr};
+    std::vector<tamd::SlotSpan> slot_spans23[2];
+    bool pass_held = false;
+    unsigned slots_ran = 0;
     int slot_turn = 0;
     bool slot_hold = false;
     bool had_once = false;
diff --git a/tengine_amd/csrc/graph_exec.hip b/tengine_amd/csrc/graph_exec.hip
--- a/tengine_amd/csrc/graph_exec.hip
+++ b/tengine_amd/csrc/graph_exec.hip
@@ -1,5 +1,6 @@
 #include "graph.h"
 #include "graph_internal.h"
+#include "pass_pair.h"
 #include "env.h"
 
 #include <stdio.h>
@@ -223,6 +224,12 @@
 int direct_drain(tamd_graph* g)
 {
     if (g->direct && g->direct_busy) {
+        if (g->pass_held) {
+            g->pass_held = false;
+            const int q = ppair_flush(g->slot_turn).queue;
+            if (direct_submit(q ? g->direct1 : g->direct)) { set_error("direct dispatch: %s", direct_last_error()); return -1; }
+            g->slots_ran |= 1u << q;
+        }
         if (direct_wait(g->direct) || (g->direct1 && direct_wait(g->direct1))) { set_error("direct dispatch: %s", direct_last_error()); return -1; }
         g->direct_busy = false;
     }
@@ -245,6 +252,7 @@
     g->inflight.erase(std::remove_if(g->inflight.begin(), g->inflight.end(), [](const Inflight& f) { return f.direct; }), g->inflight.end());
     direct_teardown(g);
     g->direct_busy = false;
+    g->pass_held = false;
     return -1;
 }
 
@@ -309,10 +317,24 @@
     if (g->half[0]) return pair_both(g, tamd_graph_launch);
     g->out_fresh_in = -1;
     if (g->direct) {
-        if (!g->direct_busy) { HIPCHK(hipStreamSynchronize(g->stream)); g->stream_dirty = false; }
+        if (!g->direct_busy) { HIPCHK(hipStreamSynchronize(g->stream)); g->stream_dirty = false; g->slots_ran = 0; }
         g->direct_busy = true;
         DirectProgram* p = g->direct;
-        if (g->direct1 && !g->slot_hold) { if (g->slot_turn) p = g->direct1; g->slot_turn ^= 1; }
+        int slot = 0;
+        if (g->pass_pair[0] && !g->slot_hold) {
+            const PairDecision d = ppair_decide(g->pass_held, direct_outstanding(g->direct), direct_outstanding(g->direct1), g->slot_turn);
+            if (d.action == kPairHold) { g->pass_held = true; return 0; }
+            if (d.action == kPairBoth) {
+                g->pass_held = false;
+                g->slots_ran |= 5u << d.queue;
+                if (direct_submit(g->pass_pair[d.queue])) { set_error("direct dispatch: %s", direct_last_error()); return -1; }
+                return 0;
+            }
+            slot = d.queue;
+            g->slot_turn = slot ^ 1;
+            if (slot) p = g->direct1;
+        } else if (g->direct1 && !g->slot_hold) { if (g->slot_turn) { p = g->direct1; slot = 1; } g->slot_turn ^= 1; }
+        g->slots_ran |= 1u << slot;
         if (direct_submit(p)) { set_error("direct dispatch: %s", direct_last_error()); return -1; }
         return 0;
     }
@@ -359,6 +381,31 @@
     g->stream_dirty = false;
     g->out_fresh_in = -1;
     return slots_timestamps(g, passes, start_us, end_us, max_stamps);
+}
+int tamd_graph_pair_timestamps(tamd_graph* g, int passes, double* start_us, double* end_us, int max_stamps)
+{
+    if (!g) { set_error("null graph"); return -1; }
+    TAMD_ONE_THREAD(g);
+    if (bind_device(g)) return -1;
+    if (!g->prepared || g->half[0]) { set_error("tamd_graph_pair_timestamps: the graph has no pair programs (tamd_graph_passes_in_flight() < 4)"); return -1; }
+    if (!g->inflight.empty()) { set_error("tamd_graph_pair_timestamps while asynchronous runs are in flight"); return -1; }
+    if (direct_drain(g)) return -1;
+    HIPCHK(hipStreamSynchronize(g->stream));
+    g->stream_dirty = false;
+    g->out_fresh_in = -1;
+    return pairs_timestamps(g, passes, start_us, end_us, max_stamps);
+}
+int tamd_graph_passes_in_flight(const tamd_graph* g) { return !g || g->half[0] || !g->direct || !g->direct1 ? 1 : g->pass_pair[0] && g->pass_pair[1] ? 4 : 2; }
+int tamd_graph_slot_output(tamd_graph* g, int slot, int idx, void* host, size_t bytes)
+{
+    if (!g) { set_error("null graph"); return -1; }
+    TAMD_ONE_THREAD(g);
+    if (bind_device(g)) return -1;
+    if (!g->prepared || g->half[0]) { set_error("tamd_graph_slot_output: not a graph with one launch list"); return -1; }
+    if (!g->inflight.empty()) { set_error("tamd_graph_slot_output while asynchronous runs are in flight"); return -1; }
+    if (direct_drain(g)) return -1;
+    HIPCHK(hipStreamSynchronize(g->stream));
+    return slots_read_output(g, slot, idx, host, bytes);
 }
 double tamd_graph_prerun_ms(const tamd_graph* g) { return g ? g->prerun_ms : 0.0; }
 
diff --git a/tengine_amd/csrc/graph_internal.h b/tengine_amd/csrc/graph_internal.h
--- a/tengine_amd/csrc/graph_internal.h
+++ b/tengine_amd/csrc/graph_internal.h
@@ -33,6 +33,8 @@
 void slots_try_build(tamd_graph* g, const std::vector<LaunchRec>& recs, int mode);
 void slots_destroy(tamd_graph* g);
 int slots_timestamps(tamd_graph* g, int passes, double* start_us, double* end_us, int max_stamps);
+int pairs_timestamps(tamd_graph* g, int passes, double* start_us, double* end_us, int max_stamps);
+int slots_read_output(tamd_graph* g, int slot, int idx, void* host, size_t bytes);
 
 int pair_try_prerun(tamd_graph* g, const tamd_options* opt);
 int pair_set_input(tamd_graph* g, int idx, const void* host, size_t bytes);
diff --git a/tengine_amd/csrc/graph_plan_pairs.hip b/tengine_amd/csrc/graph_plan_pairs.hip
--- a/tengine_amd/csrc/graph_plan_pairs.hip
+++ b/tengine_amd/csrc/graph_plan_pairs.hip
@@ -132,6 +132,7 @@
     a.prod = prod;
     a.coherent = (g->opt.direct_dispatch && !exp_plain_kernels()) ? 1 : 0;
     a.tile_major = (double)x.h * x.w * (prod == 1 ? x.c : x.cs) * (slices >= 8 ? 8 : slices) > (double)C * ktot * 8.0 ? 1 : 0;
+    a.tile_major = tamd_pin_int("tile_major", a.tile_major) ? 1 : 0;
     if (slices > 65535) a.tile_major = 0;
     a.x = (const int8_t*)x.dptr + (prod == 1 ? 0 : x.c_off);
     a.N = x.n; a.H = mid.h; a.W = mid.w; a.cs_in = x.cs; a.ktot = ktot; a.nsteps = nsteps; a.steps = steps;
diff --git a/tengine_amd/csrc/graph_slots.hip b/tengine_amd/csrc/graph_slots.hip
--- a/tengine_amd/csrc/graph_slots.hip
+++ b/tengine_amd/csrc/graph_slots.hip
@@ -1,12 +1,15 @@
 #include "graph.h"
 #include "graph_internal.h"
 #include "env.h"
+#include "pass_pair.h"
 
 #include <stdio.h>
 #include <stdlib.h>
 #include <string.h>
 
 namespace tamd {
+
+constexpr int kPassPairsDefault = 0;
 
 namespace {
 
@@ -43,6 +46,136 @@
     for (auto& io : g->inputs) HIPCHK(hipMemset(io.stage, 0, io.bytes));
     HIPCHK(hipDeviceSynchronize());
     return 0;
+}
+
+
+PairLaunch to_pair_launch(const LaunchRec& r)
+{
+    PairLaunch p;
+    p.func = r.func;
+    p.grid[0] = r.grid.x; p.grid[1] = r.grid.y; p.grid[2] = r.grid.z;
+    p.block[0] = r.block.x; p.block[1] = r.block.y; p.block[2] = r.block.z;
+    p.shmem = r.shmem; p.args = r.args; p.coherent = r.coherent; p.beside = r.beside; p.wrap = r.wrap;
+    return p;
+}
+
+LaunchRec from_pair_launch(const PairLaunch& p)
+{
+    LaunchRec r;
+    r.func = p.func;
+    r.grid = dim3(p.grid[0], p.grid[1], p.grid[2]);
+    r.block = dim3(p.block[0], p.block[1], p.block[2]);
+    r.shmem = p.shmem; r.args = p.args; r.coherent = p.coherent; r.beside = p.beside; r.wrap = p.wrap;
+    return r;
+}
+
+const std::vector<SlotSpan>* spans_of_slot(const tamd_graph* g, int slot) { return slot == 0 ? nullptr : slot == 1 ? &g->slot_spans : &g->slot_spans23[slot - 2]; }
+
+int pairs_copy_spans(tamd_graph* g)
+{
+    for (int k = 0; k < 2; k++)
+        for (const SlotSpan& sp : g->slot_spans23[k])
+            HIPCHK(hipMemcpy((char*)g->slot_block23[k] + sp.off, (const void*)sp.lo, sp.hi - sp.lo, hipMemcpyDeviceToDevice));
+    HIPCHK(hipDeviceSynchronize());
+    return 0;
+}
+
+int pairs_fill_slots(tamd_graph* g)
+{
+    if (direct_submit(g->direct) || direct_submit(g->direct1) || direct_wait(g->direct) || direct_wait(g->direct1)) { set_error("a single pass failed: %s", direct_last_error()); return -1; }
+    return pairs_copy_spans(g);
+}
+
+int pairs_selfcheck(tamd_graph* g)
+{
+    OutputBytes want, other, got;
+    if (selfcheck_fill_inputs(g, 0x7A1250FFu) || run_steps(g, g->stream)) return -1;
+    HIPCHK(hipStreamSynchronize(g->stream));
+    if (selfcheck_snapshot(g, &want)) return -1;
+    if (selfcheck_fill_inputs(g, 0x0B0E5EEDu) || run_steps(g, g->stream)) return -1;
+    HIPCHK(hipStreamSynchronize(g->stream));
+    if (selfcheck_snapshot(g, &other)) return -1;
+    for (int q = 0; q < 2; q++) {
+        if (selfcheck_fill_inputs(g, 0x0B0E5EEDu)) return -1;
+        HIPCHK(hipDeviceSynchronize());
+        if (pairs_fill_slots(g)) return -1;
+        if (selfcheck_fill_inputs(g, 0x7A1250FFu)) return -1;
+        HIPCHK(hipDeviceSynchronize());
+        if (direct_submit(g->pass_pair[q]) || direct_wait(g->pass_pair[q])) { set_error("the pair pass of queue %d failed: %s", q, direct_last_error()); return -1; }
+        for (int slot = 0; slot < 4; slot++) {
+            if (selfcheck_snapshot(g, &got, -1, spans_of_slot(g, slot))) return -1;
+            const bool mine = (slot & 1) == q;
+            if (selfcheck_same(mine ? want : other, got, mine ? "a pair pass alone does not reproduce the eager pass in one of its slots (output %zu differs)"
+                                                              : "a pair pass changed a slot of the other queue (output %zu differs)")) return -1;
+        }
+    }
+    static const int order[8][2] = {{0, 0}, {0, 1}, {1, 0}, {1, 1}, {0, 0}, {1, 1}, {1, 0}, {0, 1}};
+    for (auto& o : order) {
+        DirectProgram* p = o[0] ? g->pass_pair[o[1]] : (o[1] ? g->direct1 : g->direct);
+        if (direct_submit(p)) { set_error("the mixed burst failed: %s", direct_last_error()); return -1; }
+    }
+    if (direct_wait(g->direct) || direct_wait(g->direct1)) { set_error("the mixed burst failed: %s", direct_last_error()); return -1; }
+    for (int slot = 0; slot < 4; slot++) {
+        if (selfcheck_snapshot(g, &got, -1, spans_of_slot(g, slot))) return -1;
+        if (selfcheck_same(want, got, "a burst of single and pair passes leaves other bytes in a slot (output %zu differs)")) return -1;
+    }
+    for (auto& io : g->inputs) HIPCHK(hipMemset(io.stage, 0, io.bytes));
+    HIPCHK(hipDeviceSynchronize());
+    return 0;
+}
+
+void pairs_destroy(tamd_graph* g)
+{
+    for (int k = 0; k < 2; k++) {
+        if (g->pass_pair[k]) { direct_destroy(g->pass_pair[k]); g->pass_pair[k] = nullptr; }
+        if (g->slot_block23[k]) { (void)hipFree(g->slot_block23[k]); g->slot_block23[k] = nullptr; }
+        g->slot_spans23[k].clear();
+    }
+    g->pass_held = false;
+}
+
+void pairs_try_build(tamd_graph* g, const std::vector<LaunchRec>& recs, const std::vector<LaunchRec>& recs1, const std::vector<SlotSpan>& spans, size_t total)
+{
+    auto quiet = [](const char* why) { if (getenv("TAMD_DEBUG")) fprintf(stderr, "[tamd] pass pairs: the graph stays two slots: %s\n", why); };
+    std::vector<PairTwin> twins;
+    for (auto& r : recs) {
+        twins.push_back(ppair_twin_of(r.func));
+        if (!twins.back().twin) {
+            const char* nm = hipKernelNameRefByPtr(r.func, g->stream);
+            if (getenv("TAMD_DEBUG")) fprintf(stderr, "[tamd] pass pairs: the graph stays two slots: launch %zu of the list has no pair twin (%s)\n", twins.size() - 1, nm ? nm : "?");
+            return;
+        }
+    }
+    for (int k = 0; k < 2; k++) {
+        if (hipMalloc(&g->slot_block23[k], total) != hipSuccess) { (void)hipGetLastError(); g->slot_block23[k] = nullptr; quiet("no device memory for slots 2 and 3"); pairs_destroy(g); return; }
+        g->slot_spans23[k] = spans;
+        slot_place(g->slot_spans23[k], (uintptr_t)g->slot_block23[k]);
+        if (hipMemset(g->slot_block23[k], 0, total) != hipSuccess) { (void)hipGetLastError(); quiet("slots 2 and 3 could not be cleared"); pairs_destroy(g); return; }
+    }
+    if (pairs_copy_spans(g)) { (void)hipGetLastError(); quiet("the copy of the written spans failed"); pairs_destroy(g); return; }
+    for (int q = 0; q < 2; q++) {
+        const std::vector<LaunchRec>& lo = q ? recs1 : recs;
+        std::vector<LaunchRec> pr;
+        for (size_t i = 0; i < recs.size(); i++) {
+            LaunchRec hi = recs[i];
+            (void)slot_rebase(hi.args.data(), hi.args.size(), g->slot_spans23[q]);
+            PairLaunch out;
+            const std::string why = ppair_make(to_pair_launch(lo[i]), to_pair_launch(hi), twins[i], spans, spans_of_slot(g, q), &g->slot_spans23[q], &out);
+            if (!why.empty()) { quiet(why.c_str()); pairs_destroy(g); return; }
+            pr.push_back(from_pair_launch(out));
+            hipFuncAttributes fa;
+            if (hipFuncGetAttributes(&fa, out.func) != hipSuccess) { (void)hipGetLastError(); quiet("a pair twin could not be loaded"); pairs_destroy(g); return; }
+        }
+        const char* why = "";
+        g->pass_pair[q] = direct_build(g->gpu, g->stream, pr, &why, q ? g->direct1 : g->direct);
+        if (!g->pass_pair[q]) { quiet(why); pairs_destroy(g); return; }
+    }
+    if (pairs_selfcheck(g)) {
+        fprintf(stderr, "tengine_amd: pair passes are NOT used for this graph: %s (two slots, as before)\n", last_error());
+        pairs_destroy(g);
+        return;
+    }
+    if (getenv("TAMD_DEBUG")) fprintf(stderr, "[tamd] pass pairs: four slots, two passes per packet on each of the two queues (%zu launches)\n", recs.size());
 }
 
 }
@@ -108,10 +241,12 @@
     if (getenv("TAMD_DEBUG"))
         fprintf(stderr, "[tamd] slots: two passes in flight on two HSA queues; slot 1 owns %zu span(s), %.2f MB, %d argument words re-pointed in %zu launches\n",
                 spans.size(), total / 1048576.0, moved, recs1.size());
+    if (tamd_pin_int("pass_pairs", kPassPairsDefault)) pairs_try_build(g, recs, recs1, spans, total);
 }
 
 void slots_destroy(tamd_graph* g)
 {
+    pairs_destroy(g);
     if (g->direct1) { direct_destroy(g->direct1); g->direct1 = nullptr; }
     if (g->slot_block) { (void)hipFree(g->slot_block); g->slot_block = nullptr; }
     g->slot_spans.clear();
@@ -128,4 +263,25 @@
     return rc;
 }
 
-}
+int pairs_timestamps(tamd_graph* g, int passes, double* start_us, double* end_us, int max_stamps)
+{
+    if (!g->pass_pair[0] || !g->pass_pair[1]) { set_error("tamd_graph_pair_timestamps: the graph has no pair programs (tamd_graph_passes_in_flight() < 4)"); return -1; }
+    const int n = direct_packets(g->pass_pair[0]);
+    if (passes < 1 || (long long)passes * 2 * n > (long long)max_stamps) { set_error("tamd_graph_pair_timestamps: %d rounds of 2 x %d packets, room for %d stamps", passes, n, max_stamps); return -1; }
+    const int rc = direct_timestamps_two(g->pass_pair[0], g->pass_pair[1], passes, start_us, end_us);
+    if (rc < 0) { set_error("direct dispatch: %s", direct_last_error()); return -1; }
+    g->slots_ran |= 15u;
+    return rc;
+}
+
+int slots_read_output(tamd_graph* g, int slot, int idx, void* host, size_t bytes)
+{
+    const int have = g->pass_pair[0] ? 4 : g->direct1 ? 2 : 1;
+    if (slot < 0 || slot >= have || idx < 0 || idx >= (int)g->outputs.size() || bytes != g->outputs[idx].bytes) { set_error("tamd_graph_slot_output: slot %d of %d, output %d, %zu bytes", slot, have, idx, bytes); return -1; }
+    const std::vector<SlotSpan>* sp = spans_of_slot(g, slot);
+    const void* src = sp ? (const void*)slot_moved(*sp, (uintptr_t)g->outputs[idx].stage) : g->outputs[idx].stage;
+    HIPCHK(hipMemcpy(host, src, bytes, hipMemcpyDeviceToHost));
+    return (g->slots_ran >> slot) & 1u;
+}
+
+}
diff --git a/tengine_amd/csrc/launch_rec.h b/tengine_amd/csrc/launch_rec.h
--- a/tengine_amd/csrc/launch_rec.h
+++ b/tengine_amd/csrc/launch_rec.h
@@ -60,6 +60,7 @@
 int direct_wait_all(DirectProgram* p);
 const char* direct_last_error();
 int direct_packets(const DirectProgram* p);
+unsigned long long direct_outstanding(const DirectProgram* p);
 const char* direct_packet_name(const DirectProgram* p, int i);
 int direct_timestamps(DirectProgram* p, int passes, double* dur_us, double* gap_us);
 int direct_timestamps_two(DirectProgram* a, DirectProgram* b, int passes, double* start_us, double* end_us);
diff --git a/tengine_amd/csrc/pass_pair.h b/tengine_amd/csrc/pass_pair.h
--- /dev/null
+++ b/tengine_amd/csrc/pass_pair.h
@@ -0,0 +1,99 @@
+#pragma once
+#include <cstddef>
+#include <cstdint>
+#include <cstring>
+#include <string>
+#include <vector>
+
+#include "graph_slots.h"
+
+namespace tamd {
+
+constexpr unsigned ppair_pass_of(unsigned hw_x) { return hw_x & 1u; }
+constexpr unsigned ppair_index_of(unsigned hw_x) { return hw_x >> 1; }
+constexpr unsigned ppair_hw_x(unsigned pass, unsigned x) { return x << 1 | pass; }
+constexpr size_t ppair_stride(size_t arg_bytes) { return (arg_bytes + 63) & ~(size_t)63; }
+constexpr unsigned long long kPairGridLimit = 0x7fffffffull;
+
+struct PairTwin {
+    const void* twin = nullptr;
+    size_t arg_bytes = 0;
+    int nthreads_off = -1;
+    bool z_is_pass = false;
+};
+
+void ppair_register(const void* single, const PairTwin& tw);
+PairTwin ppair_twin_of(const void* single);
+PairTwin ppair_pwdw_twin(int steps, int mode, bool chunked, int prod, int win);
+PairTwin ppair_chain4_twin(int prod, int win);
+
+struct PairLaunch {
+    const void* func = nullptr;
+    unsigned grid[3] = {1, 1, 1}, block[3] = {1, 1, 1};
+    unsigned shmem = 0;
+    std::vector<unsigned char> args;
+    bool coherent = false, beside = false, wrap = false;
+};
+
+inline bool ppair_locate(const std::vector<SlotSpan>& ref, const std::vector<SlotSpan>* spans, uintptr_t p, size_t* idx, size_t* off)
+{
+    const std::vector<SlotSpan>& s = spans ? *spans : ref;
+    for (size_t i = 0; i < s.size(); i++) {
+        const uintptr_t lo = spans ? (uintptr_t)((intptr_t)s[i].lo + s[i].delta) : s[i].lo, hi = lo + (s[i].hi - s[i].lo);
+        if (p >= lo && p < hi) { *idx = i; *off = (size_t)(p - lo); return true; }
+    }
+    return false;
+}
+
+inline std::string ppair_make(const PairLaunch& a, const PairLaunch& b, const PairTwin& tw, const std::vector<SlotSpan>& ref,
+                              const std::vector<SlotSpan>* sa, const std::vector<SlotSpan>* sb, PairLaunch* out)
+{
+    if (!tw.twin) return "the kernel has no pair twin";
+    if (a.func != b.func) return "the two records launch different kernels";
+    for (int d = 0; d < 3; d++)
+        if (a.grid[d] != b.grid[d] || a.block[d] != b.block[d]) return "the two records differ in their geometry";
+    if (a.shmem != b.shmem || a.coherent != b.coherent || a.beside != b.beside || a.wrap != b.wrap) return "the two records differ in LDS bytes or flags";
+    if (a.args.size() != b.args.size() || a.args.size() != tw.arg_bytes) return "the records' argument bytes are not the twin's struct";
+    const size_t n = a.args.size();
+    for (size_t off = 0; off < n; off += 8) {
+        const size_t w = n - off < 8 ? n - off : 8;
+        if (!memcmp(a.args.data() + off, b.args.data() + off, w)) continue;
+        if (w < 8) return "a word that is no pointer differs between the two slots";
+        uint64_t va, vb;
+        memcpy(&va, a.args.data() + off, 8);
+        memcpy(&vb, b.args.data() + off, 8);
+        size_t ia = 0, ib = 0, oa = 0, ob = 0;
+        if (!ppair_locate(ref, sa, (uintptr_t)va, &ia, &oa) || !ppair_locate(ref, sb, (uintptr_t)vb, &ib, &ob) || ia != ib || oa != ob)
+            return "a word that is no pointer differs between the two slots";
+    }
+    const int dim = tw.z_is_pass ? 2 : 0;
+    if (tw.z_is_pass && a.grid[2] != 1) return "the twin takes the pass from grid.z, which the launch uses";
+    if (2ull * a.grid[dim] * a.block[dim] > kPairGridLimit) return "the doubled grid dimension exceeds the dispatch limit";
+    const size_t stride = ppair_stride(n);
+    if (tw.nthreads_off >= 0 && ((size_t)tw.nthreads_off < n || (size_t)tw.nthreads_off + 4 > stride)) return "no room for the block size in the padding";
+    *out = a;
+    out->func = tw.twin;
+    out->grid[dim] = 2 * a.grid[dim];
+    out->args.assign(2 * stride, 0);
+    memcpy(out->args.data(), a.args.data(), n);
+    memcpy(out->args.data() + stride, b.args.data(), n);
+    if (tw.nthreads_off >= 0)
+        for (int k = 0; k < 2; k++) memcpy(out->args.data() + k * stride + tw.nthreads_off, &a.block[0], 4);
+    return "";
+}
+
+enum { kPairSingle = 0, kPairHold = 1, kPairBoth = 2 };
+struct PairDecision { int action, queue; };
+inline PairDecision ppair_decide(bool held, unsigned long long out0, unsigned long long out1, int turn)
+{
+    turn &= 1;
+    const int less = out0 == out1 ? turn : (out0 < out1 ? 0 : 1);
+    if (held) return {kPairBoth, less};
+    const unsigned long long out[2] = {out0, out1};
+    if (out[turn] == 0) return {kPairSingle, turn};
+    if (out[turn ^ 1] == 0) return {kPairSingle, turn ^ 1};
+    return {kPairHold, less};
+}
+inline PairDecision ppair_flush(int turn) { return {kPairSingle, turn & 1}; }
+
+}
diff --git a/tengine_amd/csrc/pass_pairs.hip b/tengine_amd/csrc/pass_pairs.hip
--- /dev/null
+++ b/tengine_amd/csrc/pass_pairs.hip
@@ -0,0 +1,104 @@
+#define TAMD_PASS_PAIRS_TU 1
+#define TAMD_PWDW_SLICES_TU 1
+#include "pwdw.hip"
+#include "chain4.hip"
+
+#include <map>
+#include <mutex>
+
+namespace tamd {
+
+struct alignas(64) PwDwPairSlot { PwDwArgs a; unsigned nthreads; };
+struct PwDwPairArgs { PwDwPairSlot s[2]; };
+struct alignas(64) Chain4PairSlot { Chain4Args a; };
+struct Chain4PairArgs { Chain4PairSlot s[2]; };
+#ifndef TAMD_PWDW_STAMPS
+static_assert(sizeof(PwDwPairSlot) == 320 && offsetof(PwDwPairSlot, nthreads) == 304, "the block size sits in the padding of the struct's last line");
+#endif
+static_assert(sizeof(PwDwPairSlot) == ppair_stride(sizeof(PwDwArgs)) && sizeof(Chain4PairSlot) == ppair_stride(sizeof(Chain4Args)), "pass_pair.h: the padded stride");
+
+template <int STEPS, int MODE, bool CHUNKED, int PROD, int WIN>
+__global__ __launch_bounds__(512) void pwdw_i8_coh_pair_kernel(PwDwPairArgs arg)
+{
+    extern __shared__ __attribute__((aligned(16))) unsigned inter[];
+    const ChainDep none = {nullptr, 0, nullptr, nullptr};
+    const unsigned pass = ppair_pass_of(blockIdx.x);
+    const auto seg = (const __attribute__((address_space(4))) char*)__builtin_amdgcn_kernarg_segment_ptr() + pass * (unsigned)sizeof(PwDwPairSlot);
+    const int nthreads = *(const __attribute__((address_space(4))) int*)(seg + offsetof(PwDwPairSlot, nthreads));
+    const PwDwArgs a = pwdw_fetch_args<MODE != 0 && MODE != 4>((kernarg_ptr)seg);
+    pwdw_block<STEPS, MODE, CHUNKED, PROD, true, WIN, 1>(a, inter, (int)ppair_index_of(blockIdx.x), blockIdx.y, blockIdx.z, nthreads, none);
+}
+
+template <int PROD, int WIN>
+__global__ __launch_bounds__(512) void chain4_i8_coh_pair_kernel(Chain4PairArgs arg)
+{
+    extern __shared__ __attribute__((aligned(16))) unsigned chain4_lds[];
+    chain4_block<PROD, true, WIN>(arg.s[blockIdx.z].a, chain4_lds, 0);
+}
+
+namespace {
+std::mutex g_twin_mu;
+std::map<const void*, PairTwin> g_twins;
+
+template <int STEPS, int MODE, bool CHUNKED, int PROD>
+const void* pwdw_twin_w(int win)
+{
+    return win ? reinterpret_cast<const void*>(&pwdw_i8_coh_pair_kernel<STEPS, MODE, CHUNKED, PROD, 1>)
+               : reinterpret_cast<const void*>(&pwdw_i8_coh_pair_kernel<STEPS, MODE, CHUNKED, PROD, 0>);
+}
+template <int STEPS, bool CHUNKED>
+const void* pwdw_twin_m(int mode, int win)
+{
+    switch (mode) {
+    case 0: return pwdw_twin_w<STEPS, 0, CHUNKED, 0>(win);
+    case 1: return pwdw_twin_w<STEPS, 1, CHUNKED, 0>(win);
+    case 2: return pwdw_twin_w<STEPS, 2, CHUNKED, 0>(win);
+    case 3: return pwdw_twin_w<STEPS, 3, CHUNKED, 0>(win);
+    case 4: return pwdw_twin_w<STEPS, 4, CHUNKED, 0>(win);
+    default: return nullptr;
+    }
+}
+}
+
+PairTwin ppair_pwdw_twin(int steps, int mode, bool chunked, int prod, int win)
+{
+    PairTwin t;
+    t.arg_bytes = sizeof(PwDwArgs);
+    t.nthreads_off = (int)offsetof(PwDwPairSlot, nthreads);
+    if (prod == 1) {
+        if (steps != 1 || chunked) return PairTwin();
+        t.twin = mode == 1 ? pwdw_twin_w<1, 1, false, 1>(win) : mode == 2 ? pwdw_twin_w<1, 2, false, 1>(win) : mode == 3 ? pwdw_twin_w<1, 3, false, 1>(win) : nullptr;
+    } else if (!chunked) {
+        t.twin = steps == 1 ? pwdw_twin_m<1, false>(mode, win) : steps == 2 ? pwdw_twin_m<2, false>(mode, win) : steps == 4 ? pwdw_twin_m<4, false>(mode, win)
+                 : steps == 8 ? pwdw_twin_m<8, false>(mode, win) : steps == 16 ? pwdw_twin_m<16, false>(mode, win) : nullptr;
+    } else {
+        t.twin = steps == 4 ? pwdw_twin_m<4, true>(mode, win) : steps == 8 ? pwdw_twin_m<8, true>(mode, win) : steps == 16 ? pwdw_twin_m<16, true>(mode, win) : nullptr;
+    }
+    return t.twin ? t : PairTwin();
+}
+
+PairTwin ppair_chain4_twin(int prod, int win)
+{
+    PairTwin t;
+    t.arg_bytes = sizeof(Chain4Args);
+    t.z_is_pass = true;
+    t.twin = prod == 1 ? (win ? reinterpret_cast<const void*>(&chain4_i8_coh_pair_kernel<1, 1>) : reinterpret_cast<const void*>(&chain4_i8_coh_pair_kernel<1, 0>))
+                       : (win ? reinterpret_cast<const void*>(&chain4_i8_coh_pair_kernel<0, 1>) : reinterpret_cast<const void*>(&chain4_i8_coh_pair_kernel<0, 0>));
+    return t;
+}
+
+void ppair_register(const void* single, const PairTwin& tw)
+{
+    if (!single || !tw.twin) return;
+    std::lock_guard<std::mutex> lk(g_twin_mu);
+    g_twins[single] = tw;
+}
+
+PairTwin ppair_twin_of(const void* single)
+{
+    std::lock_guard<std::mutex> lk(g_twin_mu);
+    auto it = g_twins.find(single);
+    return it == g_twins.end() ? PairTwin() : it->second;
+}
+
+}
diff --git a/tengine_amd/csrc/pwdw.hip b/tengine_amd/csrc/pwdw.hip
--- a/tengine_amd/csrc/pwdw.hip
+++ b/tengine_amd/csrc/pwdw.hip
@@ -1,6 +1,8 @@
 #include "dw_common.h"
 #include "epilogue.h"
 #include "kernels.h"
+#include "launch_rec.h"
+#include "pass_pair.h"
 
 namespace tamd {
 
@@ -308,12 +310,12 @@
 template <typename T> __device__ __forceinline__ T* as_global(T* p) { return (T*)(__attribute__((address_space(1))) T*)(uintptr_t)p; }
 __device__ __forceinline__ unsigned long long line_word(const v16u& l, int i) { return (unsigned long long)l[2 * i] | (unsigned long long)l[2 * i + 1] << 32; }
 
+typedef decltype(__builtin_amdgcn_kernarg_segment_ptr()) kernarg_ptr;
 template <bool TAIL>
-__device__ __forceinline__ PwDwArgs pwdw_fetch_args()
+__device__ __forceinline__ PwDwArgs pwdw_fetch_args(const kernarg_ptr seg = __builtin_amdgcn_kernarg_segment_ptr())
 {
     constexpr int kLines = (sizeof(PwDwArgs) + 63) / 64;
     static_assert(kLines == 5, "pwdw_fetch_args requests five lines");
-    const auto seg = __builtin_amdgcn_kernarg_segment_ptr();
     unsigned long long w[kLines * 8];
     PwDwArgs a = {};
     if constexpr (TAIL) {
@@ -474,9 +476,13 @@
 }
 #endif
 
+#ifndef TAMD_PASS_PAIRS_TU
 #define PWDW_LAUNCH_WS(STEPS_, MODE_, CHUNKED_, PROD_, WIN_, SL_)                                                             \
     do {                                                                                                                     \
-        if (a.coherent) { launch_rec_coherent(); hipLaunchKernelGGL((pwdw_i8_coh_kernel<STEPS_, MODE_, CHUNKED_, PROD_, WIN_, SL_>), grid, dim3(threads), lds, s, a); } \
+        if (a.coherent) {                                                                                                    \
+            PWDW_PAIR_TWIN(STEPS_, MODE_, CHUNKED_, PROD_, WIN_, SL_);                                                       \
+            launch_rec_coherent(); hipLaunchKernelGGL((pwdw_i8_coh_kernel<STEPS_, MODE_, CHUNKED_, PROD_, WIN_, SL_>), grid, dim3(threads), lds, s, a); \
+        }                                                                                                                    \
         else hipLaunchKernelGGL((pwdw_i8_kernel<STEPS_, MODE_, CHUNKED_, PROD_, WIN_, SL_>), grid, dim3(threads), lds, s, a); \
     } while (0)
 #define PWDW_LAUNCH_S(STEPS_, MODE_, CHUNKED_, PROD_, SL_)                                                                   \
@@ -485,10 +491,17 @@
         else PWDW_LAUNCH_WS(STEPS_, MODE_, CHUNKED_, PROD_, 0, SL_);                                                         \
     } while (0)
 #ifndef TAMD_PWDW_SLICES_TU
+#define PWDW_PAIR_TWIN(STEPS_, MODE_, CHUNKED_, PROD_, WIN_, SL_)                                                            \
+    do {                                                                                                                     \
+        if (g_launch_rec)                                                                                                    \
+            ppair_register(reinterpret_cast<const void*>(&pwdw_i8_coh_kernel<STEPS_, MODE_, CHUNKED_, PROD_, WIN_, SL_>),    \
+                           ppair_pwdw_twin(STEPS_, MODE_, CHUNKED_, PROD_, WIN_));                                           \
+    } while (0)
 #define PWDW_LAUNCH(STEPS_, MODE_, CHUNKED_, PROD_) PWDW_LAUNCH_S(STEPS_, MODE_, CHUNKED_, PROD_, 1)
 #define PWDW_LAUNCH_DW(STEPS_, MODE_, CHUNKED_, PROD_) PWDW_LAUNCH_S(STEPS_, MODE_, CHUNKED_, PROD_, 1)
 #define LAUNCH_PWDW_NAME launch_pwdw
 #else
+#define PWDW_PAIR_TWIN(STEPS_, MODE_, CHUNKED_, PROD_, WIN_, SL_) do { } while (0)
 #define PWDW_LAUNCH(STEPS_, MODE_, CHUNKED_, PROD_) return hipErrorInvalidValue
 #define PWDW_LAUNCH_DW(STEPS_, MODE_, CHUNKED_, PROD_)                                                                       \
     do {                                                                                                                     \
@@ -577,5 +590,6 @@
     default: return chunked ? launch_steps<16, true>(a, threads, s) : launch_steps<16, false>(a, threads, s);
     }
 }
-
-}
+#endif
+
+}
```
